# pkorus/neural-imaging

Hardware: AMD Instinct MI355X
Metric: patches/s (fwd+bwd) ISP->JPEG->FAN @256^2 (higher is better)
Workload: dtype bf16; 1 GPU; c4 = train_manipulation UNet->[native,sharpen:1,resample:50,gaussian:0.83,jpeg:80]->dJPEG(QF80,soft)->FAN, ds none, trainable nip+fan, lambda_nip 0.1; raw_patch=128, batch_per_gpu=64, global_batch=64, parallelism=dp1, world_size=1, hip_graph=False

## Files before the change

include/nimg.h:

```cpp
#ifndef NIMG_H
#define NIMG_H

#include <stddef.h>
#include <stdint.h>

#ifdef __cplusplus
extern "C" {
#endif

#define NIMG_OK 0
#define NIMG_ERR_ARG (-1)
#define NIMG_ERR_LAUNCH (-2)
#define NIMG_ERR_WORKSPACE (-3)

#define NIMG_BF16_IN 1
#define NIMG_BF16_OUT 2
#define NIMG_BF16_MASK 4
#define NIMG_BF16_DZ 8
#define NIMG_D2S_OUT 16
#define NIMG_MASK_CONV 128
#define NIMG_COPY_LRELU 64
#define NIMG_S2D_OUT 32
#define NIMG_UNPOOL_OUT 512
#define NIMG_D2S_CONVT 1024
// ... 273 lines not shown
int nimg_conv2d_wgrad_bf16(const float* in1, int c1, const float* in2, int c2, const float* dz, int cout, float* dw,
                           float* db, int n, int h, int wd, int ks, int stride, int pad_t, int pad_l, int pad_mode,
                           int hout, int wout, int accumulate, void* workspace, size_t workspace_bytes, void* stream);

int nimg_conv2d_fwd_smallc_bf16(const float* in, int cin, const float* w, const float* bias, float* out, int cout,
                                int n, int h, int wd, int ks, int pad_mode, int act, float alpha, void* stream);
int nimg_conv2d_fwd_smallc_bf16_ex(const float* in, int cin, const float* w, const float* bias, float* out, int cout,
                                   int n, int h, int wd, int ks, int pad_mode, int act, float alpha, int flags, void* stream);
int nimg_conv2d_dgrad_fewin_bf16(const float* dz, const float* w, float* out, int ci, int cz, int n, int h, int wd,
                                 int ks, void* stream);

int nimg_awgn_fwd(const float* x, const float* noise, float* y, uint8_t* mask, long count, float strength,
                  void* stream);
int nimg_awgn_bwd(const float* x, const float* noise, const float* dy, const uint8_t* mask, float* dx, long count,
                  float strength, void* stream);
int nimg_gamma_fwd(const float* x, float* y, long count, float gamma, void* stream);
int nimg_gamma_bwd(const float* x, const float* dy, float* dx, long count, float gamma, void* stream);
int nimg_median_fwd(const float* x, float* y, uint8_t* sel, int n, int h, int w, int kernel, void* stream);
int nimg_median_bwd(const float* dy, const uint8_t* sel, float* dx, int n, int h, int w, int kernel, void* stream);

#define NIMG_L3IC_E_READ 1
#define NIMG_L3IC_E_LANES 2
#define NIMG_L3IC_E_RANGE 4
#define NIMG_L3IC_E_SYMBOL 8
#define NIMG_L3IC_E_FREQ 16
#define NIMG_L3IC_E_VARINT 32
#define NIMG_L3IC_E_ODD 64
#define NIMG_L3IC_E_UNUSED 128
#define NIMG_L3IC_E_STATE 256
#define NIMG_L3IC_E_RLE 512
size_t nimg_l3ic_workspace_bytes(int n_streams, int n_sym);
int nimg_l3ic_quantise(const float* z, const float* codebook, int codebook_size, uint8_t* idx, int* err, int n, int h,
                       int w, int c, void* stream);
int nimg_l3ic_encode(const uint8_t* idx, int n_streams, int n_sym, uint8_t* out, uint32_t* lengths, uint32_t* hist,
                     uint32_t* freq, void* workspace, size_t workspace_bytes, void* stream);
int nimg_l3ic_decode(const uint8_t* data, const uint32_t* offsets, const uint32_t* lengths, const float* codebook,
                     int codebook_size, float* z, uint32_t* err, int n, int h, int w, int c, void* stream);

size_t nimg_jpeg_workspace_bytes(int n, int h, int w, int hs, int vs);
int nimg_jpeg_transform(const void* x, int is_u8, int n, int h, int w, int hs, int vs, int quality, int16_t* coef, void* workspace,
                        size_t workspace_bytes, void* stream);
int nimg_jpeg_encode(const int16_t* coef, int n, int h, int w, int hs, int vs, uint8_t* out, size_t out_capacity, uint32_t* lengths,
                     void* workspace, size_t workspace_bytes, void* stream);
int nimg_jpeg_reconstruct(const int16_t* coef, int n, int h, int w, int hs, int vs, int quality, float* y, void* workspace,
                          size_t workspace_bytes, void* stream);
int nimg_jpeg_transform_items(const void* x, int is_u8, int n_src, int h, int w, int hs, int vs, const uint8_t* quality, int n_items,
                              int16_t* coef, int* err, void* workspace, size_t workspace_bytes, void* stream);
int nimg_jpeg_reconstruct_items(const int16_t* coef, int n_items, int h, int w, int hs, int vs, const uint8_t* quality, float* y, int* err,
                                void* workspace, size_t workspace_bytes, void* stream);

size_t nimg_jpeg_decode_workspace_bytes(int n, int h, int w, int hs, int vs, size_t ecd_bytes, int subseq_bits);
int nimg_jpeg_decode(const uint8_t* ecd, const uint64_t* ecd_off, const uint8_t* huffman, int n, int h, int w, int hs, int vs,
                     int subseq_bits, int16_t* coef, uint32_t* status, uint32_t* rounds, void* workspace, size_t workspace_bytes,
                     void* stream);
int nimg_jpeg_reconstruct_tables(const int16_t* coef, int n, int h, int w, int hs, int vs, const uint16_t* qtabs, void* y, int out_u8,
                                 void* workspace, size_t workspace_bytes, void* stream);

int nimg_jpeg_histogram(const int16_t* coef, int n, int h, int w, int hs, int vs, uint32_t* hist, void* stream);
int nimg_jpeg_optimal_tables(const uint32_t* hist, int n_tables, uint8_t* tables, uint32_t* status, void* stream);
size_t nimg_jpeg_encode_tables_workspace_bytes(int n, int h, int w, int hs, int vs);
int nimg_jpeg_encode_tables(const int16_t* coef, int n, int h, int w, int hs, int vs, const uint8_t* tables, uint8_t* out,
                            size_t out_capacity, uint32_t* lengths, uint32_t* status, void* workspace, size_t workspace_bytes,
                            void* stream);

int nimg_jpeg_transform_tables(const void* x, int is_u8, int n_src, int h, int w, int hs, int vs, const uint16_t* qtabs, int n_items,
                               int16_t* coef, int* err, void* workspace, size_t workspace_bytes, void* stream);
int nimg_jpeg_tables_from_float(const float* t, int n_sets, int n_tabs, uint16_t* qtabs, uint32_t* status, void* stream);

size_t nimg_jpeg_encode_restart_workspace_bytes(int n, int h, int w, int hs, int vs, int restart_interval);
int nimg_jpeg_encode_restart(const int16_t* coef, int n, int h, int w, int hs, int vs, int restart_interval, uint8_t* out,
                             size_t out_capacity, uint32_t* lengths, void* workspace, size_t workspace_bytes, void* stream);
int nimg_jpeg_histogram_restart(const int16_t* coef, int n, int h, int w, int hs, int vs, int restart_interval, uint32_t* hist,
                                void* stream);
size_t nimg_jpeg_encode_tables_restart_workspace_bytes(int n, int h, int w, int hs, int vs, int restart_interval);
int nimg_jpeg_encode_tables_restart(const int16_t* coef, int n, int h, int w, int hs, int vs, int restart_interval, const uint8_t* tables,
                                    uint8_t* out, size_t out_capacity, uint32_t* lengths, uint32_t* status, void* workspace,
                                    size_t workspace_bytes, void* stream);
size_t nimg_jpeg_decode_restart_workspace_bytes(int n, int h, int w, int hs, int vs, int restart_interval, size_t ecd_bytes,
                                                int subseq_bits);
int nimg_jpeg_decode_restart(const uint8_t* ecd, const uint64_t* ecd_off, const uint8_t* huffman, int n, int h, int w, int hs, int vs,
                             int restart_interval, int subseq_bits, int16_t* coef, uint32_t* status, uint32_t* rounds, void* workspace,
                             size_t workspace_bytes, void* stream);

#ifdef __cplusplus
}
#endif
#endif
```

neural-imaging_amd/_lib.py:

```python
import ctypes
import os
from ctypes import c_float, c_int, c_long, c_size_t, c_void_p

_HERE = os.path.dirname(os.path.abspath(__file__))
LIB_PATH = os.environ.get('NIMG_LIBPATH') or os.path.join(_HERE, 'libnimg.so')

P = c_void_p

PROTOTYPES = {
    'nimg_abi_version': (c_int, []),
    'nimg_djpeg_fwd': (c_int, [P, P, P, P, P, P, c_int, c_int, c_int, c_int, P]),
    'nimg_djpeg_bwd': (c_int, [P, P, P, P, P, c_int, c_int, c_int, c_int, P]),
    'nimg_djpeg_dq_workspace_bytes': (c_size_t, [c_int, c_int, c_int]),
    'nimg_djpeg_bwd_dq': (c_int, [P, P, P, P, P, P, c_int, c_int, c_int, c_int, c_int, P, c_size_t, P]),
    'nimg_jpeg_qtable': (c_int, [c_int, c_int, P]),
    'nimg_conv2d_fwd': (c_int, [P, c_int, P, c_int, P, P, P, c_int, P, c_int, P, c_int, c_int, c_int, c_int, c_int,
                                c_int, c_int, c_int, c_int, c_int, c_int, c_float, P]),
    'nimg_conv_flip_weights': (c_int, [P, P, c_int, c_int, c_int, c_int, P]),
    'nimg_conv2d_wgrad_workspace_bytes': (c_size_t, [c_int, c_int, c_int, c_int, c_int, c_int, c_int]),
    'nimg_conv2d_wgrad': (c_int, [P, c_int, P, c_int, P, c_int, P, P, c_int, c_int, c_int, c_int, c_int, c_int, c_int,
                                  c_int, c_int, c_int, c_int, P, c_size_t, P]),
    'nimg_bias_grad_workspace_bytes': (c_size_t, [c_long, c_int]),
    'nimg_bias_grad': (c_int, [P, P, c_long, c_int, c_int, P, c_size_t, P]),
    'nimg_bias_grad_ex': (c_int, [P, P, c_long, c_int, c_int, P, c_size_t, c_int, P]),
# ... 95 lines not shown
    'nimg_mae255': (c_int, [P, P, P, P, c_long, c_float, c_int, P, c_size_t, P]),
    'nimg_ssim_loss_workspace_bytes': (c_size_t, [c_int, c_int, c_int, c_int, c_int]),
    'nimg_ssim_loss': (c_int, [P, P, P, P, c_int, c_int, c_int, c_int, c_float, P, c_float, c_int, P, c_size_t, P]),
    'nimg_patch_stats': (c_int, [P, c_int, c_int, c_int, P, P, c_int, c_int, c_int, P, P, P]),
    'nimg_patch_select': (c_int, [P, P, P, P, c_int, c_int, c_int, c_int, P, P, P]),
    'nimg_patch_gather': (c_int, [P, P, c_int, c_int, c_int, P, P, c_int, c_int, P, P, P]),
    'nimg_mask_scale': (c_int, [P, P, P, c_long, c_float, P]),
    'nimg_conv5_dgrad_sparse_image_bytes': (c_size_t, [c_int, c_int]),
    'nimg_conv5_dgrad_sparse_weights': (c_int, [P, P, c_int, c_int, P]),
    'nimg_conv5_dgrad_sparse': (c_int, [P, P, c_int, P, P, c_int, P, c_int, c_int, c_int, c_float, c_int, P]),
    'nimg_conv2d_fwd_bf16_res': (c_int, [P, c_int, P, P, P, c_int, P, P, P, c_int, c_int, c_int, c_int, c_int, c_int, c_int, c_int, c_int,
                                 c_int, c_int, c_float, c_int, P]),
    'nimg_conv2d_fwd_bf16_unpool': (c_int, [P, P, c_int, P, P, P, c_int, P, c_int, c_int, c_int, c_int, c_int, c_int, c_int,
                                            c_int, c_int, c_float, c_int, P]),
    'nimg_conv2d_wgrad_bf16_unpool': (c_int, [P, c_int, P, P, c_int, P, P, c_int, c_int, c_int, c_int, c_int, P, c_size_t, P]),
    'nimg_cconv3': (c_int, [P, P, P, P, c_int, c_int, c_int, c_int, P]),
    'nimg_conv5c3_bf16': (c_int, [P, P, P, c_int, c_int, c_int, P]),
    'nimg_cconv3_dgrad_border': (c_int, [P, P, P, c_int, c_int, c_int, P]),
    'nimg_conv1_pool_fwd_c4': (c_int, [P, P, P, P, P, c_int, c_int, c_int, c_float, c_int, P]),
    'nimg_conv1_wgrad_c4_workspace_bytes': (c_size_t, []),
    'nimg_conv1_wgrad_c4': (c_int, [P, P, P, P, P, c_int, c_int, c_int, c_int, c_int, P, c_size_t, P]),
    'nimg_conv1_dgrad_pooled': (c_int, [P, P, P, P, c_int, c_int, c_int, c_int, P]),
    'nimg_confusion_accumulate': (c_int, [P, P, P, P, c_int, c_int, P]),
    'nimg_ssim_planes_workspace_bytes': (c_size_t, [c_int, c_int]),
    'nimg_ssim_planes': (c_int, [P, P, c_int, c_int, c_int, c_int, c_float, P, P, P, P, c_int, P, c_size_t, P]),
    'nimg_msssim_combine': (c_int, [P, P, c_int, c_int, P, P, P]),
    'nimg_ssim_maps_grad': (c_int, [P, P, P, P, P, c_int, c_int, c_int, c_int, P, c_float, c_int, P]),
    'nimg_pad2d': (c_int, [P, P, c_int, c_int, c_int, c_int, c_int, c_int, P]),
    'nimg_conv2d_fwd_bf16_ex': (c_int, [P, c_int, P, c_int, P, P, P, c_int, P, c_int, P, c_int, c_int, c_int, c_int, c_int,
                                        c_int, c_int, c_int, c_int, c_int, c_int, c_float, c_int, P]),
    'nimg_conv2d_wgrad_bf16_ex': (c_int, [P, c_int, P, c_int, P, c_int, P, P, c_int, c_int, c_int, c_int, c_int, c_int,
                                          c_int, c_int, c_int, c_int, c_int, P, c_size_t, c_int, P]),
    'nimg_conv2d_pool_fwd_bf16_ex': (c_int, [P, c_int, P, P, P, P, P, c_int, c_int, c_int, c_int, c_int, c_int, c_float,
                                             c_int, P]),
    'nimg_conv2d_dgrad_unpool_out_bf16': (c_int, [P, c_int, P, P, P, P, c_int, c_int, c_int, c_int, c_int, c_float, P]),
    'nimg_conv2d_fwd_pool_also_bf16': (c_int, [P, c_int, P, P, P, P, P, c_int, c_int, c_int, c_int, c_int, c_float, P]),
    'nimg_conv2d_wgrad_pooled_bf16_ex': (c_int, [P, c_int, P, P, c_int, P, P, c_int, c_int, c_int, c_int, c_int, P,
                                                 c_size_t, c_int, P]),
    'nimg_conv2d_dgrad_fewin_pooled_bf16_ex': (c_int, [P, P, P, P, c_int, c_int, c_int, c_int, c_int, c_int, c_int, P]),
    'nimg_maxpool2_unpool_ex': (c_int, [P, P, P, P, c_int, c_int, c_int, c_int, c_int, c_float, c_int, P]),
    'nimg_conv_weights_bf16_batch': (c_int, [P, c_int, P]),
    'nimg_convt2x2_fwd_bf16': (c_int, [P, P, P, P, c_int, c_int, c_int, c_int, c_int, P]),
    'nimg_convt2x2_fwd_bf16_ex': (c_int, [P, P, P, P, c_int, c_int, c_int, c_int, c_int, c_int, P]),
    'nimg_conv2d_fwd_smallc_bf16': (c_int, [P, c_int, P, P, P, c_int, c_int, c_int, c_int, c_int, c_int, c_int,
                                            c_float, P]),
    'nimg_conv2d_fwd_smallc_bf16_ex': (c_int, [P, c_int, P, P, P, c_int, c_int, c_int, c_int, c_int, c_int, c_int,
                                               c_float, c_int, P]),
    'nimg_conv2d_dgrad_fewin_bf16': (c_int, [P, P, P, c_int, c_int, c_int, c_int, c_int, c_int, P]),
    'nimg_awgn_fwd': (c_int, [P, P, P, P, c_long, c_float, P]),
    'nimg_awgn_bwd': (c_int, [P, P, P, P, P, c_long, c_float, P]),
    'nimg_gamma_fwd': (c_int, [P, P, c_long, c_float, P]),
    'nimg_gamma_bwd': (c_int, [P, P, P, c_long, c_float, P]),
    'nimg_median_fwd': (c_int, [P, P, P, c_int, c_int, c_int, c_int, P]),
    'nimg_median_bwd': (c_int, [P, P, P, c_int, c_int, c_int, c_int, P]),
    'nimg_sparse_axis_apply': (c_int, [P, P, P, P, P, c_int, c_int, c_int, c_int, c_int, c_int, P]),
    'nimg_l3ic_workspace_bytes': (c_size_t, [c_int, c_int]),
    'nimg_l3ic_quantise': (c_int, [P, P, c_int, P, P, c_int, c_int, c_int, c_int, P]),
    'nimg_l3ic_encode': (c_int, [P, c_int, c_int, P, P, P, P, P, c_size_t, P]),
    'nimg_l3ic_decode': (c_int, [P, P, P, P, c_int, P, P, c_int, c_int, c_int, c_int, P]),
    'nimg_jpeg_workspace_bytes': (c_size_t, [c_int, c_int, c_int, c_int, c_int]),
    'nimg_jpeg_transform': (c_int, [P, c_int, c_int, c_int, c_int, c_int, c_int, c_int, P, P, c_size_t, P]),
    'nimg_jpeg_encode': (c_int, [P, c_int, c_int, c_int, c_int, c_int, P, c_size_t, P, P, c_size_t, P]),
    'nimg_jpeg_reconstruct': (c_int, [P, c_int, c_int, c_int, c_int, c_int, c_int, P, P, c_size_t, P]),
    'nimg_jpeg_transform_items': (c_int, [P, c_int, c_int, c_int, c_int, c_int, c_int, P, c_int, P, P, P, c_size_t, P]),
    'nimg_jpeg_reconstruct_items': (c_int, [P, c_int, c_int, c_int, c_int, c_int, P, P, P, P, c_size_t, P]),
    'nimg_jpeg_decode_workspace_bytes': (c_size_t, [c_int, c_int, c_int, c_int, c_int, c_size_t, c_int]),
    'nimg_jpeg_decode': (c_int, [P, P, P, c_int, c_int, c_int, c_int, c_int, c_int, P, P, P, P, c_size_t, P]),
    'nimg_jpeg_reconstruct_tables': (c_int, [P, c_int, c_int, c_int, c_int, c_int, P, P, c_int, P, c_size_t, P]),
    'nimg_jpeg_histogram': (c_int, [P, c_int, c_int, c_int, c_int, c_int, P, P]),
    'nimg_jpeg_optimal_tables': (c_int, [P, c_int, P, P, P]),
    'nimg_jpeg_encode_tables_workspace_bytes': (c_size_t, [c_int, c_int, c_int, c_int, c_int]),
    'nimg_jpeg_encode_tables': (c_int, [P, c_int, c_int, c_int, c_int, c_int, P, P, c_size_t, P, P, P, c_size_t, P]),
    'nimg_jpeg_transform_tables': (c_int, [P, c_int, c_int, c_int, c_int, c_int, c_int, P, c_int, P, P, P, c_size_t, P]),
    'nimg_jpeg_tables_from_float': (c_int, [P, c_int, c_int, P, P, P]),
    'nimg_jpeg_encode_restart_workspace_bytes': (c_size_t, [c_int, c_int, c_int, c_int, c_int, c_int]),
    'nimg_jpeg_encode_restart': (c_int, [P, c_int, c_int, c_int, c_int, c_int, c_int, P, c_size_t, P, P, c_size_t, P]),
    'nimg_jpeg_histogram_restart': (c_int, [P, c_int, c_int, c_int, c_int, c_int, c_int, P, P]),
    'nimg_jpeg_encode_tables_restart_workspace_bytes': (c_size_t, [c_int, c_int, c_int, c_int, c_int, c_int]),
    'nimg_jpeg_encode_tables_restart': (c_int, [P, c_int, c_int, c_int, c_int, c_int, c_int, P, P, c_size_t, P, P, P, c_size_t, P]),
    'nimg_jpeg_decode_restart_workspace_bytes': (c_size_t, [c_int, c_int, c_int, c_int, c_int, c_int, c_size_t, c_int]),
    'nimg_jpeg_decode_restart': (c_int, [P, P, P, c_int, c_int, c_int, c_int, c_int, c_int, c_int, P, P, P, P, c_size_t, P]),
    'nimg_msssim_workspace_bytes': (c_size_t, [c_int, c_int, c_int, c_int]),
    'nimg_msssim': (c_int, [P, P, c_int, c_int, c_int, c_int, c_float, P, P, P, c_size_t, P]),
}

ERRORS = {-1: 'NIMG_ERR_ARG (invalid argument / unsupported configuration)',
          -2: 'NIMG_ERR_LAUNCH (HIP kernel launch failed)',
          -3: 'NIMG_ERR_WORKSPACE (workspace too small)'}

_lib = None


ABI_VERSION = 8
TICKET_BYTES = 64 * 1024


def load():
    global _lib
    if _lib is not None:
        return _lib
    if not os.path.isfile(LIB_PATH):
        raise RuntimeError('libnimg.so not found at {} - build it with neural-imaging_amd/csrc/build.sh '
                           '(or __graft_entry__.build()); there is no CPU fallback'.format(LIB_PATH))
    import torch
    lib = ctypes.CDLL(LIB_PATH)
    for name, (res, args) in PROTOTYPES.items():
        fn = getattr(lib, name)
        fn.restype = res
        fn.argtypes = args
    if lib.nimg_abi_version() != ABI_VERSION:
        raise RuntimeError('libnimg.so at {} has ABI version {}, this binding was written against {} - rebuild it '
                           '(neural-imaging_amd/csrc/build.sh)'.format(LIB_PATH, lib.nimg_abi_version(), ABI_VERSION))
    _lib = lib
    return lib


def call(name, *args):
    rc = getattr(load(), name)(*args)
    if rc != 0:
        raise RuntimeError('{} failed: {}'.format(name, ERRORS.get(rc, rc)))
    return rc
```

neural-imaging_amd/csrc/common.h:

```cpp
#pragma once
#include <hip/hip_runtime.h>
#include <stdint.h>
#include "../../include/nimg.h"

#define NIMG_CHECK_LAUNCH()                                   \
    do {                                                      \
        hipError_t e__ = hipGetLastError();                   \
        if (e__ != hipSuccess) return NIMG_ERR_LAUNCH;        \
    } while (0)

namespace nimg {

constexpr int WAVE = 64;

__device__ __forceinline__ float lrelu(float v, float alpha) { return v > 0.0f ? v : alpha * v; }

__device__ __forceinline__ float wave_sum(float v) {
#pragma unroll
    for (int o = 32; o > 0; o >>= 1) v += __shfl_xor(v, o, 64);
    return v;
}

__device__ __forceinline__ double wave_sum_d(double v) {
#pragma unroll
    for (int o = 32; o > 0; o >>= 1) v += __shfl_xor(v, o, 64);
    return v;
}

__device__ __forceinline__ bool map_coord(int& g, int size, int pad_mode) {
    const bool inside = (unsigned)g < (unsigned)size;
    const int sym = g < 0 ? -1 - g : 2 * size - 1 - g;
    const int ref = g < 0 ? -g : 2 * size - 2 - g;
    const int m = pad_mode == 1 ? sym : ref;
    const bool mapped = pad_mode != 0 && (unsigned)m < (unsigned)size;
    g = inside ? g : (mapped ? m : g);
    return inside || mapped;
}

__device__ __forceinline__ int xcd_order(int bid) {
#ifdef NIMG_NO_XCD_ORDER
    return bid;
#else
    const int g = (int)gridDim.x, x = bid & 7, r = g & 7;
    return x * (g >> 3) + (x < r ? x : r) + (bid >> 3);
#endif
}

typedef float nimg_f32x16 __attribute__((ext_vector_type(16)));

constexpr int EPI_PAD = 4;
template <int NI, bool BLOCK_SYNC = true, typename Emit>
__device__ __forceinline__ void epilogue_via_lds(const nimg_f32x16 (&acc)[NI], float* lds, int lane, Emit emit) {
    constexpr int RS = NI * 32 + EPI_PAD;
    const int half = lane >> 5, n = lane & 31;
    if (BLOCK_SYNC) __syncthreads();
    else __builtin_amdgcn_wave_barrier();
#pragma unroll
    for (int ni = 0; ni < NI; ++ni)
#pragma unroll
        for (int j = 0; j < 16; ++j) lds[((j & 3) + 8 * (j >> 2) + 4 * half) * RS + ni * 32 + n] = acc[ni][j];
    if (BLOCK_SYNC) __syncthreads();
    else __builtin_amdgcn_wave_barrier();
#pragma unroll
    for (int it = 0; it < (32 * NI * 8) / 64; ++it) {
        const int idx = it * 64 + lane, row = idx / (NI * 8), c4 = idx % (NI * 8);
        const float4 v = *reinterpret_cast<const float4*>(lds + row * RS + c4 * 4);
        emit(row, c4 * 4, v);
    }
}

template <int NI, bool BLOCK_SYNC = true, typename Bias, typename Emit>
__device__ __forceinline__ void pool_via_lds(const nimg_f32x16 (&acc)[NI], float* lds, int lane, float alpha, Bias bias4,
                                             Emit emit) {
    constexpr int RS = NI * 32 + EPI_PAD;
    const int half = lane >> 5, n = lane & 31;
    if (BLOCK_SYNC) __syncthreads();
    else __builtin_amdgcn_wave_barrier();
#pragma unroll
    for (int ni = 0; ni < NI; ++ni)
#pragma unroll
        for (int j = 0; j < 16; ++j) lds[((j & 3) + 8 * (j >> 2) + 4 * half) * RS + ni * 32 + n] = acc[ni][j];
    if (BLOCK_SYNC) __syncthreads();
    else __builtin_amdgcn_wave_barrier();
#pragma unroll
    for (int it = 0; it < NI; ++it) {
        const int idx = it * 64 + lane, pc = idx / (NI * 8), c = (idx % (NI * 8)) * 4;
        const float4 b = bias4(c);
        float m[4];
        unsigned char k[4];
#pragma unroll
        for (int pos = 0; pos < 4; ++pos) {
            const float4 r = *reinterpret_cast<const float4*>(lds + (2 * pc + (pos & 1) + 16 * (pos >> 1)) * RS + c);
            const float v[4] = {lrelu(r.x + b.x, alpha), lrelu(r.y + b.y, alpha), lrelu(r.z + b.z, alpha),
                                lrelu(r.w + b.w, alpha)};
#pragma unroll
            for (int e = 0; e < 4; ++e)
                if (pos == 0 || v[e] > m[e]) { m[e] = v[e]; k[e] = (unsigned char)pos; }
        }
// ... 351 lines not shown
```

neural-imaging_amd/csrc/conv_bf16.h:

```cpp
#pragma once
#include <stdlib.h>

#include <cstdlib>
#include "common.h"

struct ConvArgsB {
    const float* in1;
    const float* in2;
    const __bf16* wb;
    const float* bias;
    float* out1;
    float* out2;
    const float* act1;
    float* pool_out;
    unsigned char* pool_idx;
    int C1, C2, O1, O2, CinP;
    int N, H, W, Hout, Wout, pad_t, pad_l;
    int tiles_y, tiles_x, act, pad_mode;
    float alpha;
    int convt;
    int flags;
    const unsigned char* in_idx;
    const float* res;
    float* out1b;
};

namespace {

using namespace nimg;
typedef float f32x16 __attribute__((ext_vector_type(16)));
typedef __bf16 bf16x8 __attribute__((ext_vector_type(8)));

__device__ __forceinline__ bf16x8 pack8(const float (&f)[8]) {
    bf16x8 r;
#pragma unroll
    for (int k = 0; k < 8; ++k) r[k] = (__bf16)f[k];
    return r;
}

typedef __bf16 bf16x4 __attribute__((ext_vector_type(4)));
__device__ __forceinline__ void store4_bf16(float* base_as_bf16, long elem, float4 v) {
    bf16x4 o;
    o[0] = (__bf16)v.x; o[1] = (__bf16)v.y; o[2] = (__bf16)v.z; o[3] = (__bf16)v.w;
    *reinterpret_cast<bf16x4*>(reinterpret_cast<__bf16*>(base_as_bf16) + elem) = o;
}
__device__ __forceinline__ float4 load4_bf16(const float* base_as_bf16, long elem) {
    const bf16x4 o = *reinterpret_cast<const bf16x4*>(reinterpret_cast<const __bf16*>(base_as_bf16) + elem);
    return make_float4((float)o[0], (float)o[1], (float)o[2], (float)o[3]);
}

struct ConvParamsB : ConvArgsB {};

__device__ __forceinline__ unsigned unp_eq_bytes(unsigned k, unsigned pos) {
    const unsigned x = k ^ (pos * 0x01010101u);
    return (((x | (x >> 1)) & 0x01010101u) ^ 0x01010101u) * 0xFFu;
}
__device__ __forceinline__ uint4 unp_route(uint4 g, unsigned k0, unsigned k1, unsigned pos) {
    const unsigned m0 = unp_eq_bytes(k0, pos), m1 = unp_eq_bytes(k1, pos);
    return make_uint4(g.x & __builtin_amdgcn_perm(m0, m0, 0x01010000u), g.y & __builtin_amdgcn_perm(m0, m0, 0x03030202u),
                      g.z & __builtin_amdgcn_perm(m1, m1, 0x01010000u), g.w & __builtin_amdgcn_perm(m1, m1, 0x03030202u));
}

struct EpiBias { float b[8]; };
template <int NI>
__device__ __forceinline__ EpiBias epi_bias_preload(const ConvParamsB& p, int lane, int wn, int co0, int Cout) {
    EpiBias r;
#pragma unroll
    for (int e = 0; e < 8; ++e) r.b[e] = 0.f;
    const int co = co0 + wn * NI * 32 + (lane % (NI * 4)) * 8;
    if (p.bias && co + 7 < Cout) {
        const int cb = (p.flags & NIMG_D2S_CONVT) ? co % (p.O1 >> 2) : co;
        const float4 b0 = *reinterpret_cast<const float4*>(p.bias + cb), b1 = *reinterpret_cast<const float4*>(p.bias + cb + 4);
        r.b[0] = b0.x; r.b[1] = b0.y; r.b[2] = b0.z; r.b[3] = b0.w; r.b[4] = b1.x; r.b[5] = b1.y; r.b[6] = b1.z; r.b[7] = b1.w;
    }
    return r;
}

template <int TH, int TW, int NB, int PMAP>
__device__ __forceinline__ void tile_pixel(int P, int& img, int& dy, int& dx) {
    if constexpr (PMAP == 0) {
        img = P / (TH * TW);
        const int rem = P % (TH * TW);
        dy = rem / TW;
        dx = rem % TW;
    } else if constexpr (NB == 1) {
        static_assert(TH == 16 && TW == 16, "plane layout: 16 x 16 tile");
        const int f = P >> 5, l = P & 31;
        img = 0;
        dy = 4 * (f >> 1) + (l >> 3);
        dx = 8 * (f & 1) + (l & 7);
    } else {
        static_assert(TH == 8 && TW == 8 && NB == 4, "plane layout: 8 x 8 x 4 tile");
        img = (P & 31) >> 3;
        dy = P >> 5;
        dx = P & 7;
    }
}

template <int KS, int TH, int TW, int NB, int MI, int NI, int PMAP = 0>
__device__ __forceinline__ void conv_epilogue_vec(const f32x16 (&acc)[MI][NI], const ConvParamsB& p, unsigned char* smem_raw,
                                                  int wave, int lane, int wm, int wn, int co0, int Cout, int ty0, int tx0,
                                                  int grp, int phase, const EpiBias& pre_) {
#ifdef NIMG_NO_EPI_PRELOAD
    const EpiBias pre = epi_bias_preload<NI>(p, lane, wn, co0, Cout);
    (void)pre_;
#else
    const EpiBias& pre = pre_;
// ... 106 lines not shown
                    *reinterpret_cast<bf16x8*>(reinterpret_cast<__bf16*>(p.out2) + pixoff * p.O2 + (co - p.O1)) = pack8(f);
                }
            });
            if constexpr (TW == 16 && NB == 1 && PMAP == 0)
                if (p.pool_out) {
                    const int Hp = p.Hout >> 1, Wp = p.Wout >> 1, py = (ty0 >> 1) + wm * MI + mi;
                    pool_in_regs8<NI>(acc[mi], elds, lane, p.act == 1 ? p.alpha : 1.0f,
                        [&](int c) { const int co = co0 + wn * NI * 32 + c; return (p.bias && co < Cout) ? p.bias[co] : 0.f; },
                        [&](int pc, int c, float4 lo, float4 hi, uint2 k) {
                            const int co = co0 + wn * NI * 32 + c, px = (tx0 >> 1) + pc;
                            if (co >= Cout || grp >= p.N || py >= Hp || px >= Wp) return;
                            const long o = (((long)grp * Hp + py) * Wp + px) * Cout + co;
                            const float f[8] = {lo.x, lo.y, lo.z, lo.w, hi.x, hi.y, hi.z, hi.w};
                            *reinterpret_cast<bf16x8*>(reinterpret_cast<__bf16*>(p.pool_out) + o) = pack8(f);
                            if (p.pool_idx) *reinterpret_cast<uint2*>(p.pool_idx + o) = k;
                        });
                }
        }
        return;
    }
#endif
#pragma unroll
    for (int mi = 0; mi < MI; ++mi) {
        epilogue_via_lds<NI, false>(acc[mi], elds, lane, [&](int row, int c, float4 v) {
            const int co = co0 + wn * NI * 32 + c;
            if (co >= Cout) return;
            const int P = (wm * MI + mi) * 32 + row;
            int img, dy_, dx_;
            tile_pixel<TH, TW, NB, PMAP>(P, img, dy_, dx_);
            const int oy = ty0 + dy_, ox = tx0 + dx_, n = grp * NB + img;
            if (n >= p.N || oy >= p.Hout || ox >= p.Wout) return;
            const long pixoff = (KS == 1 && p.convt)
                ? ((long)n * 2 * p.Hout + 2 * oy + (phase >> 1)) * (2 * p.Wout) + 2 * ox + (phase & 1)
                : ((long)n * p.Hout + oy) * p.Wout + ox;
            if (p.bias) {
                const float4 b = *reinterpret_cast<const float4*>(p.bias + co);
                v.x += b.x; v.y += b.y; v.z += b.z; v.w += b.w;
            }
            if (p.act == 1) {
                v.x = lrelu(v.x, p.alpha); v.y = lrelu(v.y, p.alpha); v.z = lrelu(v.z, p.alpha); v.w = lrelu(v.w, p.alpha);
            }
            if (co < p.O1) {
                long o = pixoff * p.O1 + co;
                const long om_conv = o;
                if (p.flags & NIMG_D2S_OUT) {
                    const int cd = p.O1 >> 2, blk = co / cd;
                    o = (((long)n * 2 * p.Hout + 2 * oy + (blk >> 1)) * (2 * p.Wout) + 2 * ox + (blk & 1)) * cd + (co - blk * cd);
                }
                if (p.act1) {
                    const long om = (p.flags & NIMG_MASK_CONV) ? om_conv : o;
                    const float4 m = (p.flags & NIMG_BF16_MASK) ? load4_bf16(p.act1, om)
                                                                : *reinterpret_cast<const float4*>(p.act1 + om);
                    v.x *= m.x > 0.f ? 1.0f : p.alpha; v.y *= m.y > 0.f ? 1.0f : p.alpha;
                    v.z *= m.z > 0.f ? 1.0f : p.alpha; v.w *= m.w > 0.f ? 1.0f : p.alpha;
                }
                if (p.res) {
                    const float4 r = *reinterpret_cast<const float4*>(p.res + o);
                    v.x += r.x; v.y += r.y; v.z += r.z; v.w += r.w;
                }
                if (p.flags & NIMG_S2D_OUT)
                    o = (((long)n * (p.Hout >> 1) + (oy >> 1)) * (p.Wout >> 1) + (ox >> 1)) * (4 * p.O1) +
                        (2 * (oy & 1) + (ox & 1)) * p.O1 + co;
                if (p.out1b) {
                    float4 c = v;
                    if (p.flags & NIMG_COPY_LRELU) { c.x = lrelu(c.x, p.alpha); c.y = lrelu(c.y, p.alpha); c.z = lrelu(c.z, p.alpha); c.w = lrelu(c.w, p.alpha); }
                    store4_bf16(p.out1b, o, c);
                }
                if (p.flags & NIMG_BF16_OUT) store4_bf16(p.out1, o, v);
                else *reinterpret_cast<float4*>(p.out1 + o) = v;
            } else {
                if (p.flags & NIMG_BF16_OUT) store4_bf16(p.out2, pixoff * p.O2 + (co - p.O1), v);
                else *reinterpret_cast<float4*>(p.out2 + pixoff * p.O2 + (co - p.O1)) = v;
            }
        });
    }
}

}

template <int KS, int STRIDE, bool INB>
int conv_bf16_dispatch(const ConvArgsB& a, hipStream_t s);
template <int KS, bool INB>
int conv_bf16_launch_16x16(const ConvArgsB& a, bool tn32, hipStream_t s);
```

neural-imaging_amd/csrc/conv_bf16.hip:

```cpp
#include "conv_bf16.h"

namespace {

__global__ void weights_bf16_kernel(const float* __restrict__ w, __bf16* __restrict__ wb, int taps, int cin, int cout,
                                    int mode) {
    const int rows = mode == 0 ? cout : cin, cols = mode == 0 ? cin : cout;
    const int cpad = (cols + 15) / 16 * 16;
    const long total = (long)taps * rows * cpad;
    for (long i = (long)blockIdx.x * blockDim.x + threadIdx.x; i < total; i += (long)gridDim.x * blockDim.x) {
        const int c = (int)(i % 16) + 16 * (int)(i / (16L * rows * taps)), r = (int)((i / 16) % rows);
        const int t = (int)((i / (16L * rows)) % taps);
        float v = 0.f;
        if (c < cols) v = mode == 0 ? w[((long)t * cin + c) * cout + r] : w[((long)(taps - 1 - t) * cin + r) * cout + c];
        wb[i] = (__bf16)v;
    }
}

__global__ __launch_bounds__(256) void weights_bf16_batch_kernel(const long long* __restrict__ table) {
    const long long* e = table + 4 * blockIdx.y;
    const float* w = reinterpret_cast<const float*>(e[0]);
    __bf16* wb = reinterpret_cast<__bf16*>(e[1]);
    const int taps = (int)(e[2] >> 32), mode = (int)(e[2] & 0xffffffffll);
    const int cin = (int)(e[3] >> 32), cout = (int)(e[3] & 0xffffffffll);
    const int rows = mode == 0 ? cout : cin, cols = mode == 0 ? cin : cout;
    const int chunks = (cols + 15) / 16, rblocks = (rows + 63) / 64;
    const int ntiles = chunks * taps * rblocks;
    __shared__ float tile[16][65];
    const int tid = threadIdx.x;
    for (int tl = blockIdx.x; tl < ntiles; tl += gridDim.x) {
        const int rb = tl % rblocks, ct = tl / rblocks, t = ct % taps, chunk = ct / taps;
        const int r0 = rb * 64, c0 = chunk * 16;
        __syncthreads();
        if (mode == 0) {
            const int cl = tid >> 4, rq = (tid & 15) * 4;
#pragma unroll
            for (int k = 0; k < 4; ++k) {
                const int c = c0 + cl, r = r0 + rq + k;
                tile[cl][rq + k] = (c < cols && r < rows) ? w[((long)t * cin + c) * cout + r] : 0.f;
            }
        } else {
            const int rl = tid >> 2, cq = (tid & 3) * 4;
#pragma unroll
            for (int k = 0; k < 4; ++k) {
                const int c = c0 + cq + k, r = r0 + rl;
                tile[cq + k][rl] = (c < cols && r < rows) ? w[((long)(taps - 1 - t) * cin + r) * cout + c] : 0.f;
            }
        }
        __syncthreads();
        const int rl = tid >> 2, kq = (tid & 3) * 4;
        if (r0 + rl < rows) {
            bf16x4 o;
#pragma unroll
            for (int k = 0; k < 4; ++k) o[k] = (__bf16)tile[kq + k][rl];
            *reinterpret_cast<bf16x4*>(wb + ((long)ct * rows + r0 + rl) * 16 + kq) = o;
        }
    }
}

template <int KS, int STRIDE>
int dispatch_b(const ConvParamsB& p, hipStream_t s) {
    if constexpr (STRIDE == 1) {
        if (p.flags & NIMG_BF16_IN) return conv_bf16_dispatch<KS, STRIDE, true>(p, s);
    } else if constexpr (KS == 2) {
        if (p.flags & NIMG_BF16_IN) return conv_bf16_dispatch<KS, STRIDE, true>(p, s);
    } else {
        if (p.flags & NIMG_BF16_IN) return NIMG_ERR_ARG;
    }
    return conv_bf16_dispatch<KS, STRIDE, false>(p, s);
}

}

extern "C" {

size_t nimg_conv_weights_bf16_bytes(int ks_h, int ks_w, int cin, int cout, int mode) {
    const long rows = mode == 0 ? cout : cin, cols = mode == 0 ? cin : cout;
    return (size_t)ks_h * ks_w * rows * ((cols + 15) / 16 * 16) * 2;
}

int nimg_conv_weights_bf16(const float* w, void* wb, int ks_h, int ks_w, int cin, int cout, int mode, void* stream) {
    if (!w || !wb || ks_h <= 0 || ks_w <= 0 || cin <= 0 || cout <= 0 || mode < 0 || mode > 1) return NIMG_ERR_ARG;
    const long total = (long)nimg_conv_weights_bf16_bytes(ks_h, ks_w, cin, cout, mode) / 2;
    const int grid = (int)((total + 255) / 256 > 2048 ? 2048 : (total + 255) / 256);
    hipLaunchKernelGGL(weights_bf16_kernel, dim3(grid), dim3(256), 0, (hipStream_t)stream, w, (__bf16*)wb,
                       ks_h * ks_w, cin, cout, mode);
    NIMG_CHECK_LAUNCH();
    return NIMG_OK;
}

int nimg_conv_weights_bf16_batch(const void* table, int n_entries, void* stream) {
    if (n_entries == 0) return NIMG_OK;
    if (!table || n_entries < 0) return NIMG_ERR_ARG;
    hipLaunchKernelGGL(weights_bf16_batch_kernel, dim3(384, (unsigned)n_entries), dim3(256), 0, (hipStream_t)stream,
                       (const long long*)table);
    NIMG_CHECK_LAUNCH();
    return NIMG_OK;
}

static int conv2d_fwd_bf16_impl(const float* in1, int c1, const float* in2, int c2, const void* wb, const float* bias,
                         float* out1, int o1, float* out2, int o2, const float* act_mask, int n, int h, int wd,
                         int ks, int stride, int pad_t, int pad_l, int pad_mode, int hout, int wout, int act,
                         float alpha, int flags, void* stream, const unsigned char* in_idx = nullptr,
                         const float* res = nullptr, void* out1b = nullptr, float* pool_out = nullptr,
                         unsigned char* pool_idx = nullptr) {
    if (n == 0) return NIMG_OK;
    if (!in1 || !wb || !out1 || c1 <= 0 || c2 < 0 || o1 <= 0 || o2 < 0 || n < 0 || h <= 0 || wd <= 0) return NIMG_ERR_ARG;
    if ((c2 > 0 && !in2) || (o2 > 0 && !out2) || hout <= 0 || wout <= 0 || pad_t < 0 || pad_l < 0) return NIMG_ERR_ARG;
    if (act < 0 || act > 1 || pad_mode < 0 || pad_mode > 2) return NIMG_ERR_ARG;
    if (c2 == 0 ? ((c1 % 4) || ((flags & NIMG_BF16_IN) && (c1 % 8))) : ((c1 % 8) || (c2 % 8)))
        return NIMG_ERR_ARG;
    if (n == 0) return NIMG_OK;
    ConvParamsB p;
    p.in1 = in1; p.in2 = in2; p.wb = (const __bf16*)wb; p.bias = bias; p.out1 = out1; p.out2 = out2; p.act1 = act_mask;
    p.pool_out = pool_out; p.pool_idx = pool_idx; p.convt = 0; p.flags = flags; p.in_idx = in_idx; p.res = res;
    p.out1b = (float*)out1b;
    if (((flags & NIMG_POOL_ALSO) != 0) != (pool_out != nullptr)) return NIMG_ERR_ARG;
    if (res && (ks != 3 || stride != 1)) return NIMG_ERR_ARG;
    if ((res || out1b) && (o2 != 0 || (o1 & 3))) return NIMG_ERR_ARG;
    if (out1b && (flags & NIMG_BF16_OUT)) return NIMG_ERR_ARG;
    if ((flags & NIMG_COPY_LRELU) && (!out1b || act != 0)) return NIMG_ERR_ARG;
    if (in_idx && (!(flags & NIMG_BF16_IN) || stride != 1 || ks != 5 || (h & 1) || (wd & 1) || pad_mode != 0)) return NIMG_ERR_ARG;
    if ((flags & (NIMG_BF16_OUT | NIMG_BF16_MASK)) && ((o1 & 3) || (o2 & 3))) return NIMG_ERR_ARG;
    if ((flags & NIMG_BF16_MASK) && o2 != 0) return NIMG_ERR_ARG;
    if ((flags & NIMG_D2S_OUT) && (ks != 3 || stride != 1 || o2 != 0 || (o1 & 15) || in_idx)) return NIMG_ERR_ARG;
    if ((flags & NIMG_S2D_OUT) && (ks != 3 || stride != 1 || o2 != 0 || (o1 & 3) || in_idx || (hout & 1) || (wout & 1) ||
                                   (flags & NIMG_D2S_OUT)))
        return NIMG_ERR_ARG;
    p.C1 = c1; p.C2 = c2; p.O1 = o1; p.O2 = o2; p.CinP = (c1 + c2 + 15) / 16 * 16;
    p.N = n; p.H = h; p.W = wd; p.Hout = hout; p.Wout = wout; p.pad_t = pad_t; p.pad_l = pad_l;
    p.tiles_y = p.tiles_x = 0; p.act = act; p.pad_mode = pad_mode; p.alpha = alpha;
    hipStream_t s = (hipStream_t)stream;
    if (stride == 1 && ks == 1) return dispatch_b<1, 1>(p, s);
    if (stride == 1 && ks == 3) return dispatch_b<3, 1>(p, s);
    if (stride == 1 && ks == 5) return dispatch_b<5, 1>(p, s);
    if (stride == 2 && ks == 2) return dispatch_b<2, 2>(p, s);
    if (stride == 2 && ks == 5) return dispatch_b<5, 2>(p, s);
    return NIMG_ERR_ARG;
}

int nimg_conv2d_fwd_bf16(const float* in1, int c1, const float* in2, int c2, const void* wb, const float* bias,
                         float* out1, int o1, float* out2, int o2, const float* act_mask, int n, int h, int wd,
                         int ks, int stride, int pad_t, int pad_l, int pad_mode, int hout, int wout, int act,
                         float alpha, void* stream) {
    return conv2d_fwd_bf16_impl(in1, c1, in2, c2, wb, bias, out1, o1, out2, o2, act_mask, n, h, wd, ks, stride, pad_t, pad_l,
                                pad_mode, hout, wout, act, alpha, 0, stream);
}

int nimg_conv2d_fwd_bf16_ex(const float* in1, int c1, const float* in2, int c2, const void* wb, const float* bias,
                            float* out1, int o1, float* out2, int o2, const float* act_mask, int n, int h, int wd,
                            int ks, int stride, int pad_t, int pad_l, int pad_mode, int hout, int wout, int act,
                            float alpha, int flags, void* stream) {
    return conv2d_fwd_bf16_impl(in1, c1, in2, c2, wb, bias, out1, o1, out2, o2, act_mask, n, h, wd, ks, stride, pad_t, pad_l,
                                pad_mode, hout, wout, act, alpha, flags, stream);
}

int nimg_conv2d_fwd_pool_also_bf16(const float* in, int cin, const void* wb, const float* bias, float* out, float* pool_out,
                                   unsigned char* pool_idx, int cout, int n, int h, int wd, int act, float alpha, void* stream) {
#ifdef NIMG_NO_EPI8
    return NIMG_ERR_ARG;
#endif
    if (n == 0) return NIMG_OK;
    if (!pool_out || (h & 1) || (wd & 1) || h <= 8 || wd <= 8 || (cout & 7) || (cin & 7)) return NIMG_ERR_ARG;
    return conv2d_fwd_bf16_impl(in, cin, nullptr, 0, wb, bias, out, cout, nullptr, 0, nullptr, n, h, wd, 3, 1, 1, 1, 0, h, wd, act,
                                alpha, NIMG_BF16_IN | NIMG_BF16_OUT | NIMG_POOL_ALSO, stream, nullptr, nullptr, nullptr, pool_out,
                                pool_idx);
}

int nimg_conv2d_dgrad_unpool_out_bf16(const float* dz, int c1, const void* wb, const float* act, const float* skip, float* out,
                                      int cout, int n, int h, int wd, int apply_mask, float alpha, void* stream) {
#ifdef NIMG_NO_EPI8
    return NIMG_ERR_ARG;
#endif
    if (n == 0) return NIMG_OK;
    if (!dz || !wb || !act || !out || (c1 & 7) || (cout & 7) || h <= 0 || wd <= 0) return NIMG_ERR_ARG;
    if ((long)n * 4 * h * wd * cout * 2 >= (1l << 40)) return NIMG_ERR_ARG;
    ConvParamsB p;
    p.in1 = dz; p.in2 = nullptr; p.wb = (const __bf16*)wb; p.bias = nullptr; p.out1 = out; p.out2 = nullptr; p.act1 = act;
    p.pool_out = nullptr; p.pool_idx = nullptr; p.convt = 0; p.flags = NIMG_BF16_IN | NIMG_BF16_OUT | NIMG_BF16_MASK | NIMG_UNPOOL_OUT;
    p.in_idx = nullptr; p.res = skip; p.out1b = nullptr;
    p.C1 = c1; p.C2 = 0; p.O1 = cout; p.O2 = 0; p.CinP = (c1 + 15) / 16 * 16;
    p.N = n; p.H = h; p.W = wd; p.Hout = h; p.Wout = wd; p.pad_t = p.pad_l = 1;
    p.tiles_y = p.tiles_x = 0; p.act = apply_mask ? 1 : 0; p.pad_mode = 0; p.alpha = alpha;
    return dispatch_b<3, 1>(p, (hipStream_t)stream);
}

int nimg_conv2d_fwd_bf16_res(const float* in1, int c1, const void* wb, const float* bias, float* out1, int o1,
                             const float* act_mask, const float* residual, void* out_bf16_copy, int n, int h, int wd, int ks,
                             int stride, int pad_t, int pad_l, int pad_mode, int hout, int wout, int act, float alpha, int flags,
                             void* stream) {
    if (!residual && !out_bf16_copy) return NIMG_ERR_ARG;
    return conv2d_fwd_bf16_impl(in1, c1, nullptr, 0, wb, bias, out1, o1, nullptr, 0, act_mask, n, h, wd, ks, stride, pad_t, pad_l,
                                pad_mode, hout, wout, act, alpha, flags, stream, nullptr, residual, out_bf16_copy);
}

int nimg_conv2d_fwd_bf16_unpool(const void* in_pooled, const unsigned char* in_idx, int c1, const void* wb, const float* bias,
                                float* out1, int o1, const float* act_mask, int n, int h, int wd, int ks, int pad_t, int pad_l,
                                int hout, int wout, int act, float alpha, int flags, void* stream) {
    if (!in_idx) return NIMG_ERR_ARG;
    return conv2d_fwd_bf16_impl((const float*)in_pooled, c1, nullptr, 0, wb, bias, out1, o1, nullptr, 0, act_mask, n, h, wd, ks, 1,
                                pad_t, pad_l, 0, hout, wout, act, alpha, flags | NIMG_BF16_IN, stream, in_idx);
}

int nimg_convt2x2_fwd_bf16(const float* x, const void* wb, const float* bias, float* y, int n, int h, int wd, int cin,
                           int cout, void* stream) {
    return nimg_convt2x2_fwd_bf16_ex(x, wb, bias, y, n, h, wd, cin, cout, 0, stream);
}

int nimg_convt2x2_fwd_bf16_ex(const float* x, const void* wb, const float* bias, float* y, int n, int h, int wd, int cin,
                              int cout, int flags, void* stream) {
    if (n == 0) return NIMG_OK;
    if (!x || !wb || !y || n < 0 || h <= 0 || wd <= 0 || cin <= 0 || cout <= 0 || (cin % 8)) return NIMG_ERR_ARG;
    if ((flags & ~(NIMG_BF16_IN | NIMG_BF16_OUT)) || ((flags & NIMG_BF16_OUT) && (cout & 3))) return NIMG_ERR_ARG;
    ConvParamsB p;
    p.in1 = x; p.in2 = nullptr; p.wb = (const __bf16*)wb; p.bias = bias; p.out1 = y; p.out2 = nullptr; p.act1 = nullptr;
    p.pool_out = nullptr; p.pool_idx = nullptr; p.convt = 1; p.flags = flags; p.in_idx = nullptr; p.res = nullptr; p.out1b = nullptr;
    p.C1 = cin; p.C2 = 0; p.O1 = cout; p.O2 = 0; p.CinP = (cin + 15) / 16 * 16;
    p.N = n; p.H = h; p.W = wd; p.Hout = h; p.Wout = wd; p.pad_t = 0; p.pad_l = 0;
    p.tiles_y = p.tiles_x = 0; p.act = 0; p.pad_mode = 0; p.alpha = 0.f;
#ifndef NIMG_NO_EPI8
    static const bool no_fat = getenv("NIMG_NO_CONVT_FAT") != nullptr;
    if (!no_fat && (flags & NIMG_BF16_OUT) && (cout & 7) == 0) {
        p.convt = 0; p.O1 = 4 * cout; p.flags = flags | NIMG_D2S_CONVT;
    }
#endif
    return dispatch_b<1, 1>(p, (hipStream_t)stream);
}

}
```

neural-imaging_amd/csrc/conv_bf16_k5b.hip:

```cpp
#include "conv_bf16_tile.h"

template int conv_bf16_dispatch<5, 1, true>(const ConvArgsB&, hipStream_t);
template int conv_bf16_launch_16x16<5, true>(const ConvArgsB&, bool, hipStream_t);
```

neural-imaging_amd/csrc/conv_bf16_packed.hip:

```cpp
#include "conv_bf16_wgrad.h"

namespace {

template <int KS, int CINP, int TN>
__global__ __launch_bounds__(256) void conv_fwd_packed_bf16_kernel(const float* __restrict__ in,
                                                                   const float* __restrict__ w,
                                                                   const float* __restrict__ bias,
                                                                   float* __restrict__ out,
                                                                   float* __restrict__ pool_out,
                                                                   unsigned char* __restrict__ pool_idx, int N, int H,
                                                                   int W, int Cout, int pad_mode, int act, float alpha,
                                                                   int tiles_y, int tiles_x, int tiles_per_wg,
                                                                   int out_bf16) {
    constexpr int TH = 16, TW = 16, THH = TH + KS - 1, TWH = TW + KS - 1, P = (KS - 1) / 2;
    constexpr int NPIXH = THH * TWH, PS = ((NPIXH + 31) / 32) * 32 + 2;
    constexpr int KTOT = KS * KS * CINP, KSTEPS = (KTOT + 15) / 16, KP = KSTEPS * 16;
    constexpr int NI = TN / 32, MI = 2;
    extern __shared__ __attribute__((aligned(16))) unsigned char smem_raw[];
    float* sA = reinterpret_cast<float*>(smem_raw);
    constexpr int A_BYTES = (CINP * PS * 4 + 15) / 16 * 16;
    __bf16* sB = reinterpret_cast<__bf16*>(smem_raw + A_BYTES);
    const int tid = threadIdx.x, lane = tid & 63, half = lane >> 5;
    const int wave = __builtin_amdgcn_readfirstlane(tid >> 6);
    const int cot = (Cout + TN - 1) / TN;
// ... 479 lines not shown
    constexpr int MF = (KS * KS + 32 / C - 1) / (32 / C);
    constexpr bool FOLD = MF * NI <= 2;
    constexpr size_t lds_f = FOLD ? (size_t)3 * MF * NI * 16 * 64 * sizeof(float) : 0;
    constexpr size_t lds = lds_t > lds_f ? lds_t : lds_f;
    if (!q.dz_idx)
        hipLaunchKernelGGL((conv_wgrad_packed_bf16_kernel<KS, C, NI, 0>), dim3((unsigned)pblocks), dim3(256), lds, s, q);
    else if (q.flags & NIMG_BF16_DZ)
        hipLaunchKernelGGL((conv_wgrad_packed_bf16_kernel<KS, C, NI, 2>), dim3((unsigned)pblocks), dim3(256), lds, s, q);
    else
        hipLaunchKernelGGL((conv_wgrad_packed_bf16_kernel<KS, C, NI, 1>), dim3((unsigned)pblocks), dim3(256), lds, s, q);
    return FOLD ? 1 : 4;
}

int nimg_internal_wgrad_packed(WgradArgsB* a, int ks, bool want_db, hipStream_t s) {
    a->tiles_y = cdiv(a->Hout, B_TH); a->tiles_x = cdiv(a->Wout, B_TW);
    a->splits = nimg_internal_wgrad_packed_splits(a->Cout, a->N, a->Hout, a->Wout);
    const long work = (long)a->N * a->tiles_y * a->tiles_x;
    a->work_per_split = (int)((work + a->splits - 1) / a->splits);
    if (want_db) a->db_partial = a->partial + (size_t)4 * a->splits * ks * ks * a->C1 * a->Cout;
    const int ni = a->Cout <= 32 ? 1 : 2;
    const long pblocks = (long)cdiv(a->Cout, 32 * ni) * a->splits;
    const WgradParamsB q{*a};
    int slabs_per_wg;
    if (ks == 5 && q.C1 == 3) slabs_per_wg = ni == 1 ? launch_wgrad_packed<5, 3, 1>(q, pblocks, s) : launch_wgrad_packed<5, 3, 2>(q, pblocks, s);
    else if (ks == 5) slabs_per_wg = ni == 1 ? launch_wgrad_packed<5, 4, 1>(q, pblocks, s) : launch_wgrad_packed<5, 4, 2>(q, pblocks, s);
    else if (q.C1 == 3) slabs_per_wg = ni == 1 ? launch_wgrad_packed<3, 3, 1>(q, pblocks, s) : launch_wgrad_packed<3, 3, 2>(q, pblocks, s);
    else slabs_per_wg = ni == 1 ? launch_wgrad_packed<3, 4, 1>(q, pblocks, s) : launch_wgrad_packed<3, 4, 2>(q, pblocks, s);
    if (hipGetLastError() != hipSuccess) return -1;
    return slabs_per_wg * a->splits;
}

extern "C" {

static int launch_packed_bf16(const float* in, int cin, const float* w, const float* bias, float* out, float* pool_out,
                              unsigned char* pool_idx, int cout, int n, int h, int wd, int ks, int pad_mode, int act,
                              float alpha, hipStream_t s, int out_bf16 = 0) {
    const int ty = cdiv(h, 16), tx = cdiv(wd, 16);
    const long total_tiles = (long)ty * tx * n;
    const int tpw = total_tiles >= 8192 ? 8 : (total_tiles >= 2048 ? 2 : 1);
#define NIMG_FP(KS_, C_, TN_)                                                                                     \
    do {                                                                                                          \
        constexpr int THH = 16 + KS_ - 1, NPIXH = THH * THH, PS = ((NPIXH + 31) / 32) * 32 + 2;                    \
        constexpr int KP = (KS_ * KS_ * C_ + 15) / 16 * 16;                                                       \
        constexpr size_t lds = (size_t)((C_ * PS * 4 + 15) / 16 * 16) + (size_t)TN_ * KP * 2 +                    \
                               (size_t)4 * 32 * (TN_ + EPI_PAD) * sizeof(float);                                  \
        const long blocks = cdiv(total_tiles, tpw) * (long)cdiv(cout, TN_);                                       \
        hipLaunchKernelGGL((conv_fwd_packed_bf16_kernel<KS_, C_, TN_>), dim3((unsigned)blocks), dim3(256), lds, s, \
                           in, w, bias, out, pool_out, pool_idx, n, h, wd, cout, pad_mode, act, alpha, ty, tx, tpw,    \
                           out_bf16);                                                                             \
    } while (0)
    if (ks == 5 && cin == 3) { if (cout > 32) NIMG_FP(5, 3, 64); else NIMG_FP(5, 3, 32); }
    else if (ks == 5 && cin == 4) { if (cout > 32) NIMG_FP(5, 4, 64); else NIMG_FP(5, 4, 32); }
    else if (ks == 3 && cin == 3) { if (cout > 32) NIMG_FP(3, 3, 64); else NIMG_FP(3, 3, 32); }
    else if (ks == 3 && cin == 4) { if (cout > 32) NIMG_FP(3, 4, 64); else NIMG_FP(3, 4, 32); }
    else return NIMG_ERR_ARG;
#undef NIMG_FP
    NIMG_CHECK_LAUNCH();
    return NIMG_OK;
}

int nimg_conv2d_fwd_smallc_bf16(const float* in, int cin, const float* w, const float* bias, float* out, int cout,
                                int n, int h, int wd, int ks, int pad_mode, int act, float alpha, void* stream) {
    return nimg_conv2d_fwd_smallc_bf16_ex(in, cin, w, bias, out, cout, n, h, wd, ks, pad_mode, act, alpha, 0, stream);
}

int nimg_conv2d_fwd_smallc_bf16_ex(const float* in, int cin, const float* w, const float* bias, float* out, int cout,
                                   int n, int h, int wd, int ks, int pad_mode, int act, float alpha, int flags, void* stream) {
    if (n == 0) return NIMG_OK;
    if (!in || !w || !out || n < 0 || h <= 0 || wd <= 0 || cout <= 0 || pad_mode < 0 || pad_mode > 2) return NIMG_ERR_ARG;
    if ((flags & ~NIMG_BF16_OUT) || ((flags & NIMG_BF16_OUT) && (cout & 3))) return NIMG_ERR_ARG;
    return launch_packed_bf16(in, cin, w, bias, out, nullptr, nullptr, cout, n, h, wd, ks, pad_mode, act, alpha,
                              (hipStream_t)stream, (flags & NIMG_BF16_OUT) ? 1 : 0);
}

int nimg_conv2d_pool_fwd_bf16(const float* in, int cin, const float* w, const void* wb, const float* bias,
                              float* pool_out, unsigned char* pool_idx, int cout, int n, int h, int wd, int ks, int act,
                              float alpha, void* stream) {
    return nimg_conv2d_pool_fwd_bf16_ex(in, cin, w, wb, bias, pool_out, pool_idx, cout, n, h, wd, ks, act, alpha, 0, stream);
}

int nimg_conv2d_pool_fwd_bf16_ex(const float* in, int cin, const float* w, const void* wb, const float* bias,
                                 float* pool_out, unsigned char* pool_idx, int cout, int n, int h, int wd, int ks,
                                 int act, float alpha, int flags, void* stream) {
    if (n == 0) return NIMG_OK;
    if (!in || !pool_out || cin <= 0 || cout <= 0 || (cout & 3) || n < 0 || h <= 0 || wd <= 0) return NIMG_ERR_ARG;
    if ((h & 1) || (wd & 1) || (ks != 3 && ks != 5) || act < 0 || act > 1) return NIMG_ERR_ARG;
    if (n == 0) return NIMG_OK;
    hipStream_t s = (hipStream_t)stream;
    if (cin == 3 || cin == 4) {
        if (!w) return NIMG_ERR_ARG;
        if (flags & NIMG_BF16_IN) return NIMG_ERR_ARG;
        return launch_packed_bf16(in, cin, w, bias, nullptr, pool_out, pool_idx, cout, n, h, wd, ks, 0, act, alpha, s,
                                  (flags & NIMG_BF16_OUT) ? 1 : 0);
    }
    if (!wb || (cin % 8)) return NIMG_ERR_ARG;
    ConvParamsB p;
    p.in1 = in; p.in2 = nullptr; p.wb = (const __bf16*)wb; p.bias = bias; p.out1 = nullptr; p.out2 = nullptr;
    p.act1 = nullptr; p.pool_out = pool_out; p.pool_idx = pool_idx; p.convt = 0; p.flags = flags; p.in_idx = nullptr; p.res = nullptr;
    p.out1b = nullptr;
    p.C1 = cin; p.C2 = 0; p.O1 = cout; p.O2 = 0; p.CinP = (cin + 15) / 16 * 16;
    p.N = n; p.H = h; p.W = wd; p.Hout = h; p.Wout = wd; p.pad_t = p.pad_l = (ks - 1) / 2;
    p.tiles_y = p.tiles_x = 0; p.act = act; p.pad_mode = 0; p.alpha = alpha;
    const bool tn32 = cout <= 32 || (long)cdiv(cout, 64) * cdiv(h, 16) * cdiv(wd, 16) * n < 384;
    if (flags & NIMG_BF16_IN)
        return ks == 3 ? conv_bf16_launch_16x16<3, true>(p, tn32, s) : conv_bf16_launch_16x16<5, true>(p, tn32, s);
    return ks == 3 ? conv_bf16_launch_16x16<3, false>(p, tn32, s) : conv_bf16_launch_16x16<5, false>(p, tn32, s);
}

static int dgrad_fewin_impl(const float* dz, const unsigned char* dz_idx, int dz_bf16, const float* w, float* out,
                            int ci, int cz, int n, int h, int wd, int ks, void* stream) {
    if (!dz || !w || !out || n < 0 || h <= 0 || wd <= 0) return NIMG_ERR_ARG;
    if (cz != 32 || ci != 3 || ks != 5) return NIMG_ERR_ARG;
    if (n == 0) return NIMG_OK;
    constexpr int KS = 5, TH = 8, TWO = 32 - (KS - 1), ROWS = TH + KS - 1;
    const int ty = cdiv(h, TH), tx = cdiv(wd, TWO);
    constexpr size_t lds = (size_t)(ROWS * 32 * 4 + KS * 32 * 4) * sizeof(uint4) + 4 * 32 * 16 * sizeof(float);
    const long total = (long)n * ty * tx;
    if (total >= (1L << 31)) return NIMG_ERR_ARG;
    const unsigned grid = (unsigned)(total < 4096 ? total : 4096);
    hipStream_t s = (hipStream_t)stream;
    if (!dz_idx)
        hipLaunchKernelGGL((conv_dgrad_fewin_bf16_kernel<5, 3, 0>), dim3(grid), dim3(256), lds, s, dz, dz_idx, w, out, n, h, wd,
                           ty, tx);
    else if (dz_bf16)
        hipLaunchKernelGGL((conv_dgrad_fewin_bf16_kernel<5, 3, 2>), dim3(grid), dim3(256), lds, s, dz, dz_idx, w, out, n, h, wd,
                           ty, tx);
    else
        hipLaunchKernelGGL((conv_dgrad_fewin_bf16_kernel<5, 3, 1>), dim3(grid), dim3(256), lds, s, dz, dz_idx, w, out, n, h, wd,
                           ty, tx);
    NIMG_CHECK_LAUNCH();
    return NIMG_OK;
}

int nimg_conv2d_dgrad_fewin_bf16(const float* dz, const float* w, float* out, int ci, int cz, int n, int h, int wd,
                                 int ks, void* stream) {
    return dgrad_fewin_impl(dz, nullptr, 0, w, out, ci, cz, n, h, wd, ks, stream);
}

int nimg_conv2d_dgrad_fewin_pooled_bf16(const float* g, const unsigned char* idx, const float* w, float* out, int ci,
                                        int cz, int n, int h, int wd, int ks, void* stream) {
    return nimg_conv2d_dgrad_fewin_pooled_bf16_ex(g, idx, w, out, ci, cz, n, h, wd, ks, 0, stream);
}

int nimg_conv2d_dgrad_fewin_pooled_bf16_ex(const float* g, const unsigned char* idx, const float* w, float* out, int ci,
                                           int cz, int n, int h, int wd, int ks, int flags, void* stream) {
    if (!idx || (h & 1) || (wd & 1)) return NIMG_ERR_ARG;
    return dgrad_fewin_impl(g, idx, (flags & NIMG_BF16_DZ) ? 1 : 0, w, out, ci, cz, n, h, wd, ks, stream);
}

}
```

neural-imaging_amd/csrc/conv_bf16_ring.h:

```cpp
#pragma once
#include "conv_bf16.h"

namespace {

typedef unsigned int r_u32x4 __attribute__((ext_vector_type(4)));
__device__ __forceinline__ void glds16(r_u32x4 rsrc, unsigned lds_addr, unsigned voff, int soff) {
    unsigned keep;
    asm volatile("s_mov_b32 %0, m0\n\ts_mov_b32 m0, %1\n\ts_nop 0\n\tbuffer_load_dwordx4 %2, %3, %4 offen lds\n\ts_mov_b32 m0, %0"
                 : "=&s"(keep) : "s"(lds_addr), "v"(voff), "s"(rsrc), "s"(soff) : "memory");
}
__device__ __forceinline__ void dma_wait() { asm volatile("s_waitcnt vmcnt(0)" ::: "memory"); }
template <int N>
__device__ __forceinline__ void dma_wait_leave() { asm volatile("s_waitcnt vmcnt(%0)" ::"n"(N) : "memory"); }

#ifndef NIMG_RING_ABLATE
#define NIMG_RING_ABLATE 0
#endif

template <int TN, int NW = 4, int KS = 5>
struct RingGeom {
    static constexpr int NI = TN / 32, MI = NI == 1 ? 4 : 8 / NI;
    static constexpr int NT = 64 * NW;
    static constexpr int TH = 2 * NW * MI, TW = 16, THH = TH + KS - 1, TWH = TW + KS - 1;
    static constexpr int NPIXH = THH * TWH, AP = (NPIXH * 2 + NT - 1) / NT;
// ... 170 lines not shown
                    else dma_wait_leave<NLO>();
                }
                asm volatile("s_waitcnt lgkmcnt(0)\n\ts_barrier" ::: "memory");
            }
            s0 = (s0 + 2) % 3;
        }
    } else
    for (int c = 0; c < chunks; ++c) {
        const int ab = G::ADBL ? (c & 1) * ABUF : 0;
        const bool more = c + 1 < chunks;
#pragma unroll
        for (int ky = 0; ky < KS; ++ky) {
            const int slot = (c + ky) & 1;
            if constexpr (!(ABL & 1)) {
                if (ky < KS - 1) gldsB(c, ky + 1, slot ^ 1);
                else if (more) gldsB(c + 1, 0, slot ^ 1);
            }
            if constexpr (!(ABL & 2)) if (ky == 0 && more) fetchA((c + 1) * 16);
            const uint4* sBs = sB + slot * SLOT + bbase;
#pragma unroll
            for (int kx = 0; kx < KS; ++kx) {
                bf16x8 a[MI], b[NI];
#pragma unroll
                for (int mi = 0; mi < MI; ++mi) {
                    if constexpr (ABL & 8) { a[mi] = a0[mi]; continue; }
                    const uint4 v = sA[ab + abase[mi] + ky * 32 + kx];
                    a[mi] = *reinterpret_cast<const bf16x8*>(&v);
                }
#pragma unroll
                for (int ni = 0; ni < NI; ++ni) {
                    if constexpr (ABL & 8) { b[ni] = b0[ni]; continue; }
                    const uint4 v = sBs[(kx * TN + ni * 32) * 2];
                    b[ni] = *reinterpret_cast<const bf16x8*>(&v);
                }
#pragma unroll
                for (int mi = 0; mi < MI; ++mi)
#pragma unroll
                    for (int ni = 0; ni < NI; ++ni)
                        acc[mi][ni] = __builtin_amdgcn_mfma_f32_32x32x16_bf16(a[mi], b[ni], acc[mi][ni], 0, 0, 0);
            }
            if constexpr (!(ABL & 2)) if (G::ADBL && ky == KS - 1 && more) commitA(ab ^ ABUF);
            if constexpr (!(ABL & 4)) {
                dma_wait();
                __syncthreads();
            }
            if constexpr (!(ABL & 2)) if (!G::ADBL && ky == KS - 1 && more) {
                commitA(0);
                if constexpr (!(ABL & 4)) __syncthreads();
            }
        }
    }
    if constexpr (ABL & 4) { dma_wait(); __syncthreads(); }
    if constexpr (ABL & 16) {
        float sacc = 0.f;
#pragma unroll
        for (int mi = 0; mi < MI; ++mi)
#pragma unroll
            for (int ni = 0; ni < NI; ++ni)
#pragma unroll
                for (int j = 0; j < 16; ++j) sacc += acc[mi][ni][j];
        if (sacc == 123.456f) p.out1[0] = sacc;
        return;
    }
    if constexpr (KS == 3) {
        conv_epilogue_vec<3, TH, TW, 1, MI, NI>(acc, p, smem_raw, wave, lane, wave, 0, co0, Cout, ty0, tx0, grp, 0,
                                                epi_bias_preload<NI>(p, lane, 0, co0, Cout));
        return;
    }
    float* elds = reinterpret_cast<float*>(smem_raw) + wave * (32 * (NI * 32 + EPI_PAD));
    if (p.pool_out) {
        const int Hp = p.Hout >> 1, Wp = p.Wout >> 1;
        const float al = p.act == 1 ? p.alpha : 1.0f;
        if (p.flags & NIMG_BF16_OUT) {
#pragma unroll
            for (int mi = 0; mi < MI; ++mi) {
                const int py = (ty0 >> 1) + wave * MI + mi;
                pool_in_regs8<NI>(acc[mi], elds, lane, al,
                    [&](int c) { return p.bias ? p.bias[co0 + c] : 0.f; },
                    [&](int pc, int c, float4 lo, float4 hi, uint2 k) {
                        const int px = (tx0 >> 1) + pc;
                        if (grp >= p.N || py >= Hp || px >= Wp) return;
                        const long o = (((long)grp * Hp + py) * Wp + px) * Cout + co0 + c;
                        const float f[8] = {lo.x, lo.y, lo.z, lo.w, hi.x, hi.y, hi.z, hi.w};
                        *reinterpret_cast<bf16x8*>(reinterpret_cast<__bf16*>(p.pool_out) + o) = pack8(f);
                        if (p.pool_idx) *reinterpret_cast<uint2*>(p.pool_idx + o) = k;
                    });
            }
            return;
        }
#pragma unroll
        for (int mi = 0; mi < MI; ++mi) {
            const int py = (ty0 >> 1) + wave * MI + mi;
            pool_in_regs<NI>(acc[mi], elds, lane, al,
                [&](int c) { return p.bias ? p.bias[co0 + c] : 0.f; },
                [&](int pc, int c, float4 v, uchar4 k) {
                    const int co = co0 + c, px = (tx0 >> 1) + pc;
                    if (grp >= p.N || py >= Hp || px >= Wp) return;
                    const long o = (((long)grp * Hp + py) * Wp + px) * Cout + co;
                    if (p.flags & NIMG_BF16_OUT) store4_bf16(p.pool_out, o, v);
                    else *reinterpret_cast<float4*>(p.pool_out + o) = v;
                    if (p.pool_idx) *reinterpret_cast<uchar4*>(p.pool_idx + o) = k;
                });
        }
        return;
    }
    if ((p.flags & NIMG_BF16_OUT) && (!p.act1 || (p.flags & NIMG_BF16_MASK))) {
#pragma unroll
        for (int mi = 0; mi < MI; ++mi) {
            epilogue_via_lds8<NI>(acc[mi], elds, lane, [&](int row, int c, float4 lo, float4 hi) {
                const int P = (wave * MI + mi) * 32 + row;
                const int oy = ty0 + P / TW, ox = tx0 + P % TW;
                if (grp >= p.N || oy >= p.Hout || ox >= p.Wout) return;
                const long o = (((long)grp * p.Hout + oy) * p.Wout + ox) * Cout + co0 + c;
                float f[8] = {lo.x, lo.y, lo.z, lo.w, hi.x, hi.y, hi.z, hi.w};
                if (p.bias) {
#pragma unroll
                    for (int e = 0; e < 8; ++e) f[e] += p.bias[co0 + c + e];
                }
                if (p.act == 1) {
#pragma unroll
                    for (int e = 0; e < 8; ++e) f[e] = lrelu(f[e], p.alpha);
                }
                if (p.act1) {
                    const bf16x8 m = *reinterpret_cast<const bf16x8*>(reinterpret_cast<const __bf16*>(p.act1) + o);
#pragma unroll
                    for (int e = 0; e < 8; ++e) f[e] *= (float)m[e] > 0.f ? 1.0f : p.alpha;
                }
                *reinterpret_cast<bf16x8*>(reinterpret_cast<__bf16*>(p.out1) + o) = pack8(f);
            });
        }
        return;
    }
#pragma unroll
    for (int mi = 0; mi < MI; ++mi) {
        epilogue_via_lds<NI, false>(acc[mi], elds, lane, [&](int row, int c, float4 v) {
            const int co = co0 + c;
            const int P = (wave * MI + mi) * 32 + row;
            const int oy = ty0 + P / TW, ox = tx0 + P % TW;
            if (grp >= p.N || oy >= p.Hout || ox >= p.Wout) return;
            const long o = (((long)grp * p.Hout + oy) * p.Wout + ox) * Cout + co;
            if (p.bias) {
                const float4 b = *reinterpret_cast<const float4*>(p.bias + co);
                v.x += b.x; v.y += b.y; v.z += b.z; v.w += b.w;
            }
            if (p.act == 1) {
                v.x = lrelu(v.x, p.alpha); v.y = lrelu(v.y, p.alpha); v.z = lrelu(v.z, p.alpha); v.w = lrelu(v.w, p.alpha);
            }
            if (p.act1) {
                const float4 m = (p.flags & NIMG_BF16_MASK) ? load4_bf16(p.act1, o) : *reinterpret_cast<const float4*>(p.act1 + o);
                v.x *= m.x > 0.f ? 1.0f : p.alpha; v.y *= m.y > 0.f ? 1.0f : p.alpha;
                v.z *= m.z > 0.f ? 1.0f : p.alpha; v.w *= m.w > 0.f ? 1.0f : p.alpha;
            }
            if (p.flags & NIMG_BF16_OUT) store4_bf16(p.out1, o, v);
            else *reinterpret_cast<float4*>(p.out1 + o) = v;
        });
    }
}

template <int TN, int NW = 4, int KS = 5>
int launch_conv5_ring(const ConvParamsB& p, hipStream_t stream) {
    using G = RingGeom<TN, NW, KS>;
    if constexpr (NW == 4 && TN == 128 && KS == 5) {
        static const bool nw8 = getenv("NIMG_RING_NW8") != nullptr;
        if (nw8 && p.Hout % 32 == 0) return launch_conv5_ring<TN, 8>(p, stream);
    }
    ConvParamsB q = p;
    q.tiles_y = cdiv(p.Hout, G::TH);
    q.tiles_x = cdiv(p.Wout, G::TW);
    const long blocks = (long)(p.O1 / TN) * q.tiles_y * q.tiles_x * p.N;
    auto kern = conv5_ring_kernel<TN, false, NW, KS>;
    if constexpr (KS == 5) { if (p.in_idx) kern = conv5_ring_kernel<TN, true, NW, KS>; }
    (void)hipFuncSetAttribute((const void*)kern, hipFuncAttributeMaxDynamicSharedMemorySize, (int)G::LDS);
    hipLaunchKernelGGL(kern, dim3((unsigned)blocks), dim3(G::NT), G::LDS, stream, q);
    NIMG_CHECK_LAUNCH();
    return NIMG_OK;
}

}
```

neural-imaging_amd/csrc/conv_bf16_tile.h:

```cpp
#pragma once
#include "conv_bf16_dma.h"
#include "conv_bf16_ring.h"

namespace {

template <int KS, int STRIDE, int TH, int TW, int NB, int TN, bool INB, bool BUF = false, bool UNP = false, int CKT = 16>
__global__ __launch_bounds__(256) void conv_fwd_bf16_kernel(const ConvParamsB p) {
#ifdef NIMG_CK32
    constexpr int CK = CKT != 16 ? CKT : ((KS == 3 && !INB && !BUF) ? 32 : 16);
#else
    constexpr int CK = CKT;
#endif
    static_assert(CK == 16 || CK == 32 || (CK == 64 && KS == 1 && !BUF), "K chunk");
    constexpr int CKH = CK / 8;
    static_assert(!UNP || (INB && BUF && STRIDE == 1), "un-pooling input: bf16 buffer-load path only");
    constexpr int THH = (TH - 1) * STRIDE + KS, TWH = (TW - 1) * STRIDE + KS;
    constexpr int NPIXH = NB * THH * TWH;
    constexpr int MFRAGS = NB * TH * TW / 32, NFRAGS = TN / 32;
    constexpr int WAVES_M = MFRAGS >= 4 ? 4 : MFRAGS, WAVES_N = 4 / WAVES_M;
    constexpr int MI = MFRAGS / WAVES_M, NI = NFRAGS / WAVES_N;
    constexpr int TAPS = KS * KS;
    static_assert(NI >= 1 && MFRAGS % WAVES_M == 0, "bad tile configuration");
    extern __shared__ __attribute__((aligned(16))) unsigned char smem_raw[];
    constexpr bool PLANAR = (STRIDE == 1 && TW == 16 && NB == 1 && KS == 5);
// ... 189 lines not shown
                    const uint4 v = CKH == 2 ? sB[row * 2 + (half ^ ((row >> 3) & 1))]
                                             : (CKH == 4 ? sB[row * 4 + ((2 * ks2 + half) ^ ((row >> 2) & 3))]
                                                         : sB[row * 8 + ((2 * ks2 + half) ^ ((row >> 1) & 7))]);
                    b[ni] = *reinterpret_cast<const bf16x8*>(&v);
                }
#pragma unroll
                for (int mi = 0; mi < MI; ++mi)
#pragma unroll
                    for (int ni = 0; ni < NI; ++ni)
                        acc[mi][ni] = __builtin_amdgcn_mfma_f32_32x32x16_bf16(a[mi], b[ni], acc[mi][ni], 0, 0, 0);
            }
        }
    }
    if constexpr ((GABL & 16) != 0) {
        float sacc = 0.f;
#pragma unroll
        for (int mi = 0; mi < MI; ++mi)
#pragma unroll
            for (int ni = 0; ni < NI; ++ni)
#pragma unroll
                for (int j = 0; j < 16; ++j) sacc += acc[mi][ni][j];
        if (sacc == 123.456f) p.out1[0] = sacc;
        return;
    }
    if constexpr (TW == 16 && NB == 1 && STRIDE == 1) {
        if (p.pool_out && !(p.flags & NIMG_POOL_ALSO)) {
            float* elds = reinterpret_cast<float*>(smem_raw) + wave * (32 * (NI * 32 + EPI_PAD));
            const int Hp = p.Hout >> 1, Wp = p.Wout >> 1;
            const float al = p.act == 1 ? p.alpha : 1.0f;
#pragma unroll
            for (int mi = 0; mi < MI; ++mi) {
                const int py = (ty0 >> 1) + wm * MI + mi;
                pool_via_lds<NI>(acc[mi], elds, lane, al,
                    [&](int c) {
                        const int co = co0 + wn * NI * 32 + c;
                        return (p.bias && co < Cout) ? *reinterpret_cast<const float4*>(p.bias + co)
                                                     : make_float4(0.f, 0.f, 0.f, 0.f);
                    },
                    [&](int pc, int c, float4 v, uchar4 k) {
                        const int co = co0 + wn * NI * 32 + c, px = (tx0 >> 1) + pc;
                        if (co >= Cout || grp >= p.N || py >= Hp || px >= Wp) return;
                        const long o = (((long)grp * Hp + py) * Wp + px) * Cout + co;
                        if (p.flags & NIMG_BF16_OUT) store4_bf16(p.pool_out, o, v);
                        else *reinterpret_cast<float4*>(p.pool_out + o) = v;
                        if (p.pool_idx) *reinterpret_cast<uchar4*>(p.pool_idx + o) = k;
                    });
            }
            return;
        }
    }
    if ((p.O1 & 3) == 0 && (p.O2 & 3) == 0) {
        conv_epilogue_vec<KS, TH, TW, NB, MI, NI>(acc, p, smem_raw, wave, lane, wm, wn, co0, Cout, ty0, tx0, grp, phase, epi_pre);
        return;
    }
#pragma unroll
    for (int ni = 0; ni < NI; ++ni) {
        const int co = co0 + (wn * NI + ni) * 32 + (lane & 31);
        if (co >= Cout) continue;
        const float bv = p.bias ? p.bias[co] : 0.f;
#pragma unroll
        for (int mi = 0; mi < MI; ++mi)
#pragma unroll
            for (int j = 0; j < 16; ++j) {
                const int row = (j & 3) + 8 * (j >> 2) + 4 * half;
                const int P = (wm * MI + mi) * 32 + row;
                const int img = P / (TH * TW), rem = P % (TH * TW);
                const int oy = ty0 + rem / TW, ox = tx0 + rem % TW, n = grp * NB + img;
                if (n >= p.N || oy >= p.Hout || ox >= p.Wout) continue;
                const long pixoff = (KS == 1 && p.convt)
                    ? ((long)n * 2 * p.Hout + 2 * oy + (phase >> 1)) * (2 * p.Wout) + 2 * ox + (phase & 1)
                    : ((long)n * p.Hout + oy) * p.Wout + ox;
                float v = acc[mi][ni][j] + bv;
                if (p.act == 1) v = lrelu(v, p.alpha);
                if (co < p.O1) {
                    if (p.act1) v *= (p.act1[pixoff * p.O1 + co] > 0.f ? 1.0f : p.alpha);
                    p.out1[pixoff * p.O1 + co] = v;
                } else {
                    p.out2[pixoff * p.O2 + (co - p.O1)] = v;
                }
            }
    }
}

template <int KS, int STRIDE, int TH, int TW, int NB, int TN, bool INB = false, bool BUF = false, int CKT = 16>
int launch_conv_b(const ConvParamsB& p, hipStream_t stream) {
    if constexpr (KS == 1 && !BUF && CKT == 16) {
        static const bool no_ck64 = getenv("NIMG_NO_CK64") != nullptr;
        if (!no_ck64 && (p.C1 + p.C2) % 64 == 0 && (p.C2 == 0 || p.C1 % 64 == 0))
            return launch_conv_b<KS, STRIDE, TH, TW, NB, TN, INB, false, 64>(p, stream);
    }
    if constexpr (INB && !BUF && KS == 3 && STRIDE == 1 && CKT == 16 && (TN == 32 || TN == 64)) {
        static const bool no_dma = getenv("NIMG_NO_CONV3_DMA") != nullptr || getenv("NIMG_NO_BUFFER_LOADS") != nullptr;
        const long px = (long)p.N * p.H * p.W;
        const long w_bytes = (long)(p.CinP >> 4) * KS * KS * 16 * (p.O1 + p.O2) * 2;
        static const long max_hw = getenv("NIMG_CONV3_DMA_MAXHW") ? atol(getenv("NIMG_CONV3_DMA_MAXHW")) : 1024;
        const bool pays = p.C2 > 0 || (long)p.Hout * p.Wout <= max_hw;
        if (!no_dma && pays && !p.convt && !p.in_idx && (!p.pool_out || (p.flags & NIMG_POOL_ALSO)) && p.C1 % 16 == 0 && p.C2 % 16 == 0 && (p.O1 & 3) == 0 &&
            (p.O2 & 3) == 0 && px * p.C1 * 2 < (1l << 31) - 65536 && px * p.C2 * 2 < (1l << 31) - 65536 &&
            w_bytes < (1l << 31) - 65536)
            return launch_conv3_dma<TH, TW, NB, TN>(p, stream);
    }
    if constexpr (INB && !BUF && (KS == 5 || KS == 3) && STRIDE == 1 && 128 % TN == 0) {
        static const bool no_buf = getenv("NIMG_NO_BUFFER_LOADS") != nullptr;
        const int Cin = p.C1 + p.C2, Cout = p.O1 + p.O2;
        const long in_bytes = ((long)p.N * p.H * p.W * p.C1 * 2) >> (p.in_idx ? 2 : 0);
        const long w_bytes = (long)(p.CinP >> 4) * KS * KS * 16 * Cout * 2;
        if (!no_buf && p.C2 == 0 && Cin % 16 == 0 && Cout % TN == 0 && !p.convt && in_bytes < (1l << 31) - 65536 &&
            w_bytes < (1l << 31) - 65536) {
            if constexpr (KS == 3 && TH == 16 && TW == 16 && NB == 1 && TN == 64) {
                static const long ring3_min = getenv("NIMG_CONV3_RING_MIN") ? atol(getenv("NIMG_CONV3_RING_MIN")) : -1;
                const long rblocks = (long)(Cout / 128) * cdiv(p.Hout, 16) * cdiv(p.Wout, 16) * p.N;
                if (ring3_min >= 0 && Cout % 128 == 0 && p.O2 == 0 && (p.O1 & 7) == 0 && p.pad_t == 1 && p.pad_l == 1 && p.Hout == p.H &&
                    p.Wout == p.W && !p.pool_out && !p.in_idx && rblocks >= ring3_min)
                    return launch_conv5_ring<128, 4, 3>(p, stream);
            }
            if constexpr (KS == 5 && TH == 16 && TW == 16 && NB == 1 && TN == 64) {
                static const bool no_ring = getenv("NIMG_NO_CONV5_RING") != nullptr;
                static const bool no_ring64 = getenv("NIMG_NO_CONV5_RING64") != nullptr;
                const bool plain_epi = !p.res && !p.out1b && !(p.flags & (NIMG_D2S_OUT | NIMG_S2D_OUT | NIMG_COPY_LRELU));
                if (!no_ring && plain_epi && p.O2 == 0 && p.pad_t == 2 && p.pad_l == 2 && p.Hout == p.H && p.Wout == p.W) {
                    static const bool tn64 = getenv("NIMG_RING_TN64") != nullptr;
                    if (Cout % 128 == 0 && !(tn64 && p.Hout >= 32)) return launch_conv5_ring<128>(p, stream);
                    if (!no_ring64 && p.Hout >= 32) return launch_conv5_ring<64>(p, stream);
                }
            }
            return launch_conv_b<KS, STRIDE, TH, TW, NB, TN, true, true>(p, stream);
        }
    }
    constexpr int THH = (TH - 1) * STRIDE + KS, TWH = (TW - 1) * STRIDE + KS;
    constexpr bool PLANAR = (STRIDE == 1 && TW == 16 && NB == 1 && KS == 5);
#ifdef NIMG_CK32
    constexpr int CKH = CKT != 16 ? CKT / 8 : ((KS == 3 && !INB && !BUF) ? 4 : 2);
#else
    constexpr int CKH = CKT / 8;
#endif
    constexpr size_t a_entries = PLANAR ? (size_t)2 * THH * 32 : (size_t)NB * THH * TWH * CKH;
    constexpr size_t lds_tiles = (a_entries + (size_t)KS * KS * TN * CKH) * sizeof(uint4);
    constexpr size_t lds_epi = (size_t)4 * 32 * (TN + EPI_PAD) * sizeof(float);
    constexpr size_t lds = lds_tiles > lds_epi ? lds_tiles : lds_epi;
    ConvParamsB q = p;
    q.tiles_y = cdiv(p.Hout, TH);
    q.tiles_x = cdiv(p.Wout, TW);
    const long blocks = (long)cdiv(p.O1 + p.O2, TN) * q.tiles_y * q.tiles_x * cdiv(p.N, NB) * (p.convt ? 4 : 1);
    auto kern = conv_fwd_bf16_kernel<KS, STRIDE, TH, TW, NB, TN, INB, BUF, false, CKT>;
    if (p.in_idx) {
        if constexpr (INB && BUF && STRIDE == 1 && CKT == 16) kern = conv_fwd_bf16_kernel<KS, STRIDE, TH, TW, NB, TN, true, true, true>;
        else return NIMG_ERR_ARG;
    }
    (void)hipFuncSetAttribute((const void*)kern, hipFuncAttributeMaxDynamicSharedMemorySize, (int)lds);
    hipLaunchKernelGGL(kern, dim3((unsigned)blocks), dim3(256), lds, stream, q);
    NIMG_CHECK_LAUNCH();
    return NIMG_OK;
}

template <int KS, int STRIDE, bool INB>
int dispatch_b_t(const ConvParamsB& p, hipStream_t s) {
    const int Cout = p.O1 + p.O2;
    const bool small = (p.Hout <= 8 && p.Wout <= 8);
    const long blocks64 = (long)cdiv(Cout, 64) * cdiv(p.Hout, small ? 8 : 16) * cdiv(p.Wout, small ? 8 : 16) *
                          cdiv(p.N, small ? 4 : 1);
    static const long tn32_below = getenv("NIMG_TN32_BELOW") ? atol(getenv("NIMG_TN32_BELOW")) : 384;
    const bool tn32 = (Cout <= 32) || (blocks64 < 512 && Cout % 64 != 0) || (blocks64 < tn32_below);
    if (small)
        return tn32 ? launch_conv_b<KS, STRIDE, 8, 8, 4, 32, INB>(p, s) : launch_conv_b<KS, STRIDE, 8, 8, 4, 64, INB>(p, s);
    if constexpr (STRIDE == 1 && KS == 5) {
        if constexpr (INB) {
            static const bool no_ring32 = getenv("NIMG_NO_CONV5_RING32") != nullptr || getenv("NIMG_NO_CONV5_RING") != nullptr ||
                                          getenv("NIMG_NO_BUFFER_LOADS") != nullptr;
            const long in_bytes = ((long)p.N * p.H * p.W * p.C1 * 2) >> (p.in_idx ? 2 : 0);
            if (!no_ring32 && !p.res && !p.out1b && !(p.flags & NIMG_COPY_LRELU) && Cout == 32 && p.O2 == 0 && p.C2 == 0 && p.C1 % 16 == 0 && !p.convt && p.pad_t == 2 && p.pad_l == 2 &&
                p.Hout == p.H && p.Wout == p.W && p.Hout >= 32 && in_bytes < (1l << 31) - 65536)
                return launch_conv5_ring<32>(p, s);
        }
        if (Cout <= 32 && !p.pool_out && p.Hout % 32 == 0 && (long)cdiv(p.Hout, 32) * cdiv(p.Wout, 16) * p.N >= 2048)
            return launch_conv_b<KS, STRIDE, 32, 16, 1, 32, INB>(p, s);
    }
    return tn32 ? launch_conv_b<KS, STRIDE, 16, 16, 1, 32, INB>(p, s) : launch_conv_b<KS, STRIDE, 16, 16, 1, 64, INB>(p, s);
}

}

template <int KS, int STRIDE, bool INB>
int conv_bf16_dispatch(const ConvArgsB& a, hipStream_t s) {
    return dispatch_b_t<KS, STRIDE, INB>(ConvParamsB{a}, s);
}
template <int KS, bool INB>
int conv_bf16_launch_16x16(const ConvArgsB& a, bool tn32, hipStream_t s) {
    const ConvParamsB p{a};
    return tn32 ? launch_conv_b<KS, 1, 16, 16, 1, 32, INB>(p, s) : launch_conv_b<KS, 1, 16, 16, 1, 64, INB>(p, s);
}
```

neural-imaging_amd/csrc/frontend.hip:

```cpp
#include <stdlib.h>
#include "common.h"

namespace {

using namespace nimg;

typedef __bf16 bf16x4 __attribute__((ext_vector_type(4)));

struct CConvParams {
    const float* in;
    const float* w;
    float* out_f32;
    uint2* out_c4;
    int N, H, W, pad_mode, tiles_y, tiles_x;
};

template <int TPR, int RPT>
__global__ __launch_bounds__(256) void cconv_kernel(const float* __restrict__ p_in, const float* __restrict__ p_w,
                                                    float* __restrict__ p_out_f32, uint2* __restrict__ p_out_c4,
                                                    const CConvParams p) {
    constexpr int TW = 4 * TPR, TROWS = 256 / TPR, TR = TROWS * RPT, HR = TR + 4, HC = TW + 4;
    constexpr int RS = (HC * 3 + 3) / 4 * 4;
    constexpr int NPIX = HR * HC, PPT = (NPIX + 255) / 256;
    extern __shared__ __attribute__((aligned(16))) float tile[];
// ... 138 lines not shown
            }
        }
    }
}

__global__ void cdgrad_border_kernel(const float* __restrict__ dc, const float* __restrict__ nf, float* __restrict__ dx, int N,
                                     int H, int W) {
    const int per = 4 * W + 4 * (H - 4);
    const long total = (long)N * per;
    for (long t = (long)blockIdx.x * blockDim.x + threadIdx.x; t < total; t += (long)gridDim.x * blockDim.x) {
        const int n = (int)(t / per), b = (int)(t % per);
        int y, x;
        if (b < 4 * W) {
            const int r = b / W;
            y = r < 2 ? r : H - 4 + r;
            x = b % W;
        } else {
            const int c = (b - 4 * W) & 3;
            y = 2 + (b - 4 * W) / 4;
            x = c < 2 ? c : W - 4 + c;
        }
        int us[3], vs[3], nu = 0, nv = 0;
        us[nu++] = y + 2;
        if (y < 2) us[nu++] = 1 - y;
        if (y >= H - 2) us[nu++] = 2 * H + 1 - y;
        vs[nv++] = x + 2;
        if (x < 2) vs[nv++] = 1 - x;
        if (x >= W - 2) vs[nv++] = 2 * W + 1 - x;
        float a0 = 0.f, a1 = 0.f, a2 = 0.f;
        for (int iu = 0; iu < nu; ++iu)
            for (int iv = 0; iv < nv; ++iv) {
                if (iu == 0 && iv == 0) continue;
                const int u = us[iu], v = vs[iv];
                for (int ky = 0; ky < 5; ++ky) {
                    const int py = u - ky;
                    if (py < 0 || py >= H) continue;
                    for (int kx = 0; kx < 5; ++kx) {
                        const int px = v - kx;
                        if (px < 0 || px >= W) continue;
                        const float* g = dc + (((long)n * H + py) * W + px) * 3;
                        const float* wv = nf + (ky * 5 + kx) * 9;
#pragma unroll
                        for (int o = 0; o < 3; ++o) {
                            a0 = fmaf(g[o], wv[o], a0);
                            a1 = fmaf(g[o], wv[3 + o], a1);
                            a2 = fmaf(g[o], wv[6 + o], a2);
                        }
                    }
                }
            }
        float* d = dx + (((long)n * H + y) * W + x) * 3;
        d[0] += a0; d[1] += a1; d[2] += a2;
    }
}

#ifndef CONV1_WGS
#define CONV1_WGS 3
#endif
typedef float f32x16 __attribute__((ext_vector_type(16)));
typedef __bf16 bf16x8 __attribute__((ext_vector_type(8)));
typedef unsigned int u32x2 __attribute__((ext_vector_type(2)));
typedef unsigned int u32x4 __attribute__((ext_vector_type(4)));

__device__ __forceinline__ float dpp_swap1(float v) {
    return __int_as_float(__builtin_amdgcn_mov_dpp(__float_as_int(v), 0xB1, 0xF, 0xF, true));
}

__device__ __forceinline__ unsigned pk_bf16(float a, float b) {
    typedef __bf16 bf16x2 __attribute__((ext_vector_type(2)));
    bf16x2 r;
    r[0] = (__bf16)a; r[1] = (__bf16)b;
    return *reinterpret_cast<const unsigned*>(&r);
}

__device__ __forceinline__ void conv1_slot(int ks, int h, int j, int& ky, int& kx) {
    if (ks < 5) { ky = ks; kx = 2 * h + j; }
    else if (ks == 5) { ky = 2 * h + j; kx = 4; }
    else { ky = (h == 0 && j == 0) ? 4 : -1; kx = 4; }
}

template <int TWD, bool OUT_BF16>
__global__ __launch_bounds__(256, CONV1_WGS) void conv1_pool_fwd_kernel(const void* __restrict__ c4, const float* __restrict__ w,
                                                             const float* __restrict__ bias, void* __restrict__ pooled,
                                                             unsigned char* __restrict__ pidx, int N, int H, int W,
                                                             float alpha, int tiles_y, int tiles_x) {
    constexpr int TRD = 8, HR = TRD + 4, HC = TWD + 4, NPC = HC / 2;
    constexpr int PT = NPC <= 64 ? 64 : 128, RG = 256 / PT, RPTS = (HR + RG - 1) / RG;
    constexpr int EXC = NPC > PT ? NPC - PT : 0, EXN = EXC * HR;
    constexpr int UC = TWD / 64, UNITS = (TRD / 2) * UC;
    constexpr unsigned OOB = 0x80000000u;
    static_assert(EXN <= 256 && HC % 2 == 0, "staging layout");
    __shared__ __attribute__((aligned(16))) uint4 tile[HR * NPC];
    const int tid = threadIdx.x, lane = tid & 63, h = lane >> 5, nl = lane & 31;
    const int wave = __builtin_amdgcn_readfirstlane(tid >> 6);
    const int tiles = tiles_y * tiles_x, total = N * tiles;

    const int co_a = 16 * ((nl >> 2) & 1) + 4 * (nl >> 3) + (nl & 3);
    bf16x8 wa[7];
#pragma unroll
    for (int ks = 0; ks < 7; ++ks)
#pragma unroll
        for (int j = 0; j < 2; ++j) {
            int ky, kx;
            conv1_slot(ks, h, j, ky, kx);
#pragma unroll
            for (int c = 0; c < 4; ++c)
                wa[ks][4 * j + c] = (__bf16)((ky >= 0 && c < 3) ? w[((ky * 5 + kx) * 3 + c) * 32 + co_a] : 0.f);
        }
    float br[16];
#pragma unroll
    for (int r = 0; r < 16; ++r) br[r] = bias ? bias[16 * h + r] : 0.f;

    const __amdgpu_buffer_rsrc_t rin = __builtin_amdgcn_make_buffer_rsrc(const_cast<void*>(c4), 0, (int)((long)N * H * W * 8),
                                                                         0x00020000);
    const int sp = tid % PT, sr = tid / PT;
    const int er = EXC ? tid / (EXC ? EXC : 1) : 0, ep = EXC ? PT + tid % (EXC ? EXC : 1) : 0;
    u32x4 pre[RPTS], pre_x;
    auto fetch = [&](int t) {
        const int n = t / tiles, tl = t % tiles;
        const int y0 = (tl / tiles_x) * TRD, x0 = (tl % tiles_x) * TWD;
        const int gx = x0 - 2 + 2 * sp;
        const unsigned xb = (sp < NPC && (unsigned)gx < (unsigned)W) ? (unsigned)(gx * 8) : OOB;
#pragma unroll
        for (int q = 0; q < RPTS; ++q) {
            const int gy = y0 - 2 + q * RG + sr;
            const bool ok = ((unsigned)gy < (unsigned)H) & (q * RG + sr < HR);
            pre[q] = __builtin_amdgcn_raw_buffer_load_b128(rin, ((unsigned)((n * H + gy) * W * 8) + xb) | (ok ? 0u : OOB), 0, 0);
        }
        if constexpr (EXN > 0) {
            const int gy = y0 - 2 + er, gx2 = x0 - 2 + 2 * ep;
            const bool ok = ((unsigned)gy < (unsigned)H) & ((unsigned)gx2 < (unsigned)W) & (tid < EXN);
            pre_x = __builtin_amdgcn_raw_buffer_load_b128(rin, ok ? (unsigned)(((n * H + gy) * W + gx2) * 8) : OOB, 0, 0);
        }
    };
    const int first = xcd_order(blockIdx.x);
    if (first < total) fetch(first);
    const int Hp = H >> 1, Wp = W >> 1;
    for (int t = first; t < total; t += gridDim.x) {
        const int n = t / tiles, tl = t % tiles;
        const int y0 = (tl / tiles_x) * TRD, x0 = (tl % tiles_x) * TWD;
        __syncthreads();
        if (sp < NPC) {
#pragma unroll
            for (int q = 0; q < RPTS; ++q)
                if (q * RG + sr < HR) tile[(q * RG + sr) * NPC + sp] = *reinterpret_cast<const uint4*>(&pre[q]);
        }
        if constexpr (EXN > 0) {
            if (tid < EXN) tile[er * NPC + ep] = *reinterpret_cast<const uint4*>(&pre_x);
        }
        __syncthreads();
        if (t + (int)gridDim.x < total) fetch(t + gridDim.x);

        const unsigned char* tb = reinterpret_cast<const unsigned char*>(tile);
        for (int u = wave; u < UNITS; u += 4) {
            const int ur = u / UC, uc = u % UC;
            const int a0 = ((2 * ur) * HC + 64 * uc + 2 * nl) * 8;
            const int baseA = a0 + h * 16, baseB = a0 + h * (2 * HC * 8);
            f32x16 acc[2][2];
            auto rd = [&](int off) { return *reinterpret_cast<const u32x2*>(tb + off); };
            auto op = [](u32x2 lo, u32x2 hi) {
                u32x4 b;
                b[0] = lo[0]; b[1] = lo[1]; b[2] = hi[0]; b[3] = hi[1];
                return *reinterpret_cast<const bf16x8*>(&b);
            };
#pragma unroll
            for (int ks = 0; ks < 7; ++ks)
#pragma unroll
                for (int row = 0; row < 2; ++row) {
                    bf16x8 b0, b1;
                    if (ks < 5) {
                        const int o = baseA + (ks + row) * HC * 8;
                        const u32x2 q0 = rd(o), q1 = rd(o + 8), q2 = rd(o + 16);
                        b0 = op(q0, q1);
                        b1 = op(q1, q2);
                    } else if (ks == 5) {
                        const int o = baseB + row * HC * 8 + 4 * 8;
                        b0 = op(rd(o), rd(o + HC * 8));
                        b1 = op(rd(o + 8), rd(o + HC * 8 + 8));
                    } else {
                        const int o = a0 + ((4 + row) * HC + 4) * 8;
                        const u32x2 q0 = rd(o), q1 = rd(o + 8);
                        b0 = op(q0, q0);
                        b1 = op(q1, q1);
                    }
                    if (ks == 0) {
                        const f32x16 zero = {0.f, 0.f, 0.f, 0.f, 0.f, 0.f, 0.f, 0.f, 0.f, 0.f, 0.f, 0.f, 0.f, 0.f, 0.f, 0.f};
                        acc[row][0] = __builtin_amdgcn_mfma_f32_32x32x16_bf16(wa[0], b0, zero, 0, 0, 0);
                        acc[row][1] = __builtin_amdgcn_mfma_f32_32x32x16_bf16(wa[0], b1, zero, 0, 0, 0);
                    } else {
                        acc[row][0] = __builtin_amdgcn_mfma_f32_32x32x16_bf16(wa[ks], b0, acc[row][0], 0, 0, 0);
                        acc[row][1] = __builtin_amdgcn_mfma_f32_32x32x16_bf16(wa[ks], b1, acc[row][1], 0, 0, 0);
                    }
                }
            float mx[16];
            unsigned kk[16];
#pragma unroll
            for (int r = 0; r < 16; ++r) {
                const float tl = acc[0][0][r], tr = acc[0][1][r], bl = acc[1][0][r], bq = acc[1][1][r];
                const bool rt = tr > tl, rb = bq > bl;
                const float mt = rt ? tr : tl, mb = rb ? bq : bl;
                const unsigned kt = rt ? 1u : 0u, kb = rb ? 3u : 2u;
                const bool bot = mb > mt;
                const float v = (bot ? mb : mt) + br[r];
                mx[r] = __builtin_fmaxf(v, alpha * v);
                kk[r] = bot ? kb : kt;
            }
            const int py = (y0 + 2 * ur) >> 1, px = ((x0 + 64 * uc) >> 1) + nl;
            if (py < Hp && px < Wp) {
                const long po = ((long)(n * Hp + py) * Wp + px) * 32 + 16 * h;
                if (pidx) {
                    unsigned ib = 0;
#pragma unroll
                    for (int r = 0; r < 16; ++r) ib |= kk[r] << (2 * r);
                    *reinterpret_cast<unsigned*>(pidx + (po >> 2)) = ib;
                }
                if constexpr (OUT_BF16) {
                    unsigned pb[8];
#pragma unroll
                    for (int g = 0; g < 8; ++g) pb[g] = pk_bf16(mx[2 * g], mx[2 * g + 1]);
                    uint4* d = reinterpret_cast<uint4*>(reinterpret_cast<unsigned short*>(pooled) + po);
                    d[0] = make_uint4(pb[0], pb[1], pb[2], pb[3]);
                    d[1] = make_uint4(pb[4], pb[5], pb[6], pb[7]);
                } else {
                    float4* d = reinterpret_cast<float4*>(reinterpret_cast<float*>(pooled) + po);
#pragma unroll
                    for (int g = 0; g < 4; ++g) d[g] = make_float4(mx[4 * g], mx[4 * g + 1], mx[4 * g + 2], mx[4 * g + 3]);
                }
            }
        }
    }
}

template <int TPR, int RPT>
int launch_cconv(CConvParams p, hipStream_t s) {
    constexpr int TW = 4 * TPR, TR = (256 / TPR) * RPT, HR = TR + 4, HC = TW + 4, RS = (HC * 3 + 3) / 4 * 4;
    constexpr size_t lds = ((size_t)HR * RS + 5 * 48) * sizeof(float);
    p.tiles_y = cdiv(p.H, TR);
    p.tiles_x = cdiv(p.W, TW);
    const long total = (long)p.N * p.tiles_y * p.tiles_x;
    static const int capmul = getenv("NIMG_CCONV_CAP") ? atoi(getenv("NIMG_CCONV_CAP")) : 0;
    const long cap = 256L * (capmul > 0 ? capmul : (lds > 40000 ? 3 : (lds > 20000 ? 4 : 8)));
    auto k = cconv_kernel<TPR, RPT>;
    (void)hipFuncSetAttribute((const void*)k, hipFuncAttributeMaxDynamicSharedMemorySize, (int)lds);
    hipLaunchKernelGGL(k, dim3((unsigned)(total < cap ? total : cap)), dim3(256), lds, s, p.in, p.w, p.out_f32, p.out_c4, p);
    NIMG_CHECK_LAUNCH();
    return NIMG_OK;
}

typedef short s16x4 __attribute__((ext_vector_type(4)));
typedef short s16x8 __attribute__((ext_vector_type(8)));

__device__ __forceinline__ bf16x8 tr_read8(const unsigned char* p0, const unsigned char* p1) {
    const s16x4 lo = __builtin_amdgcn_ds_read_tr16_b64_v4i16((s16x4 __attribute__((address_space(3)))*)p0);
    const s16x4 hi = __builtin_amdgcn_ds_read_tr16_b64_v4i16((s16x4 __attribute__((address_space(3)))*)p1);
    s16x8 r;
    r[0] = lo[0]; r[1] = lo[1]; r[2] = lo[2]; r[3] = lo[3]; r[4] = hi[0]; r[5] = hi[1]; r[6] = hi[2]; r[7] = hi[3];
    return *reinterpret_cast<bf16x8*>(&r);
}

__device__ __forceinline__ u32x2 argmax2_bytes(unsigned short k16) {
    const unsigned k = k16;
    auto spread = [](unsigned x) {
        const unsigned t = (x | (x << 12)) & 0x000F000Fu;
        return (t | (t << 6)) & 0x03030303u;
    };
    u32x2 r;
    r[0] = spread(k & 0xFFu);
    r[1] = spread(k >> 8);
    return r;
}

__device__ __forceinline__ unsigned eq_bytes(unsigned k, unsigned pos) {
    const unsigned x = k ^ (pos * 0x01010101u);
    return (((x | (x >> 1)) & 0x01010101u) ^ 0x01010101u) * 0xFFu;
}

constexpr int F_TR = 8, F_TW = 64, F_HR = F_TR + 4, F_HC = F_TW + 4;
constexpr int F_C4_BYTES = F_HR * F_HC * 8, F_DZ_BYTES = F_TR * F_TW * 64;
constexpr int F_DW = 25 * 3 * 32;

template <bool GB>
__global__ __launch_bounds__(256) void conv1_wgrad_pooled_kernel(const void* __restrict__ c4, const void* __restrict__ gp,
                                                                 const unsigned char* __restrict__ pidx,
                                                                 float* __restrict__ dw_slabs, float* __restrict__ db_slabs,
                                                                 int N, int H, int W, int tiles_y, int tiles_x, int per_wg) {
    constexpr unsigned OOB = 0x80000000u;
    __shared__ __attribute__((aligned(16))) unsigned char smem[F_C4_BYTES + F_DZ_BYTES];
    unsigned char* sC = smem;
    unsigned char* sZ = smem + F_C4_BYTES;
    const int tid = threadIdx.x, lane = tid & 63, kh = lane >> 5, q1 = (lane >> 4) & 1, g16 = lane & 15;
    const int wave = __builtin_amdgcn_readfirstlane(tid >> 6);
    const int tiles = tiles_y * tiles_x, total = N * tiles;
    const int Hp = H >> 1, Wp = W >> 1;
    const int w_begin = blockIdx.x * per_wg, w_end = min(total, w_begin + per_wg);

    const __amdgpu_buffer_rsrc_t rc = __builtin_amdgcn_make_buffer_rsrc(const_cast<void*>(c4), 0, (int)((long)N * H * W * 8),
                                                                        0x00020000);
    const __amdgpu_buffer_rsrc_t rg = __builtin_amdgcn_make_buffer_rsrc(const_cast<void*>(gp), 0,
                                                                        (int)((long)N * Hp * Wp * 32 * (GB ? 2 : 4)), 0x00020000);
    const __amdgpu_buffer_rsrc_t rk = __builtin_amdgcn_make_buffer_rsrc(const_cast<unsigned char*>(pidx), 0,
                                                                        (int)((long)N * Hp * Wp * 8), 0x00020000);
    const int tl = 4 * q1 + (g16 & 3);
    int a_off[4];
#pragma unroll
    for (int f = 0; f < 4; ++f) {
// ... 205 lines not shown
        __syncthreads();
        if (t + (int)gridDim.x < total) fetch(t + gridDim.x);

#ifndef NIMG_E_NO_PAIR
        static_assert(E_TR == 8, "four waves x two adjacent rows");
        {
            const int r0 = 2 * wave;
            f32x4 acc2[2][5];
#pragma unroll
            for (int fq = 0; fq < 5; ++fq) {
                const int q = 16 * fq + nl;
                const int slot = (kg ^ (((q >> 3) & 1) << 1)) * 16;
                f32x4 a0 = {0.f, 0.f, 0.f, 0.f}, a1 = {0.f, 0.f, 0.f, 0.f};
#pragma unroll
                for (int j = 0; j < 6; ++j) {
                    const bf16x8 b = *reinterpret_cast<const bf16x8*>(sZ + ((r0 + 5 - j) * E_HC + q) * 64 + slot);
                    if (j < 5) a1 = __builtin_amdgcn_mfma_f32_16x16x32_bf16(wa[j], b, a1, 0, 0, 0);
                    if (j >= 1) a0 = __builtin_amdgcn_mfma_f32_16x16x32_bf16(wa[j - 1], b, a0, 0, 0, 0);
                }
                acc2[0][fq] = a0;
                acc2[1][fq] = a1;
            }
#pragma unroll
            for (int rr = 0; rr < 2; ++rr) {
#pragma unroll
                for (int fq = 0; fq < 5; ++fq) {
                    const int q = 16 * fq + nl;
                    if (q < E_HC) {
#pragma unroll
                        for (int reg = 0; reg < 4; ++reg) sP[(4 * kg + reg) * E_PS + q] = acc2[rr][fq][reg];
                    }
                }
                __builtin_amdgcn_wave_barrier();
                const int oy = y0 + r0 + rr;
                float o3[3] = {0.f, 0.f, 0.f};
#pragma unroll
                for (int kx = 0; kx < 5; ++kx)
#pragma unroll
                    for (int ci = 0; ci < 3; ++ci) o3[ci] += sP[(kx * 3 + ci) * E_PS + lane + 4 - kx];
                if (oy < H && x0 + lane < W) {
                    float* d = dc + ((long)(n * H + oy) * W + x0 + lane) * 3;
                    d[0] = o3[0]; d[1] = o3[1]; d[2] = o3[2];
                }
                __builtin_amdgcn_wave_barrier();
            }
        }
#else
        for (int r = wave; r < E_TR; r += 4) {
#pragma unroll
            for (int fq = 0; fq < 5; ++fq) {
                const int q = 16 * fq + nl;
                const int slot = (kg ^ (((q >> 3) & 1) << 1)) * 16;
                f32x4 acc = {0.f, 0.f, 0.f, 0.f};
#pragma unroll
                for (int ky = 0; ky < 5; ++ky) {
                    const bf16x8 b = *reinterpret_cast<const bf16x8*>(sZ + ((r + 4 - ky) * E_HC + q) * 64 + slot);
                    acc = __builtin_amdgcn_mfma_f32_16x16x32_bf16(wa[ky], b, acc, 0, 0, 0);
                }
                if (q < E_HC) {
#pragma unroll
                    for (int reg = 0; reg < 4; ++reg) sP[(4 * kg + reg) * E_PS + q] = acc[reg];
                }
            }
            __builtin_amdgcn_wave_barrier();
            const int oy = y0 + r;
            float o3[3] = {0.f, 0.f, 0.f};
#pragma unroll
            for (int kx = 0; kx < 5; ++kx)
#pragma unroll
                for (int ci = 0; ci < 3; ++ci) o3[ci] += sP[(kx * 3 + ci) * E_PS + lane + 4 - kx];
            if (oy < H && x0 + lane < W) {
                float* d = dc + ((long)(n * H + oy) * W + x0 + lane) * 3;
                d[0] = o3[0]; d[1] = o3[1]; d[2] = o3[2];
            }
            __builtin_amdgcn_wave_barrier();
        }
#endif
    }
}

constexpr int F1_WGS = 1024;

template <int TWD>
int launch_conv1_pool(const void* c4, const float* w, const float* bias, void* pooled, unsigned char* pidx, int n, int h,
                      int wd, float alpha, int out_bf16, hipStream_t s) {
    const int tiles_y = cdiv(h, 8), tiles_x = cdiv(wd, TWD);
    const long total = (long)n * tiles_y * tiles_x;
    static const int capmul = getenv("NIMG_CONV1_CAP") ? atoi(getenv("NIMG_CONV1_CAP")) : 0;
    const long cap = 256L * (capmul > 0 ? capmul : CONV1_WGS);
    const dim3 grid((unsigned)(total < cap ? total : cap));
    if (out_bf16)
        hipLaunchKernelGGL((conv1_pool_fwd_kernel<TWD, true>), grid, dim3(256), 0, s, c4, w, bias, pooled, pidx, n, h, wd, alpha,
                           tiles_y, tiles_x);
    else
        hipLaunchKernelGGL((conv1_pool_fwd_kernel<TWD, false>), grid, dim3(256), 0, s, c4, w, bias, pooled, pidx, n, h, wd,
                           alpha, tiles_y, tiles_x);
    NIMG_CHECK_LAUNCH();
    return NIMG_OK;
}


typedef float f32x4c __attribute__((ext_vector_type(4)));
typedef __bf16 bf16x8c __attribute__((ext_vector_type(8)));

template <int ABL>
__global__ __launch_bounds__(256) void conv5c3_mfma_kernel(const float* __restrict__ in, const float* __restrict__ w,
                                                           float* __restrict__ out, int N, int H, int W, int tiles_y) {
    constexpr int TR = 16, TC = 64, HR = TR + 4, HC = TC + 8;
    __shared__ __attribute__((aligned(16))) uint2 tile[HR * HC];
    __shared__ __attribute__((aligned(16))) float orow[4][TC * 3];
    const int tid = threadIdx.x, lane = tid & 63;
    const int wave = __builtin_amdgcn_readfirstlane(tid >> 6);
    int bid = xcd_order(blockIdx.x);
    const int tiles_x = W / TC;
    const int tx = bid % tiles_x;
    bid /= tiles_x;
    const int ty = bid % tiles_y, n = bid / tiles_y;
    const int y0 = ty * TR, x0 = tx * TC;
    constexpr int ITEMS = HR * (TC + 4), SQ = (ITEMS + 255) / 256;
    float sv[SQ][3];
    bool sok[SQ];
#pragma unroll
    for (int q = 0; q < SQ; ++q) {
        const int i = tid + 256 * q, r = i / (TC + 4), c = i % (TC + 4);
        const int gy = y0 - 2 + r, gx = x0 - 2 + c;
        sok[q] = !(ABL & 1) && i < ITEMS && (unsigned)gy < (unsigned)H && (unsigned)gx < (unsigned)W;
        const float* src = in + (sok[q] ? (((long)n * H + gy) * W + gx) * 3 : 0L);
        sv[q][0] = src[0]; sv[q][1] = src[1]; sv[q][2] = src[2];
    }
#pragma unroll
    for (int q = 0; q < SQ; ++q) {
        const int i = tid + 256 * q, r = i / (TC + 4), c = i % (TC + 4);
        if (i < ITEMS) {
            const __bf16 b0 = (__bf16)(sok[q] ? sv[q][0] : 0.f), b1 = (__bf16)(sok[q] ? sv[q][1] : 0.f), b2 = (__bf16)(sok[q] ? sv[q][2] : 0.f);
            tile[r * HC + c] = make_uint2((unsigned)__builtin_bit_cast(unsigned short, b0) | ((unsigned)__builtin_bit_cast(unsigned short, b1) << 16),
                                          (unsigned)__builtin_bit_cast(unsigned short, b2));
        }
    }
    __shared__ float sw[232];
    if (tid < 225) sw[tid] = w[tid];
    if (tid >= 225 && tid < 232) sw[tid] = 0.f;
    const int col = lane & 15, kg = lane >> 4;
    const int j = col / 3, co = col % 3;
    __syncthreads();
    bf16x8c bw[5];
#pragma unroll
    for (int wr = 0; wr < 5; ++wr)
#pragma unroll
        for (int e = 0; e < 8; ++e) {
            const int wc = 2 * kg + (e >> 2), ci = e & 3, kx = wc - j;
            const bool on = col < 12 && ci < 3 && kx >= 0 && kx < 5;
            const float v = sw[on ? ((wr * 5 + kx) * 3 + ci) * 3 + co : 225];
            bw[wr][e] = (__bf16)v;
        }
    const int g = lane & 15;
    const uint2* abase = tile + 4 * g + 2 * kg;
#pragma unroll
    for (int q = 0; q < TR / 4; ++q) {
        const int r = wave + 4 * q;
        f32x4c acc = {0.f, 0.f, 0.f, 0.f};
        if (!(ABL & 4))
#pragma unroll
        for (int wr = 0; wr < 5; ++wr) {
            const uint4 v = *reinterpret_cast<const uint4*>(abase + (r + wr) * HC);
            acc = __builtin_amdgcn_mfma_f32_16x16x32_bf16(*reinterpret_cast<const bf16x8c*>(&v), bw[wr], acc, 0, 0, 0);
        }
        __builtin_amdgcn_wave_barrier();
        if (col < 12) {
#pragma unroll
            for (int e = 0; e < 4; ++e) orow[wave][12 * (4 * kg + e) + col] = acc[e];
        }
        __builtin_amdgcn_wave_barrier();
        const int gy = y0 + r;
        if (!(ABL & 2) && gy < H && lane < 48)
            *reinterpret_cast<float4*>(out + (((long)n * H + gy) * W + x0) * 3 + 4 * lane) =
                *reinterpret_cast<const float4*>(&orow[wave][4 * lane]);
    }
}

}

extern "C" {

int nimg_conv1_pool_fwd_c4(const void* c4, const float* w, const float* bias, void* pooled, unsigned char* pool_idx, int n,
                           int h, int wd, float alpha, int out_bf16, void* stream) {
    if (n == 0) return NIMG_OK;
    if (!c4 || !w || !pooled || n < 0 || h < 2 || wd < 2 || (h & 1) || (wd & 1) || !(alpha > 0.f && alpha <= 1.f))
        return NIMG_ERR_ARG;
    const long per_image = (long)h * wd * 8;
    if (per_image > 0x7fffffffL) return NIMG_ERR_ARG;
    const int chunk = (int)(0x7fffffffL / per_image);
    const size_t esz = out_bf16 ? 2 : 4;
    for (int n0 = 0; n0 < n; n0 += chunk) {
        const int nn = n - n0 < chunk ? n - n0 : chunk;
        const long px0 = (long)n0 * h * wd, pp0 = (long)n0 * (h / 2) * (wd / 2) * 32;
        const void* src = (const char*)c4 + px0 * 8;
        void* dst = (char*)pooled + pp0 * esz;
        unsigned char* di = pool_idx ? pool_idx + (pp0 >> 2) : nullptr;
        const int rc = wd > 96 ? launch_conv1_pool<256>(src, w, bias, dst, di, nn, h, wd, alpha, out_bf16, (hipStream_t)stream)
                               : launch_conv1_pool<64>(src, w, bias, dst, di, nn, h, wd, alpha, out_bf16, (hipStream_t)stream);
        if (rc != NIMG_OK) return rc;
    }
    return NIMG_OK;
}

int nimg_conv1_dgrad_pooled(const void* g, const unsigned char* pool_idx, const float* w, float* dc, int n, int h, int wd,
                            int g_bf16, void* stream) {
    if (n == 0) return NIMG_OK;
    if (!g || !pool_idx || !w || !dc || n < 0 || h < 2 || wd < 2 || (h & 1) || (wd & 1)) return NIMG_ERR_ARG;
    if ((long)n * (h / 2) * (wd / 2) * 32 * (g_bf16 ? 2 : 4) > 0x7fffffffL) return NIMG_ERR_ARG;
    const int tiles_y = cdiv(h, E_TR), tiles_x = cdiv(wd, E_TW);
    const long total = (long)n * tiles_y * tiles_x;
    const dim3 grid((unsigned)(total < 512 ? total : 512));
    if (g_bf16)
        hipLaunchKernelGGL((conv1_dgrad_pooled_kernel<true>), grid, dim3(256), 0, (hipStream_t)stream, g, pool_idx, w, dc, n, h, wd,
                           tiles_y, tiles_x);
    else
        hipLaunchKernelGGL((conv1_dgrad_pooled_kernel<false>), grid, dim3(256), 0, (hipStream_t)stream, g, pool_idx, w, dc, n, h,
                           wd, tiles_y, tiles_x);
    NIMG_CHECK_LAUNCH();
    return NIMG_OK;
}

size_t nimg_conv1_wgrad_c4_workspace_bytes(void) { return (size_t)F1_WGS * (F_DW + 32) * sizeof(float); }

int nimg_conv1_wgrad_c4(const void* c4, const void* g, const unsigned char* pool_idx, float* dw, float* db, int n, int h, int wd,
                        int g_bf16, int accumulate, void* workspace, size_t workspace_bytes, void* stream) {
    if (n == 0) return NIMG_OK;
    if (!c4 || !g || !pool_idx || !dw || !workspace || n < 0 || h < 2 || wd < 2 || (h & 1) || (wd & 1)) return NIMG_ERR_ARG;
    if (workspace_bytes < nimg_conv1_wgrad_c4_workspace_bytes()) return NIMG_ERR_WORKSPACE;
    if ((long)n * h * wd * 8 > 0x7fffffffL) return NIMG_ERR_ARG;
    const int tiles_y = cdiv(h, F_TR), tiles_x = cdiv(wd, F_TW);
    const long total = (long)n * tiles_y * tiles_x;
    const int wgs = (int)(total < F1_WGS ? total : F1_WGS), per = cdiv(total, wgs);
    const int used = cdiv(total, per);
    float* dws = (float*)workspace;
    float* dbs = dws + (size_t)F1_WGS * F_DW;
    if (g_bf16)
        hipLaunchKernelGGL((conv1_wgrad_pooled_kernel<true>), dim3(used), dim3(256), 0, (hipStream_t)stream, c4, g, pool_idx, dws,
                           db ? dbs : nullptr, n, h, wd, tiles_y, tiles_x, per);
    else
        hipLaunchKernelGGL((conv1_wgrad_pooled_kernel<false>), dim3(used), dim3(256), 0, (hipStream_t)stream, c4, g, pool_idx,
                           dws, db ? dbs : nullptr, n, h, wd, tiles_y, tiles_x, per);
    NIMG_CHECK_LAUNCH();
    launch_reduce2(dws, dw, F_DW, used, db ? dbs : nullptr, db, 32, used, accumulate, (hipStream_t)stream);
    NIMG_CHECK_LAUNCH();
    return NIMG_OK;
}

int nimg_cconv3(const float* in, const float* w, float* out_f32, void* out_c4, int n, int h, int wd, int pad_mode,
                void* stream) {
    if (n == 0) return NIMG_OK;
    if (!in || !w || (!out_f32 && !out_c4) || n < 0 || h < 1 || wd < 1 || pad_mode < 0 || pad_mode > 2) return NIMG_ERR_ARG;
    if (pad_mode != 0 && (h < 2 || wd < 2)) return NIMG_ERR_ARG;
    const long per_image = (long)h * wd * 12;
    if (per_image > 0x7fffffffL) return NIMG_ERR_ARG;
    const int chunk = (int)(0x7fffffffL / per_image);
    for (int n0 = 0; n0 < n; n0 += chunk) {
        CConvParams p;
        const long px0 = (long)n0 * h * wd;
        p.in = in + px0 * 3; p.w = w; p.out_f32 = out_f32 ? out_f32 + px0 * 3 : nullptr;
        p.out_c4 = out_c4 ? (uint2*)out_c4 + px0 : nullptr;
        p.N = n - n0 < chunk ? n - n0 : chunk; p.H = h; p.W = wd; p.pad_mode = pad_mode; p.tiles_y = p.tiles_x = 0;
        static const int variant = getenv("NIMG_CCONV_VARIANT") ? atoi(getenv("NIMG_CCONV_VARIANT")) : 0;
        const int rc = wd <= 96 ? launch_cconv<16, 1>(p, (hipStream_t)stream)
                     : variant == 1 ? launch_cconv<64, 1>(p, (hipStream_t)stream)
                     : variant == 2 ? launch_cconv<64, 4>(p, (hipStream_t)stream)
                     : variant == 3 ? launch_cconv<32, 2>(p, (hipStream_t)stream)
                                    : launch_cconv<64, 2>(p, (hipStream_t)stream);
        if (rc != NIMG_OK) return rc;
    }
    return NIMG_OK;
}

int nimg_conv5c3_bf16(const float* in, const float* w, float* out, int n, int h, int wd, void* stream) {
    if (n == 0) return NIMG_OK;
    if (!in || !w || !out || n < 0 || h < 1 || wd < 64 || (wd & 63)) return NIMG_ERR_ARG;
    const int tiles_y = (h + 15) / 16;
    const long blocks = (long)n * tiles_y * (wd / 64);
    if (blocks > 0x7fffffffL) return NIMG_ERR_ARG;
    static const int abl = getenv("NIMG_C5C3_ABL") ? atoi(getenv("NIMG_C5C3_ABL")) : 0;
    auto kern = abl == 1 ? conv5c3_mfma_kernel<1> : abl == 2 ? conv5c3_mfma_kernel<2> : abl == 4 ? conv5c3_mfma_kernel<4>
              : abl == 3 ? conv5c3_mfma_kernel<3> : conv5c3_mfma_kernel<0>;
// ... 18 lines not shown
```

neural-imaging_amd/models/forensics.py:

```python
import os
from collections import OrderedDict

import numpy as np

import torch

from .. import ops, parallel
from ..device import DeviceArray, to_device
from ..helpers import paramspec
from .layers import ConstrainedConv2D, Conv2D
from .tfmodel import ParamStore, TFModel, glorot_uniform_


LATE_PARAMS = os.environ.get('NIMG_NO_LATE_PARAMS') is None
LATE_MIN_IMAGES = int(os.environ.get('NIMG_LATE_MIN_IMAGES', '160'))
DEFER_MASK = int(os.environ.get('NIMG_PIPELINE_FAN_MASK', '255'))
LATE_MASK = int(os.environ.get('NIMG_LATE_MASK', '255'))


class FAN(TFModel):

    def __init__(self, n_classes, patch_size=None, n_filters=32, n_fscale=2, n_convolutions=4, kernel=5, dropout=0.0,
                 use_gap=True, n_dense=0, activation='leaky_relu', device=None, seed=4321):
        super().__init__(device=device)
        self._h = paramspec.ParamSpec({
            'n_classes': (7, int, (2, 256)),
            'n_filters': (32, int, (4, 128)),
            'n_fscale': (2, float, (0.25, 4)),
            'n_convolutions': (4, int, (1, 32)),
            'kernel': (5, int, (3, 11)),
            'dropout': (0, float, (0, 1)),
            'use_gap': (False, bool, None),
            'n_dense': (2, int, (0, 16)),
            'activation': ('leaky_relu', str, set(ops.ACTIVATIONS)),
        })
        params = locals()
        self._h.update(**{k: params[k] for k in self._h.keys()})
        if not 0 <= float(dropout) < 1:
            raise ValueError('dropout rate must be in [0, 1)')
        self._dropout_gen, self._dropout_seed = None, int(seed) + 17
        self.dropout_masks = None
        if not use_gap and patch_size is None:
            raise ValueError('the Flatten head (use_gap=False) needs a fixed patch_size')
        self.patch_size = patch_size
        self.x = _Shape((None, patch_size, patch_size, 3))
        self.y = _Shape((None, n_classes))

        self._constrained = ConstrainedConv2D('constrained')
        self._convs = []
        cin, nf = 3, n_filters
        for i in range(self._h.n_convolutions):
            self._convs.append(Conv2D('conv{}'.format(i + 1), self._h.kernel, cin, nf, self._h.activation,
                                      mask_activation=self._h.activation))
            cin, nf = nf, int(nf * self._h.n_fscale)
        nf = int(nf // self._h.n_fscale)
        self._conv1x1 = Conv2D('conv1x1', 1, cin, nf, self._h.activation, mask_activation=self._h.activation)
        self._generic_act = self._h.activation != 'leaky_relu'
        self._use_gap = bool(use_gap)
        feat = nf if use_gap else nf * (patch_size // 2 ** self._h.n_convolutions) ** 2
        self._hidden = []
        for i in range(self._h.n_dense):
            nf = int(nf // self._h.n_fscale)
            self._hidden.append(Conv2D('dense' if i == 0 else 'dense_{}'.format(i), 1, feat, nf, self._h.activation))
            feat = nf
        self._cls = 'dense' if self._h.n_dense == 0 else 'dense_{}'.format(self._h.n_dense)
        self._n_features = feat
        specs = self._constrained.specs()
        for c in self._convs:
            specs += c.specs()
        specs += self._conv1x1.specs()
        for d in self._hidden:
            specs += [(d.name + '/kernel', (d.cin, d.cout)), (d.name + '/bias', (d.cout,))]
        specs += [(self._cls + '/kernel', (feat, n_classes)), (self._cls + '/bias', (n_classes,))]
        self._model = ParamStore(specs, self.device)
        gen = torch.Generator().manual_seed(seed)
        self._constrained.init(self._model)
        for c in self._convs:
            c.init(self._model, gen)
        self._conv1x1.init(self._model, gen)
        for d in self._hidden + [None]:
            name, fi, fo = (d.name, d.cin, d.cout) if d is not None else (self._cls, feat, n_classes)
            k = torch.empty((fi, fo), dtype=torch.float32)
            glorot_uniform_(k, fi, fo, gen)
            self._model.p[name + '/kernel'].copy_(k)
            self._model.p[name + '/bias'].zero_()
        self.learning_rate = 1e-3
        self.loss = self._loss

    def reset_performance_stats(self):
        self.performance = {'loss': {'training': [], 'validation': []}, 'accuracy': {'validation': []},
                            'confusion': []}

    def forward(self, x, labels=None, training=False, loss_scale=None):
        self._model.refresh_images()
        P = self._model
        t = OrderedDict()
        t['x'] = x
        c1 = self._convs[0]
        front = ops.front_end_ok(c1.cin, c1.cout, c1.ks, x.shape[1], x.shape[2], n=x.shape[0] if training else None) and \
            c1.activation == 'leaky_relu'
        net, nf = self._constrained.forward(P, x, c4_only=front)
        t['constrained'], t['nf'] = net, nf
        for i, c in enumerate(self._convs):
            if i == 0 and front:
                nxt = self._convs[1] if len(self._convs) > 1 else self._conv1x1
                as_bf16 = ops.STORE_BF16 and nxt.cout >= 8
                net, idx = ops.conv1_pool_c4(net, P.p[c.name + '/kernel'], P.p[c.name + '/bias'], want_idx=training,
                                             out_bf16=as_bf16)
                t['idx1'], t['front'] = idx, True
            elif c.can_pool(net):
                nxt = self._convs[i + 1] if i + 1 < len(self._convs) else self._conv1x1
                as_bf16 = ops.COMPUTE == 'bf16' and ops.STORE_BF16 and c.cout % 8 == 0 and nxt.cout >= 8
                net, idx = c.forward_pool(P, net, want_idx=training, out_bf16=as_bf16)
                t['idx{}'.format(i + 1)] = idx
            else:
                a = c.forward(P, net)
                t['conv{}'.format(i + 1)] = a
                net = ops.maxpool2(a)
            t['pool{}'.format(i + 1)] = net
        n = x.shape[0]
        ls = (1.0 / n) if loss_scale is None else loss_scale
        c5 = self._conv1x1
        if self._use_gap and not self._hidden and not self._generic_act and c5.cin == c5.cout and ops.head_fused_ok(net, c5.cout):
            gap, mask, mask_p = ops.head_fwd(net, P.p[c5.name + '/kernel'], P.p[c5.name + '/bias'], want_mask=training)
            t['head_mask_p'] = mask_p
            probs, loss_per, dlogits = ops.fan_dense_fwd(gap, P.p[self._cls + '/kernel'], P.p[self._cls + '/bias'], labels, ls)
            t['head_mask'], t['gap'], t['probs'], t['loss_per'], t['dlogits'], t['loss_scale'] = mask, gap, probs, loss_per, dlogits, ls
            return probs, (t if training else None)
        a = self._conv1x1.forward(P, net)
        t['conv1x1'] = a
        head_in = a
        if self._hidden or not self._use_gap:
            if self._use_gap:
                if a.shape[1] != a.shape[2]:
                    raise ValueError('the hidden-Dense head pools square feature maps')
                head_in = ops.avgpool(a, a.shape[1])
            else:
                head_in = a.reshape(n, 1, 1, -1)
            t['feat'] = head_in
            rate = float(self._h.dropout)
            for li, d in enumerate(self._hidden):
                w4 = P.p[d.name + '/kernel'].view(1, 1, d.cin, d.cout)
                if self._generic_act:
                    head_in = ops.conv2d(head_in, w4, P.p[d.name + '/bias'])
                    ops.activation(head_in, self._h.activation, out=head_in)
                else:
                    head_in = ops.conv2d(head_in, w4, P.p[d.name + '/bias'], act='leaky_relu')
                t[d.name] = head_in
                if training and rate > 0:
                    if self.dropout_masks is not None:
                        keep = self.dropout_masks[li].to(device=x.device, dtype=torch.uint8).reshape(head_in.shape).contiguous()
                    else:
                        if self._dropout_gen is None:
                            self._dropout_gen = parallel.rank_generator(self._dropout_seed, x.device)
                        keep = (torch.rand(head_in.shape, device=x.device, generator=self._dropout_gen) >= rate).to(torch.uint8)
                    head_in = ops.mask_scale(head_in, keep, 1.0 / (1.0 - rate))
                    t[d.name + '/keep'], t[d.name + '/dropped'] = keep, head_in
            if training:
                self.dropout_masks = None
        gap, probs, loss_per, dlogits = ops.fan_head_fwd(head_in, P.p[self._cls + '/kernel'], P.p[self._cls + '/bias'],
                                                         labels, ls)
        t['head_in'] = head_in
        t['gap'], t['probs'], t['loss_per'], t['dlogits'], t['loss_scale'] = gap, probs, loss_per, dlogits, ls
        return probs, (t if training else None)

    def backward(self, t, need_input_grad=False, join=True, defer=None):
        late = [] if ((LATE_PARAMS or defer is not None) and not join) else None
        self._defer = defer if late is not None else None
        def params(fn, layer=0):
            if late is None or not (LATE_MASK >> layer) & 1:
                fn()
            elif self._defer is not None and (DEFER_MASK >> layer) & 1:
                self._defer.append(fn)
            else:
                late.append(fn)
        P = self._model
        hw = lambda a: (a.shape[1], a.shape[2])
        nconv = len(self._convs)
        fused = lambda i: i >= 1 and t.get('idx{}'.format(i)) is not None
        pooled_path = lambda i: fused(i) and not fused(i - 1) and ops.pooled_backward_ok(
            self._convs[i - 1].cin, self._convs[i - 1].cout, self._convs[i - 1].ks)
        g_bf16 = lambda i: (ops.COMPUTE == 'bf16' and ops.STORE_BF16 and fused(i) and self._convs[i - 1].cout % 8 == 0 and
                            (pooled_path(i) or self._convs[i - 1].cin % 8 == 0))
        if 'head_mask' in t:
            d_pool, loss = self._fused_head_backward(t)
        else:
            d_pool, loss = self._head_backward(t, fused, g_bf16)
        return self._conv_backward(t, d_pool, loss, fused, g_bf16, params, late, need_input_grad, join)

    def _fused_head_backward(self, t):
        P, c5 = self._model, self._conv1x1
        pool = t['pool{}'.format(len(self._convs))]
        wd = P.p[self._cls + '/kernel']
        loss = ops.fan_dense_bwd(t['gap'], t['dlogits'], t['loss_per'], t['loss_scale'], P.g[self._cls + '/kernel'],
                                 P.g[self._cls + '/bias'])
        dw = P.g[c5.name + '/kernel']
        with ops.side_stream(pool, t['head_mask_p'], t['dlogits'], wd, key=dw.data_ptr()):
            ops.head_wgrad(pool, t['head_mask_p'], t['dlogits'], wd, dw.view(dw.shape[2], dw.shape[3]), P.g[c5.name + '/bias'])
        d_pool = ops.head_dgrad(t['head_mask'], t['dlogits'], wd, P.p[c5.name + '/kernel'],
                                pool if t.get('idx{}'.format(len(self._convs))) is not None else None, pool.shape)
        return d_pool, loss

    def _head_backward(self, t, fused, g_bf16):
        P = self._model
        hw = lambda a: (a.shape[1], a.shape[2])
        a = t['conv1x1']
        gen = self._generic_act
        act_bwd = (lambda g, y: ops.activation_bwd(g, y, self._h.activation, out=g)) if gen else ops.lrelu_bwd
        dz, loss = ops.fan_head_bwd(t['head_in'], t['gap'], P.p[self._cls + '/kernel'], t['dlogits'], t['loss_per'],
                                    t['loss_scale'], P.g[self._cls + '/kernel'], P.g[self._cls + '/bias'],
                                    alpha=1.0 if gen else None)
        if gen and not ('feat' in t and self._hidden):
            dz = act_bwd(dz.reshape(a.shape), a)
        if 'feat' in t:
            keep_scale = 1.0 / (1.0 - float(self._h.dropout))
            for i in range(len(self._hidden) - 1, -1, -1):
                d = self._hidden[i]
                if d.name + '/keep' in t:
                    dz = ops.mask_scale(dz.reshape(t[d.name].shape), t[d.name + '/keep'], keep_scale)
                if gen:
                    dz = act_bwd(dz.reshape(t[d.name].shape), t[d.name])
                prev = self._hidden[i - 1].name if i > 0 else None
                inp = t.get(prev + '/dropped', t[prev]) if i > 0 else t['feat']
                ops.conv2d_wgrad(inp, dz, 1, dw=P.g[d.name + '/kernel'].view(1, 1, d.cin, d.cout),
                                 db=P.g[d.name + '/bias'])
                w4 = P.p[d.name + '/kernel'].view(1, 1, d.cin, d.cout)
                dz = ops.conv2d_dgrad(dz, w4, (1, 1), act_mask=t[prev] if (i > 0 and not gen) else None)
            if self._hidden:
                if self._use_gap:
                    dz = act_bwd(ops.avgpool_bwd(dz, a.shape[1]), a)
                else:
                    dz = act_bwd(dz.reshape(a.shape).contiguous(), a)
            else:
                dz = dz.reshape(a.shape)
        nconv = len(self._convs)
        pool = t['pool{}'.format(nconv)]
        self._conv1x1.backward_params(P, pool, dz)
        d_pool = self._conv1x1.backward_input(P, dz, hw(pool), act_mask=pool if fused(nconv) else None,
                                              out_bf16=g_bf16(nconv))
        return d_pool, loss

    def _conv_backward(self, t, d_pool, loss, fused, g_bf16, params, late, need_input_grad, join):
        P = self._model
        hw = lambda a: (a.shape[1], a.shape[2])
        gen = self._generic_act
        act_bwd = (lambda g, y: ops.activation_bwd(g, y, self._h.activation, out=g)) if gen else ops.lrelu_bwd
        nconv = len(self._convs)
        for i in range(nconv, 0, -1):
            conv = self._convs[i - 1]
            inp = t['pool{}'.format(i - 1)] if i > 1 else t['constrained']
            prev_mask = inp if fused(i - 1) else None
            if i == 1 and t.get('front'):
                params(lambda inp=inp, g=d_pool, i=i, conv=conv: ops.conv1_wgrad_c4(
                    inp, g, t['idx{}'.format(i)], dw=P.g[conv.name + '/kernel'], db=P.g[conv.name + '/bias'], side=True), i)
                d_pool = ops.conv1_dgrad_pooled(d_pool, t['idx{}'.format(i)], P.p[conv.name + '/kernel'])
                continue
            if fused(i) and ops.pooled_backward_ok(conv.cin, conv.cout, conv.ks) and prev_mask is None:
                params(lambda inp=inp, g=d_pool, i=i, conv=conv: ops.conv2d_wgrad_pooled(
                    inp, g, t['idx{}'.format(i)], conv.ks, dw=P.g[conv.name + '/kernel'], db=P.g[conv.name + '/bias'],
                    side=True), i)
                d_pool = ops.conv2d_dgrad_pooled(d_pool, t['idx{}'.format(i)], P.p[conv.name + '/kernel'])
                continue
            if fused(i) and ops.unpool_fold_ok(inp, d_pool, conv.cin, conv.cout, conv.ks):
                params(lambda inp=inp, g=d_pool, i=i, conv=conv: ops.conv2d_wgrad_unpool(
                    inp, g, t['idx{}'.format(i)], conv.ks, dw=P.g[conv.name + '/kernel'], db=P.g[conv.name + '/bias'], side=True), i)
                d_pool = ops.conv2d_dgrad_unpool(d_pool, t['idx{}'.format(i)], P.p[conv.name + '/kernel'], act_mask=prev_mask,
                                                 out_bf16=g_bf16(i - 1))
                continue
            if fused(i):
                as_bf16 = ops.COMPUTE == 'bf16' and ops.STORE_BF16 and conv.cout % 8 == 0 and conv.cin % 8 == 0
                dz = ops.maxpool2_unpool(d_pool, t['idx{}'.format(i)], None, apply_mask=False, out_bf16=as_bf16)
            else:
                dz = ops.maxpool2_bwd(d_pool, t['conv{}'.format(i)], None, apply_mask=not gen)
                if gen:
                    dz = act_bwd(dz, t['conv{}'.format(i)])
            params(lambda conv=conv, inp=inp, dz=dz: conv.backward_params(P, inp, dz), i)
            d_pool = conv.backward_input(P, dz, hw(inp), act_mask=prev_mask, out_bf16=g_bf16(i - 1))
        params(lambda g=d_pool: self._constrained.backward_params(P, t['x'], g))
        dx = self._constrained.backward_input(t['nf'], d_pool) if need_input_grad else None
        self._defer = None
        with ops.one_fork():
            for fn in late or ():
                fn()
        if join:
            ops.join_side_stream()
            P.grads_pending = False
        else:
            P.grads_pending = True
        return loss, dx

    def _loss(self, labels, probs):
        p = np.clip(np.asarray(probs, np.float64), 1e-7, 1 - 1e-7)
        lab = np.asarray(labels).astype(np.int64)
        return float(np.mean(np.log(p.sum(axis=1)) - np.log(p[np.arange(len(lab)), lab])))

    def process(self, batch_x, training=False):
        return DeviceArray(self.forward(to_device(batch_x, self.device))[0])

    def process_and_decide(self, batch_x, with_confidence=False):
        probs = self.process(batch_x).numpy()
        if with_confidence:
            return probs.argmax(axis=1), probs.max(axis=1)
        return probs.argmax(axis=1)

    def training_step(self, batch_x, target_labels, learning_rate=None):
        x = to_device(batch_x, self.device)
        labels = torch.as_tensor(np.asarray(target_labels), dtype=torch.int32).to(self.device)
        _, ctx = self.forward(x, labels, training=True)
        loss, _ = self.backward(ctx, need_input_grad=False)
        world = parallel.sync_gradients(self._model.flat_grad)
        if learning_rate is not None:
            self.learning_rate = learning_rate
        self._model.adam(self.learning_rate, grad_scale=1.0 / world)
        return DeviceArray(loss)

    def summary(self):
        return '{kernel}x{kernel} CNN: 1+{conv}+1 conv layers {gap}+ {fc} fc layers [{params:,} parameters]'.format(
            kernel=self._h.kernel, conv=self._h.n_convolutions, fc=self._h.n_dense,
            gap='+ (GAP) ' if self._h.use_gap else '', params=self.count_parameters())


class _Shape(object):
    def __init__(self, shape):
        self.shape = tuple(shape)
```

neural-imaging_amd/models/layers.py:

```python
import numpy as np
import torch

from .. import ops
from ..helpers import kernels as hk


FUSED_ACTIVATIONS = (None, 'leaky_relu')


def act_forward(y, activation):
    if isinstance(y, tuple):
        raise RuntimeError('a bf16 copy cannot be combined with activation {}'.format(activation))
    return ops.activation(y, activation, out=y)


class Conv2D(object):

    def __init__(self, name, ks, cin, cout, activation=None, stride=1, cin2=0, mask_activation='leaky_relu'):
        self.name, self.ks, self.cin, self.cin2, self.cout = name, ks, cin, cin2, cout
        self.activation, self.stride = activation, stride
        self.mask_activation = mask_activation

    def specs(self):
        return [(self.name + '/kernel', (self.ks, self.ks, self.cin + self.cin2, self.cout)),
                (self.name + '/bias', (self.cout,))]

    def init(self, store, gen):
        from .tfmodel import glorot_uniform_
        rf = self.ks * self.ks
        k = torch.empty(store.p[self.name + '/kernel'].shape, dtype=torch.float32)
        glorot_uniform_(k, (self.cin + self.cin2) * rf, self.cout * rf, gen)
        store.p[self.name + '/kernel'].copy_(k)
        store.p[self.name + '/bias'].zero_()

    def forward(self, store, x, x2=None, out_bf16=False, residual=None, bf16_copy=False, d2s_out=False, copy_lrelu=False,
                s2d_out=False):
        fused = self.activation in FUSED_ACTIVATIONS
        y = ops.conv2d(x, store.p[self.name + '/kernel'], store.p[self.name + '/bias'], x2=x2,
                       stride=self.stride, act=self.activation if fused else None, out_bf16=out_bf16, residual=residual,
                       bf16_copy=bf16_copy, d2s_out=d2s_out, copy_lrelu=copy_lrelu, s2d_out=s2d_out)
        return y if fused else act_forward(y, self.activation)

    def can_pool(self, x):
        return self.stride == 1 and self.cin2 == 0 and self.ks in (3, 5) and self.cout % 4 == 0 and \
            x.shape[1] % 2 == 0 and x.shape[2] % 2 == 0 and self.activation == 'leaky_relu'

    def forward_pool(self, store, x, want_idx=True, out_bf16=False):
        return ops.conv2d_pool(x, store.p[self.name + '/kernel'], store.p[self.name + '/bias'], act=self.activation,
                               want_idx=want_idx, out_bf16=out_bf16)

    def forward_and_pool(self, store, x, out_bf16=False):
        w = store.p[self.name + '/kernel']
        if out_bf16 and self.can_pool(x) and ops.conv2d_and_pool_ok(x, w):
            return ops.conv2d_and_pool(x, w, store.p[self.name + '/bias'], act=self.activation)
        y = self.forward(store, x, out_bf16=out_bf16)
        return y, ops.maxpool2(y)

    def backward_params(self, store, x, dz, x2=None):
        ops.conv2d_wgrad(x, dz, self.ks, x2=x2, stride=self.stride, dw=store.g[self.name + '/kernel'],
                         db=store.g[self.name + '/bias'], side=True)

    def s2d_chain_ok(self, in_hw):
        return self.stride == 2 and self.ks == 5 and self.cin2 == 0 and self.cin % 8 == 0 and self.cout % 8 == 0 and \
            ops.COMPUTE == 'bf16' and ops.STORE_BF16 and ops.D2S_EPILOGUE and \
            ops.s2d_conv_ok(self.ks, self.stride, in_hw[0], in_hw[1], self.cin)

    def forward_s2d(self, store, xs, bf16_copy=False, copy_lrelu=False):
        w3 = ops.s2d_conv_weights(store.p[self.name + '/kernel'])
        fused = self.activation in FUSED_ACTIVATIONS
        y = ops.conv2d(xs, w3, store.p[self.name + '/bias'], act=self.activation if fused else None, bf16_copy=bf16_copy,
                       copy_lrelu=copy_lrelu)
        return y if fused else act_forward(y, self.activation)

    def backward_params_s2d(self, store, xs, dz):
        with ops.side_stream(xs, dz, key=store.g[self.name + '/kernel'].data_ptr()):
            dw3 = ops.conv2d_wgrad(xs, dz, 3, db=store.g[self.name + '/bias'])
            ops.s2d_conv_weights_bwd(dw3, store.g[self.name + '/kernel'])

    def backward_input(self, store, dz, in_hw, act_mask=None, out=None, out2=None, out_bf16=False, residual=None,
                       bf16_copy=False, s2d_out=False, mask_s2d=False, mask_activation=None):
        kind = mask_activation or self.mask_activation
        if act_mask is not None and kind not in FUSED_ACTIVATIONS:
            if out2 is not None or mask_s2d:
                raise NotImplementedError('split / space-to-depth-stored masks with activation {}'.format(kind))
            d = self.backward_input(store, dz, in_hw, out=out)
            ops.activation_bwd(d, act_mask, kind, out=d)
            if residual is not None:
                ops.add(residual, d, out=d)
            if s2d_out:
                d = ops.d2s_clip_bwd(d, 1.0)
            return (d, None) if bf16_copy else d
        if self.stride == 2:
            d = ops.conv2d_dgrad_strided2(dz, store.p[self.name + '/kernel'], in_hw, act_mask=act_mask, out_bf16=out_bf16,
                                          mask_s2d=mask_s2d)
            d = d if residual is None else ops.add(residual, d, out=d)
            return (d, None) if bf16_copy else d
        return ops.conv2d_dgrad(dz, store.p[self.name + '/kernel'], in_hw, stride=self.stride, act_mask=act_mask,
                                out=out, out2=out2, out_bf16=out_bf16, residual=residual, bf16_copy=bf16_copy,
                                s2d_out=s2d_out)


class Conv5x5Stride2Image(Conv2D):

    def s2d_ok(self, x):
        return ops.s2d_conv_ok(self.ks, self.stride, x.shape[1], x.shape[2], self.cin) and self.cin2 == 0 and 4 * self.cin <= 16

    def forward_image(self, store, x, a, b, s2d_out=False):
        if not self.s2d_ok(x):
            if s2d_out:
                raise RuntimeError('s2d_out needs the space-to-depth form of the layer')
            x0 = ops.affine(x, a, b)
            return self.forward(store, x0), x0
        xs = ops.s2d2_affine(x, a, b, cp=16)
        w3 = ops.s2d_conv_weights(store.p[self.name + '/kernel'], cp=16)
        fused = self.activation in FUSED_ACTIVATIONS
        y = ops.conv2d(xs, w3, store.p[self.name + '/bias'], act=self.activation if fused else None, s2d_out=s2d_out,
                       out_bf16=s2d_out)
        return (y if fused else act_forward(y, self.activation)), xs

    def backward_params_image(self, store, ctx, dz):
        if ctx.dtype != torch.bfloat16:
            return self.backward_params(store, ctx, dz)
        with ops.side_stream(ctx, dz, key=store.g[self.name + '/kernel'].data_ptr()):
            dw3 = ops.conv2d_wgrad(ctx, dz, 3, db=store.g[self.name + '/bias'])
            ops.s2d_conv_weights_bwd(dw3, store.g[self.name + '/kernel'])

    def backward_input_image(self, store, dz, in_hw, a):
        return ops.conv2d_dgrad_strided2(dz, store.p[self.name + '/kernel'], in_hw, scale=a)


class Conv2DTranspose2x2(object):

# ... 55 lines not shown
```

neural-imaging_amd/ops.py:

```python
import math
import os

import numpy as np
import torch

from . import _lib

LRELU_ALPHA = 0.2

COMPUTE = 'f32'


STORE_BF16 = True


def set_compute(mode):
    global COMPUTE
    if mode not in ('f32', 'bf16'):
        raise ValueError('compute mode must be f32 or bf16')
    COMPUTE = mode


_WB_REGISTRY = {}

# ... 705 lines not shown
        entry = (ctypes.c_char * int(_lib.load().nimg_reduce_entry_bytes()))()
    ws = _SIDE['ws'][k].claim(need, device)
    name, pre = ('nimg_conv2d_wgrad_bf16_chained', (_CHAIN.get(k),)) if carrier == 'chain' else ('nimg_conv2d_wgrad_bf16_deferred', ())
    _lib.call(name, *operands, _p(ws), ws.numel(), flags, *pre, entry, _stream())
    if carrier == 'defer':
        st['n'] += 1
    elif carrier == 'chain':
        _CHAIN[k] = entry
    else:
        _reduce_behind(k, entry, device)


def bias_grad(dz, db=None, accumulate=False, side=False):
    if side and _SIDE['enabled'] and db is not None:
        with _on_side_stream(dz, key=db.data_ptr()):
            return bias_grad(dz, db=db, accumulate=accumulate, side=False)
    _f32(db)
    _fb(dz)
    cout = dz.shape[-1]
    npix = dz.numel() // cout
    if db is None:
        db = torch.empty((cout,), dtype=torch.float32, device=dz.device)
    need = _lib.load().nimg_bias_grad_workspace_bytes(npix, cout)
    ws = _ws_current(dz.device).get(need, dz.device)
    _lib.call('nimg_bias_grad_ex', _p(dz), _p(db), npix, cout, 1 if accumulate else 0, _p(ws), ws.numel(),
              BF16_DZ if _is_bf16(dz) else 0, _stream())
    return db


def convt2x2(x, w, bias, out_bf16=False):
    _f32(w, bias)
    _fb(x)
    n, h, wd, cin = x.shape
    cout = w.shape[2]
    y = torch.empty((n, 2 * h, 2 * wd, cout), dtype=torch.bfloat16 if out_bf16 else torch.float32, device=x.device)
    if COMPUTE == 'bf16' and cin % 8 == 0 and cout >= 8:
        wb = weights_bf16(w, 1)
        _lib.call('nimg_convt2x2_fwd_bf16_ex', _p(x), _p(wb), _p(bias), _p(y), n, h, wd, cin, cout,
                  (BF16_IN if _is_bf16(x) else 0) | (BF16_OUT if out_bf16 else 0), _stream())
        return y
    if _is_bf16(x) or out_bf16:
        raise RuntimeError('bf16-stored tensor reached a float32 transposed-convolution path')
    _lib.call('nimg_convt2x2_fwd', _p(x), _p(w), _p(bias), _p(y), n, h, wd, cin, cout, _stream())
    return y


def convt2x2_dgrad(dy, w, act_mask=None, out_bf16=False):
    n, h2, w2, _ = dy.shape
    return conv2d(dy, w, None, stride=2, pads=(0, 0), out_hw=(h2 // 2, w2 // 2), act_mask=act_mask, out_bf16=out_bf16)


def convt2x2_wgrad(x, dy, dw=None, side=False):
    return conv2d_wgrad(dy, x, 2, stride=2, pads=(0, 0), dw=dw, side=side)


def maxpool2(x):
    _fb(x)
    n, h, w, c = x.shape
    y = torch.empty((n, h // 2, w // 2, c), dtype=x.dtype, device=x.device)
    if _is_bf16(x):
        _lib.call('nimg_maxpool2_fwd_bf16', _p(x), _p(y), n, h, w, c, _stream())
        return y
    _lib.call('nimg_maxpool2_fwd', _p(x), _p(y), n, h, w, c, _stream())
    return y


def maxpool2_bwd(dp, yact, add=None, apply_mask=True, out=None, alpha=None):
    a = LRELU_ALPHA if alpha is None else float(alpha)
    _fb(dp, yact, add, out)
    n, h, w, c = yact.shape
    dz = torch.empty_like(yact) if out is None else out
    if _is_bf16(yact):
        if any(t is not None and not _is_bf16(t) for t in (dp, add, dz)):
            raise RuntimeError('maxpool2_bwd on a bf16-stored activation needs bf16-stored gradients')
        _lib.call('nimg_maxpool2_bwd_bf16', _p(dp), _p(yact), _p(add), _p(dz), n, h, w, c, 1 if apply_mask else 0,
                  a, _stream())
        return dz
    _f32(dp, add, dz)
    _lib.call('nimg_maxpool2_bwd', _p(dp), _p(yact), _p(add), _p(dz), n, h, w, c, 1 if apply_mask else 0,
              a, _stream())
    return dz


def conv2d_pool(x, w, bias=None, act='leaky_relu', want_idx=True, out_bf16=False):
    _f32(w, bias)
    _fb(x)
    n, h, wd, cin = x.shape
    ks, cout = w.shape[0], w.shape[3]
    if w.shape[2] != cin or (h & 1) or (wd & 1) or (cout & 3) or ks not in (3, 5):
        raise ValueError('conv2d_pool: unsupported shape')
    bf16_path = COMPUTE == 'bf16' and (cin in (3, 4) or cin % 8 == 0)
    if (out_bf16 or _is_bf16(x)) and not bf16_path:
        raise RuntimeError('bf16 storage needs the throughput-mode convolution path')
    pooled = torch.empty((n, h // 2, wd // 2, cout), dtype=torch.bfloat16 if out_bf16 else torch.float32, device=x.device)
    idx = torch.empty((n, h // 2, wd // 2, cout), dtype=torch.uint8, device=x.device) if want_idx else None
    a = 1 if act == 'leaky_relu' else 0
    if bf16_path:
        wb = None if cin in (3, 4) else weights_bf16(w, 0)
        flags = (BF16_IN if _is_bf16(x) else 0) | (BF16_OUT if out_bf16 else 0)
        _lib.call('nimg_conv2d_pool_fwd_bf16_ex', _p(x), cin, _p(w), _p(wb), _p(bias), _p(pooled), _p(idx), cout, n, h, wd,
                  ks, a, LRELU_ALPHA, flags, _stream())
    else:
        _lib.call('nimg_conv2d_pool_fwd', _p(x), cin, _p(w), _p(bias), _p(pooled), _p(idx), cout, n, h, wd, ks, a,
                  LRELU_ALPHA, _stream())
    return pooled, idx


POOL_ALSO = _os.environ.get('NIMG_NO_POOL_ALSO') is None


_EPI8 = {}


def _epi8_built(entry):
    if entry not in _EPI8:
        lib = _lib.load()
        if entry == 'nimg_conv2d_fwd_pool_also_bf16':
            rc = lib.nimg_conv2d_fwd_pool_also_bf16(None, 8, None, None, None, None, None, 8, 0, 16, 16, 1, LRELU_ALPHA, None)
        else:
            rc = lib.nimg_conv2d_dgrad_unpool_out_bf16(None, 8, None, None, None, None, 8, 0, 16, 16, 1, LRELU_ALPHA, None)
        _EPI8[entry] = rc == 0
    return _EPI8[entry]


def conv2d_and_pool_ok(x, w):
    n, h, wd, cin = x.shape
    return POOL_ALSO and _epi8_built('nimg_conv2d_fwd_pool_also_bf16') and COMPUTE == 'bf16' and _is_bf16(x) and w.shape[0] == 3 and w.shape[1] == 3 and cin % 8 == 0 and \
        w.shape[3] % 8 == 0 and h % 2 == 0 and wd % 2 == 0 and h > 8 and wd > 8


def conv2d_and_pool(x, w, bias=None, act='leaky_relu'):
    _f32(w, bias)
    if not conv2d_and_pool_ok(x, w):
        raise ValueError('conv2d_and_pool: unsupported shape / mode')
    n, h, wd, cin = x.shape
    cout = w.shape[3]
    y = torch.empty((n, h, wd, cout), dtype=torch.bfloat16, device=x.device)
    pooled = torch.empty((n, h // 2, wd // 2, cout), dtype=torch.bfloat16, device=x.device)
    if wd == 128 and rows_conv_ok(x, None, 3, 1, cout, (h, wd), (1, 1), 0, y, None, None, act):
        _lib.call('nimg_conv3_rows_bf16', _p(x), cin, None, 0, _p(weights_bf16(w, 0)), _p(bias), None, _p(y), None, _p(pooled), n, h,
                  wd, cout, 1 if act == 'leaky_relu' else 0, LRELU_ALPHA, 0, _stream())
        return y, pooled
    _lib.call('nimg_conv2d_fwd_pool_also_bf16', _p(x), cin, _p(weights_bf16(w, 0)), _p(bias), _p(y), _p(pooled), None, cout,
              n, h, wd, 1 if act == 'leaky_relu' else 0, LRELU_ALPHA, _stream())
    return y, pooled


DGRAD_UNPOOL_OUT = _os.environ.get('NIMG_NO_DGRAD_UNPOOL_OUT') is None


def conv2d_dgrad_unpool_out_ok(dz, w, act, skip):
    return DGRAD_UNPOOL_OUT and _epi8_built('nimg_conv2d_dgrad_unpool_out_bf16') and COMPUTE == 'bf16' and _is_bf16(dz) and _is_bf16(act) and (skip is None or _is_bf16(skip)) and \
        w.shape[0] == 3 and w.shape[1] == 3 and w.shape[2] % 8 == 0 and w.shape[3] % 8 == 0 and \
        act.shape[1] == 2 * dz.shape[1] and act.shape[2] == 2 * dz.shape[2] and act.shape[3] == w.shape[2]


def conv2d_dgrad_unpool_out(dz, w, act, skip=None, apply_mask=True, out=None):
    if not conv2d_dgrad_unpool_out_ok(dz, w, act, skip):
        raise ValueError('conv2d_dgrad_unpool_out: unsupported shape / mode')
    _f32(w)
    n, h, wd, cz = dz.shape
    cin = w.shape[2]
    if out is None:
        out = torch.empty_like(act)
    _lib.call('nimg_conv2d_dgrad_unpool_out_bf16', _p(dz), cz, _p(weights_bf16(w, 1)), _p(act), _p(skip), _p(out), cin, n, h, wd,
              1 if apply_mask else 0, LRELU_ALPHA, _stream())
    return out


def maxpool2_unpool(dp, idx, pooled, apply_mask=True, out=None, out_bf16=False, alpha=None):
    _f32(pooled)
    _fb(dp, out)
    _chk(idx)
    n, ho, wo, c = dp.shape
    if out is None:
        out = torch.empty((n, 2 * ho, 2 * wo, c), dtype=torch.bfloat16 if out_bf16 else torch.float32, device=dp.device)
    flags = (BF16_IN if _is_bf16(dp) else 0) | (BF16_OUT if _is_bf16(out) else 0)
    _lib.call('nimg_maxpool2_unpool_ex', _p(dp), _p(idx), _p(pooled), _p(out), n, ho, wo, c, 1 if apply_mask else 0,
              LRELU_ALPHA if alpha is None else float(alpha), flags, _stream())
    return out


UNPOOL_FOLD = _os.environ.get('NIMG_NO_UNPOOL_FOLD') is None


def unpool_fold_ok(x, g, cin, cout, ks):
    small = max(x.numel(), g.numel()) * 2 < (1 << 31) - 65536 and 25 * cin * cout * 2 < (1 << 31) - 65536
    return UNPOOL_FOLD and COMPUTE == 'bf16' and ks == 5 and _is_bf16(x) and _is_bf16(g) and cin % 32 == 0 and \
        cout % 64 == 0 and x.shape[1] % 2 == 0 and x.shape[2] % 2 == 0 and small and \
        _os.environ.get('NIMG_NO_BUFFER_LOADS') is None


def conv2d_dgrad_unpool(g, idx, w, act_mask=None, out_bf16=False):
    _f32(w)
    _fb(g, act_mask)
    _chk(idx)
    n, hp, wp, cz = g.shape
    ks, ci = w.shape[0], w.shape[2]
    out = torch.empty((n, 2 * hp, 2 * wp, ci), dtype=torch.bfloat16 if out_bf16 else torch.float32, device=g.device)
    flags = (BF16_OUT if out_bf16 else 0) | (BF16_MASK if _is_bf16(act_mask) else 0)
    if SPARSE_DGRAD and ks == 5 and ci % 32 == 0 and cz % 8 == 0 and _is_bf16(g) and g.numel() * 2 < (1 << 31) - 65536:
        img = torch.empty(int(_lib.load().nimg_conv5_dgrad_sparse_image_bytes(ci, cz)), dtype=torch.uint8, device=g.device)
        _lib.call('nimg_conv5_dgrad_sparse_weights', _p(w), _p(img), ci, cz, _stream())
        _lib.call('nimg_conv5_dgrad_sparse', _p(g), _p(idx), cz, _p(img), _p(out), ci, _p(act_mask), n, 2 * hp, 2 * wp, LRELU_ALPHA,
                  flags, _stream())
        return out
    wb = weights_bf16(w, 1)
    _lib.call('nimg_conv2d_fwd_bf16_unpool', _p(g), _p(idx), cz, _p(wb), None, _p(out), ci, _p(act_mask), n, 2 * hp, 2 * wp, ks,
              ks - 1 - (ks - 1) // 2, ks - 1 - (ks - 1) // 2, 2 * hp, 2 * wp, 0, LRELU_ALPHA, flags, _stream())
    return out


def conv2d_wgrad_unpool(x, g, idx, ks, dw, db=None, side=False, _defer_k=None):
    if side and _SIDE['enabled'] and dw is not None:
        ctx = _on_side_stream(x, g, idx, key=dw.data_ptr())
        with ctx:
            return conv2d_wgrad_unpool(x, g, idx, ks, dw, db=db, side=False, _defer_k=ctx.k)
    _f32(dw, db)
    _fb(x, g)
    _chk(idx)
    n, h, wd, cin = x.shape
    cout = g.shape[3]
    need = _lib.load().nimg_conv2d_wgrad_bf16_workspace_bytes(cin, cout, ks, ks, n, h, wd)
    carrier = _reduce_carrier() if _defer_k is not None and ks == 5 and h % 2 == 0 and wd % 2 == 0 else None
    if carrier:
        _wgrad_carried(_defer_k, carrier, x.device, need, BF16_IN | BF16_DZ, _p(x), cin, None, 0, _p(g), _p(idx), cout, _p(dw), _p(db),
                       n, h, wd, ks, 1, 2, 2, 0, h, wd)
        return dw
    ws = _ws_current(x.device).get(need, x.device)
    _lib.call('nimg_conv2d_wgrad_bf16_unpool', _p(x), cin, _p(g), _p(idx), cout, _p(dw), _p(db), n, h, wd, ks, 0, _p(ws),
              ws.numel(), _stream())
    return dw


def pooled_backward_ok(cin, cout, ks):
    return COMPUTE == 'bf16' and cin == 3 and cout == 32 and ks == 5


def conv2d_wgrad_pooled(x, g, idx, ks, dw=None, db=None, side=False):
    if side and _SIDE['enabled'] and dw is not None:
        with _on_side_stream(x, g, idx, key=dw.data_ptr()):
            return conv2d_wgrad_pooled(x, g, idx, ks, dw=dw, db=db, side=False)
    _f32(x, dw, db)
    _fb(g)
    _chk(idx)
    n, h, wd, cin = x.shape
    cout = g.shape[3]
    if dw is None:
        dw = torch.empty((ks, ks, cin, cout), dtype=torch.float32, device=x.device)
    need = _lib.load().nimg_conv2d_wgrad_bf16_workspace_bytes(cin, cout, ks, ks, n, h, wd)
    ws = _ws_current(x.device).get(need, x.device)
    _lib.call('nimg_conv2d_wgrad_pooled_bf16_ex', _p(x), cin, _p(g), _p(idx), cout, _p(dw), _p(db), n, h, wd, ks, 0, _p(ws),
              ws.numel(), BF16_DZ if _is_bf16(g) else 0, _stream())
    return dw


def conv2d_dgrad_pooled(g, idx, w, out=None):
    _f32(w, out)
    _fb(g)
    _chk(idx)
    n, hp, wp, cz = g.shape
    ks, ci = w.shape[0], w.shape[2]
    if out is None:
        out = torch.empty((n, 2 * hp, 2 * wp, ci), dtype=torch.float32, device=g.device)
    _lib.call('nimg_conv2d_dgrad_fewin_pooled_bf16_ex', _p(g), _p(idx), _p(w), _p(out), ci, cz, n, 2 * hp, 2 * wp, ks,
              BF16_DZ if _is_bf16(g) else 0, _stream())
    return out


def d2s_clip(x, scale=1.0, shift=0.0, clip=True, out=None):
    _f32(x, out)
    n, h, w, c4 = x.shape
    if out is not None and tuple(out.shape) != (n, 2 * h, 2 * w, c4 // 4):
        raise ValueError('d2s_clip: output shape mismatch')
    y = torch.empty((n, 2 * h, 2 * w, c4 // 4), dtype=torch.float32, device=x.device) if out is None else out
    _lib.call('nimg_d2s_clip_fwd', _p(x), _p(y), n, h, w, c4 // 4, float(scale), float(shift), 1 if clip else 0,
              _stream())
    return y


def d2s_clip_bwd(dy, scale=1.0):
    _f32(dy)
    n, h2, w2, c = dy.shape
    dx = torch.empty((n, h2 // 2, w2 // 2, 4 * c), dtype=torch.float32, device=dy.device)
    _lib.call('nimg_d2s_clip_bwd', _p(dy), _p(dx), n, h2 // 2, w2 // 2, c, float(scale), _stream())
    return dx


def lrelu_bwd(dy, yact, out=None, alpha=None):
    _f32(dy, yact, out)
# ... 193 lines not shown
def adam_lr_t(lr, step, beta1=0.9, beta2=0.999):
    lr, beta1, beta2 = (float(np.float32(v)) for v in (lr, beta1, beta2))
    return lr * math.sqrt(1.0 - math.pow(beta2, float(int(step)))) / (1.0 - math.pow(beta1, float(int(step))))


def adam_step(params, grads, m, v, lr, step, beta1=0.9, beta2=0.999, eps=1e-7, grad_scale=1.0, skip_flag=None,
              lr_t_dev=None):
    join_side_stream()
    _f32(params, grads, m, v, lr_t_dev)
    if lr_t_dev is not None:
        _lib.call('nimg_adam_step_dev', _p(params), _p(grads), _p(m), _p(v), params.numel(), _p(lr_t_dev), float(beta1),
                  float(beta2), float(eps), float(grad_scale), _p(skip_flag), _stream())
        return
    _lib.call('nimg_adam_step', _p(params), _p(grads), _p(m), _p(v), params.numel(), float(lr), float(beta1),
              float(beta2), float(eps), int(step), float(grad_scale), _p(skip_flag), _stream())


def int_fill(t, value=0):
    _chk(t)
    if t.dtype != torch.int32 or not t.is_contiguous():
        raise ValueError('int_fill: contiguous int32 tensor expected')
    _lib.call('nimg_int_words', _p(t), None, t.numel(), int(value), 0, _stream())
    return t


def int_max_(dst, src):
    _chk(dst, src)
    if dst.dtype != torch.int32 or src.dtype != torch.int32 or dst.numel() != src.numel():
        raise ValueError('int_max_: two int32 tensors of one size expected')
    _lib.call('nimg_int_words', _p(dst), _p(src), dst.numel(), 0, 1, _stream())
    return dst


def float_fill(t, value):
    _f32(t)
    _lib.call('nimg_float_fill', _p(t), t.numel(), float(value), _stream())
    return t


def nan_flag(g, flag):
    join_side_stream()
    _f32(g)
    _lib.call('nimg_nan_flag', _p(g), g.numel(), _p(flag), _stream())


def constrained_kernel(kernel, strength=100.0):
    _f32(kernel)
    nf = torch.empty_like(kernel)
    _lib.call('nimg_constrained_kernel_fwd', _p(kernel), _p(nf), kernel.shape[0], kernel.shape[2], float(strength),
              _stream())
    return nf


def constrained_kernel_bwd(kernel, dnf, dk, strength=100.0):
    _f32(kernel, dnf, dk)
    _lib.call('nimg_constrained_kernel_bwd', _p(kernel), _p(dnf), _p(dk), kernel.shape[0], kernel.shape[2],
              float(strength), _stream())
    return dk


def cconv3(x, w, pad_mode=1, out=None, want_f32=True, want_c4=False):
    _f32(x, w, out)
    n, h, wd, c = x.shape
    if c != 3 or tuple(w.shape) != (5, 5, 3, 3):
        raise ValueError('cconv3: (N,H,W,3) input and a (5,5,3,3) kernel expected')
    y = (torch.empty_like(x) if out is None else out) if want_f32 else None
    c4 = torch.empty((n, h, wd, 4), dtype=torch.bfloat16, device=x.device) if want_c4 else None
    _lib.call('nimg_cconv3', _p(x), _p(w), _p(y), _p(c4), n, h, wd, int(pad_mode), _stream())
    return y, c4


FRONT_END = _os.environ.get('NIMG_OLD_FRONTEND') is None
CCONV_DGRAD_MFMA = _os.environ.get('NIMG_NO_CCONV_DGRAD_MFMA') is None
S2D_CONV = _os.environ.get('NIMG_NO_S2D_CONV') is None
SPARSE_DGRAD = _os.environ.get('NIMG_SPARSE_DGRAD') is not None


def front_end_ok(cin, cout, ks, h, w, n=None):
    small = n is None or n * h * w * 16 < (1 << 31) - 65536
    return FRONT_END and COMPUTE == 'bf16' and cin == 3 and cout == 32 and ks == 5 and h % 2 == 0 and w % 2 == 0 and \
        h >= 4 and w >= 4 and small


def conv1_pool_c4(c4, w, bias, act='leaky_relu', want_idx=True, out_bf16=True):
    _f32(w, bias)
    _chk(c4)
    n, h, wd, c = c4.shape
    if c4.dtype != torch.bfloat16 or c != 4 or tuple(w.shape) != (5, 5, 3, 32) or (h & 1) or (wd & 1):
        raise ValueError('conv1_pool_c4: (N,H,W,4) bf16 pixels, a (5,5,3,32) kernel and even sizes expected')
    pooled = torch.empty((n, h // 2, wd // 2, 32), dtype=torch.bfloat16 if out_bf16 else torch.float32, device=c4.device)
    idx = torch.empty((n, h // 2, wd // 2, 8), dtype=torch.uint8, device=c4.device) if want_idx else None
    _lib.call('nimg_conv1_pool_fwd_c4', _p(c4), _p(w), _p(bias), _p(pooled), _p(idx), n, h, wd,
              LRELU_ALPHA if act == 'leaky_relu' else 1.0, 1 if out_bf16 else 0, _stream())
    return pooled, idx


def conv1_wgrad_c4(c4, g, idx, dw=None, db=None, accumulate=False, side=False):
    if side and _SIDE['enabled'] and dw is not None:
        with _on_side_stream(c4, g, idx, key=dw.data_ptr()):
            return conv1_wgrad_c4(c4, g, idx, dw=dw, db=db, accumulate=accumulate, side=False)
    _f32(dw, db)
    _fb(g)
    _chk(c4, idx)
    n, h, wd, _ = c4.shape
    if c4.dtype != torch.bfloat16 or tuple(g.shape) != (n, h // 2, wd // 2, 32) or tuple(idx.shape) != (n, h // 2, wd // 2, 8) or \
            idx.dtype != torch.uint8:
        raise ValueError('conv1_wgrad_c4: (N,H,W,4) bf16 pixels, a (N,H/2,W/2,32) gradient and (N,H/2,W/2,8) arg-max codes expected')
    if dw is None:
        dw = torch.empty((5, 5, 3, 32), dtype=torch.float32, device=c4.device)
    need = _lib.load().nimg_conv1_wgrad_c4_workspace_bytes()
    ws = _ws_current(c4.device).get(need, c4.device)
    _lib.call('nimg_conv1_wgrad_c4', _p(c4), _p(g), _p(idx), _p(dw), _p(db), n, h, wd, 1 if _is_bf16(g) else 0,
              1 if accumulate else 0, _p(ws), ws.numel(), _stream())
    return dw


def conv1_dgrad_pooled(g, idx, w, out=None):
    _f32(w, out)
    _fb(g)
    _chk(idx)
    n, hp, wp, c = g.shape
    if c != 32 or tuple(w.shape) != (5, 5, 3, 32) or tuple(idx.shape) != (n, hp, wp, 8) or idx.dtype != torch.uint8:
        raise ValueError('conv1_dgrad_pooled: a (N,H/2,W/2,32) gradient, (N,H/2,W/2,8) arg-max codes and a (5,5,3,32) kernel expected')
    if out is None:
        out = torch.empty((n, 2 * hp, 2 * wp, 3), dtype=torch.float32, device=g.device)
    _lib.call('nimg_conv1_dgrad_pooled', _p(g), _p(idx), _p(w), _p(out), n, 2 * hp, 2 * wp, 1 if _is_bf16(g) else 0, _stream())
    return out


def cconv3_dgrad(dy, nf):
    _f32(dy, nf)
    n, h, wd, _ = dy.shape
    if COMPUTE == 'bf16' and wd % 64 == 0 and CCONV_DGRAD_MFMA:
        dx = torch.empty_like(dy)
        _lib.call('nimg_conv5c3_bf16', _p(dy), _p(flip_weights(nf)), _p(dx), n, h, wd, _stream())
    else:
        dx, _ = cconv3(dy, flip_weights(nf), pad_mode=0)
    _lib.call('nimg_cconv3_dgrad_border', _p(dy), _p(nf), _p(dx), n, h, wd, _stream())
    return dx


def fold_pad(dpad, pad, pad_mode):
    _f32(dpad)
    n, hp, wp, c = dpad.shape
    dx = torch.empty((n, hp - 2 * pad, wp - 2 * pad, c), dtype=torch.float32, device=dpad.device)
    _lib.call('nimg_fold_pad', _p(dpad), _p(dx), n, hp - 2 * pad, wp - 2 * pad, c, pad, pad_mode, _stream())
    return dx


def gaussian_fwd(x, gk25, out=None, clip=True, want_mask=True):
    _f32(x, gk25, out)
    n, h, w, _ = x.shape
    y = torch.empty_like(x) if out is None else out
    mask = torch.empty((n, h, w), dtype=torch.uint8, device=x.device) if want_mask else None
    _lib.call('nimg_gaussian_fwd', _p(x), _p(y), _p(mask), _p(gk25), n, h, w, 1 if clip else 0, _stream())
    return y, mask


def gaussian_bwd(dy, mask, gk25):
    _f32(dy, gk25)
    n, h, w, _ = dy.shape
    dx = torch.empty_like(dy)
    _lib.call('nimg_gaussian_bwd', _p(dy), _p(mask), _p(dx), _p(gk25), n, h, w, _stream())
    return dx


def dwfilter_fwd(x, taps, k, pad_mode, out=None, clip=True, want_mask=True):
    _f32(x, taps, out)
    n, h, w, _ = x.shape
    if taps.numel() != k * k:
        raise ValueError('taps: k*k floats')
    y = torch.empty_like(x) if out is None else out
    mask = torch.empty((n, h, w), dtype=torch.uint8, device=x.device) if want_mask else None
    _lib.call('nimg_dwfilter_fwd', _p(x), _p(y), _p(mask), _p(taps), int(k), PAD_MODES[pad_mode], n, h, w,
              1 if clip else 0, _stream())
    return y, mask

# ... 877 lines not shown
```

Measured before the change: 8291 patches/s.

## Emit packed activation sign bits in pooled conv forward for backward masking

Pooled conv forward kernels (front-end conv1 and the ring conv5 path) now also write a 1-bit-per-channel sign plane of the pooled bf16 output. The backward unpool dgrad then reads these bits to apply the leaky-ReLU derivative instead of loading the full bf16 activation mask. This cuts the backward read of the mask by about 16x, at the cost of an extra small write in the forward pass and more plumbing. It only applies to specific shapes (ring tn=64/128 path, bf16 in and out).

```diff
diff --git a/include/nimg.h b/include/nimg.h
--- a/include/nimg.h
+++ b/include/nimg.h
@@ -379,6 +379,17 @@
                              int restart_interval, int subseq_bits, int16_t* coef, uint32_t* status, uint32_t* rounds, void* workspace,
                              size_t workspace_bytes, void* stream);
 
+int nimg_conv1_pool_fwd_c4_sign(const void* c4, const float* w, const float* bias, void* pooled, unsigned char* pool_idx,
+                                unsigned char* pool_sign, int n, int h, int wd, float alpha, int out_bf16, void* stream);
+int nimg_conv2d_pool_sign_ok(int cin, int cout, int n, int h, int wd, int ks, int flags);
+int nimg_conv2d_pool_fwd_bf16_sign(const float* in, int cin, const float* w, const void* wb, const float* bias,
+                                   float* pool_out, unsigned char* pool_idx, unsigned char* pool_sign, int cout, int n, int h,
+                                   int wd, int ks, int act, float alpha, int flags, void* stream);
+int nimg_conv2d_fwd_bf16_unpool_sign(const void* in_pooled, const unsigned char* in_idx, int c1, const void* wb, const float* bias,
+                                     float* out1, int o1, const float* act_mask, const unsigned char* act_sign, int n, int h, int wd,
+                                     int ks, int pad_t, int pad_l, int hout, int wout, int act, float alpha, int flags,
+                                     void* stream);
+
 #ifdef __cplusplus
 }
 #endif
diff --git a/neural-imaging_amd/_lib.py b/neural-imaging_amd/_lib.py
--- a/neural-imaging_amd/_lib.py
+++ b/neural-imaging_amd/_lib.py
@@ -201,6 +201,12 @@
     'nimg_jpeg_decode_restart': (c_int, [P, P, P, c_int, c_int, c_int, c_int, c_int, c_int, c_int, P, P, P, P, c_size_t, P]),
     'nimg_msssim_workspace_bytes': (c_size_t, [c_int, c_int, c_int, c_int]),
     'nimg_msssim': (c_int, [P, P, c_int, c_int, c_int, c_int, c_float, P, P, P, c_size_t, P]),
+    'nimg_conv1_pool_fwd_c4_sign': (c_int, [P, P, P, P, P, P, c_int, c_int, c_int, c_float, c_int, P]),
+    'nimg_conv2d_pool_sign_ok': (c_int, [c_int, c_int, c_int, c_int, c_int, c_int, c_int]),
+    'nimg_conv2d_pool_fwd_bf16_sign': (c_int, [P, c_int, P, P, P, P, P, P, c_int, c_int, c_int, c_int, c_int, c_int, c_float,
+                                               c_int, P]),
+    'nimg_conv2d_fwd_bf16_unpool_sign': (c_int, [P, P, c_int, P, P, P, c_int, P, P, c_int, c_int, c_int, c_int, c_int, c_int, c_int,
+                                                 c_int, c_int, c_float, c_int, P]),
 }
 
 ERRORS = {-1: 'NIMG_ERR_ARG (invalid argument / unsupported configuration)',
diff --git a/neural-imaging_amd/csrc/common.h b/neural-imaging_amd/csrc/common.h
--- a/neural-imaging_amd/csrc/common.h
+++ b/neural-imaging_amd/csrc/common.h
@@ -14,6 +14,19 @@
 constexpr int WAVE = 64;
 
 __device__ __forceinline__ float lrelu(float v, float alpha) { return v > 0.0f ? v : alpha * v; }
+
+typedef unsigned short nimg_u16x2 __attribute__((ext_vector_type(2)));
+__device__ __forceinline__ unsigned bf16x2_positive(unsigned packed) {
+    const nimg_u16x2 one = {1, 1}, inf = {0x7F80, 0x7F80};
+    const nimg_u16x2 u = __builtin_bit_cast(nimg_u16x2, packed) - one;
+    return __builtin_bit_cast(unsigned, __builtin_elementwise_min(__builtin_elementwise_sub_sat(inf, u), one));
+}
+__device__ __forceinline__ unsigned sign_bits_interleave(unsigned x) {
+    x = (x | (x << 4)) & 0x0F0F0F0Fu;
+    x = (x | (x << 2)) & 0x33333333u;
+    x = (x | (x << 1)) & 0x55555555u;
+    return (x | (x >> 15)) & 0xFFFFu;
+}
 
 __device__ __forceinline__ float wave_sum(float v) {
 #pragma unroll
diff --git a/neural-imaging_amd/csrc/conv_bf16.h b/neural-imaging_amd/csrc/conv_bf16.h
--- a/neural-imaging_amd/csrc/conv_bf16.h
+++ b/neural-imaging_amd/csrc/conv_bf16.h
@@ -23,6 +23,8 @@
     const unsigned char* in_idx;
     const float* res;
     float* out1b;
+    unsigned char* pool_sign = nullptr;
+    const unsigned char* act_sign = nullptr;
 };
 
 namespace {
@@ -295,3 +297,4 @@
 int conv_bf16_dispatch(const ConvArgsB& a, hipStream_t s);
 template <int KS, bool INB>
 int conv_bf16_launch_16x16(const ConvArgsB& a, bool tn32, hipStream_t s);
+int conv_bf16_pool_ring_tn(const ConvArgsB& a, bool tn32);
diff --git a/neural-imaging_amd/csrc/conv_bf16.hip b/neural-imaging_amd/csrc/conv_bf16.hip
--- a/neural-imaging_amd/csrc/conv_bf16.hip
+++ b/neural-imaging_amd/csrc/conv_bf16.hip
@@ -102,7 +102,7 @@
                          int ks, int stride, int pad_t, int pad_l, int pad_mode, int hout, int wout, int act,
                          float alpha, int flags, void* stream, const unsigned char* in_idx = nullptr,
                          const float* res = nullptr, void* out1b = nullptr, float* pool_out = nullptr,
-                         unsigned char* pool_idx = nullptr) {
+                         unsigned char* pool_idx = nullptr, const unsigned char* act_sign = nullptr) {
     if (n == 0) return NIMG_OK;
     if (!in1 || !wb || !out1 || c1 <= 0 || c2 < 0 || o1 <= 0 || o2 < 0 || n < 0 || h <= 0 || wd <= 0) return NIMG_ERR_ARG;
     if ((c2 > 0 && !in2) || (o2 > 0 && !out2) || hout <= 0 || wout <= 0 || pad_t < 0 || pad_l < 0) return NIMG_ERR_ARG;
@@ -122,6 +122,8 @@
     if (in_idx && (!(flags & NIMG_BF16_IN) || stride != 1 || ks != 5 || (h & 1) || (wd & 1) || pad_mode != 0)) return NIMG_ERR_ARG;
     if ((flags & (NIMG_BF16_OUT | NIMG_BF16_MASK)) && ((o1 & 3) || (o2 & 3))) return NIMG_ERR_ARG;
     if ((flags & NIMG_BF16_MASK) && o2 != 0) return NIMG_ERR_ARG;
+    if (act_sign && (!act_mask || !(flags & NIMG_BF16_MASK) || !(flags & NIMG_BF16_OUT) || (o1 & 7) || o2 != 0)) return NIMG_ERR_ARG;
+    p.act_sign = act_sign;
     if ((flags & NIMG_D2S_OUT) && (ks != 3 || stride != 1 || o2 != 0 || (o1 & 15) || in_idx)) return NIMG_ERR_ARG;
     if ((flags & NIMG_S2D_OUT) && (ks != 3 || stride != 1 || o2 != 0 || (o1 & 3) || in_idx || (hout & 1) || (wout & 1) ||
                                    (flags & NIMG_D2S_OUT)))
@@ -196,9 +198,18 @@
 int nimg_conv2d_fwd_bf16_unpool(const void* in_pooled, const unsigned char* in_idx, int c1, const void* wb, const float* bias,
                                 float* out1, int o1, const float* act_mask, int n, int h, int wd, int ks, int pad_t, int pad_l,
                                 int hout, int wout, int act, float alpha, int flags, void* stream) {
+    return nimg_conv2d_fwd_bf16_unpool_sign(in_pooled, in_idx, c1, wb, bias, out1, o1, act_mask, nullptr, n, h, wd, ks, pad_t, pad_l,
+                                            hout, wout, act, alpha, flags, stream);
+}
+
+int nimg_conv2d_fwd_bf16_unpool_sign(const void* in_pooled, const unsigned char* in_idx, int c1, const void* wb, const float* bias,
+                                     float* out1, int o1, const float* act_mask, const unsigned char* act_sign, int n, int h, int wd,
+                                     int ks, int pad_t, int pad_l, int hout, int wout, int act, float alpha, int flags,
+                                     void* stream) {
     if (!in_idx) return NIMG_ERR_ARG;
     return conv2d_fwd_bf16_impl((const float*)in_pooled, c1, nullptr, 0, wb, bias, out1, o1, nullptr, 0, act_mask, n, h, wd, ks, 1,
-                                pad_t, pad_l, 0, hout, wout, act, alpha, flags | NIMG_BF16_IN, stream, in_idx);
+                                pad_t, pad_l, 0, hout, wout, act, alpha, flags | NIMG_BF16_IN, stream, in_idx, nullptr, nullptr,
+                                nullptr, nullptr, act_sign);
 }
 
 int nimg_convt2x2_fwd_bf16(const float* x, const void* wb, const float* bias, float* y, int n, int h, int wd, int cin,
diff --git a/neural-imaging_amd/csrc/conv_bf16_k5b.hip b/neural-imaging_amd/csrc/conv_bf16_k5b.hip
--- a/neural-imaging_amd/csrc/conv_bf16_k5b.hip
+++ b/neural-imaging_amd/csrc/conv_bf16_k5b.hip
@@ -2,3 +2,5 @@
 
 template int conv_bf16_dispatch<5, 1, true>(const ConvArgsB&, hipStream_t);
 template int conv_bf16_launch_16x16<5, true>(const ConvArgsB&, bool, hipStream_t);
+
+int conv_bf16_pool_ring_tn(const ConvArgsB& a, bool tn32) { return tn32 ? 0 : conv5_ring_tn(ConvParamsB{a}); }
diff --git a/neural-imaging_amd/csrc/conv_bf16_packed.hip b/neural-imaging_amd/csrc/conv_bf16_packed.hip
--- a/neural-imaging_amd/csrc/conv_bf16_packed.hip
+++ b/neural-imaging_amd/csrc/conv_bf16_packed.hip
@@ -585,10 +585,37 @@
 int nimg_conv2d_pool_fwd_bf16_ex(const float* in, int cin, const float* w, const void* wb, const float* bias,
                                  float* pool_out, unsigned char* pool_idx, int cout, int n, int h, int wd, int ks,
                                  int act, float alpha, int flags, void* stream) {
+    return nimg_conv2d_pool_fwd_bf16_sign(in, cin, w, wb, bias, pool_out, pool_idx, nullptr, cout, n, h, wd, ks, act, alpha, flags,
+                                          stream);
+}
+
+static bool pool_fwd_params(ConvParamsB& p, int cin, int cout, int n, int h, int wd, int ks, int act, float alpha, int flags) {
+    p.in2 = nullptr; p.out1 = nullptr; p.out2 = nullptr;
+    p.act1 = nullptr; p.pool_idx = nullptr; p.convt = 0; p.flags = flags; p.in_idx = nullptr; p.res = nullptr;
+    p.out1b = nullptr;
+    p.C1 = cin; p.C2 = 0; p.O1 = cout; p.O2 = 0; p.CinP = (cin + 15) / 16 * 16;
+    p.N = n; p.H = h; p.W = wd; p.Hout = h; p.Wout = wd; p.pad_t = p.pad_l = (ks - 1) / 2;
+    p.tiles_y = p.tiles_x = 0; p.act = act; p.pad_mode = 0; p.alpha = alpha;
+    return cout <= 32 || (long)cdiv(cout, 64) * cdiv(h, 16) * cdiv(wd, 16) * n < 384;
+}
+
+int nimg_conv2d_pool_sign_ok(int cin, int cout, int n, int h, int wd, int ks, int flags) {
+    if (cin <= 0 || cout <= 0 || n <= 0 || h <= 0 || wd <= 0 || (h & 1) || (wd & 1) || ks != 5 || (cin % 8) || (cout & 7)) return 0;
+    if ((flags & (NIMG_BF16_IN | NIMG_BF16_OUT)) != (NIMG_BF16_IN | NIMG_BF16_OUT)) return 0;
+    ConvParamsB p;
+    p.in1 = nullptr; p.wb = nullptr; p.bias = nullptr; p.pool_out = nullptr;
+    const bool tn32 = pool_fwd_params(p, cin, cout, n, h, wd, ks, 1, 0.f, flags);
+    return conv_bf16_pool_ring_tn(p, tn32) != 0 ? 1 : 0;
+}
+
+int nimg_conv2d_pool_fwd_bf16_sign(const float* in, int cin, const float* w, const void* wb, const float* bias,
+                                   float* pool_out, unsigned char* pool_idx, unsigned char* pool_sign, int cout, int n, int h,
+                                   int wd, int ks, int act, float alpha, int flags, void* stream) {
     if (n == 0) return NIMG_OK;
     if (!in || !pool_out || cin <= 0 || cout <= 0 || (cout & 3) || n < 0 || h <= 0 || wd <= 0) return NIMG_ERR_ARG;
     if ((h & 1) || (wd & 1) || (ks != 3 && ks != 5) || act < 0 || act > 1) return NIMG_ERR_ARG;
     if (n == 0) return NIMG_OK;
+    if (pool_sign && !nimg_conv2d_pool_sign_ok(cin, cout, n, h, wd, ks, flags)) return NIMG_ERR_ARG;
     hipStream_t s = (hipStream_t)stream;
     if (cin == 3 || cin == 4) {
         if (!w) return NIMG_ERR_ARG;
@@ -598,13 +625,8 @@
     }
     if (!wb || (cin % 8)) return NIMG_ERR_ARG;
     ConvParamsB p;
-    p.in1 = in; p.in2 = nullptr; p.wb = (const __bf16*)wb; p.bias = bias; p.out1 = nullptr; p.out2 = nullptr;
-    p.act1 = nullptr; p.pool_out = pool_out; p.pool_idx = pool_idx; p.convt = 0; p.flags = flags; p.in_idx = nullptr; p.res = nullptr;
-    p.out1b = nullptr;
-    p.C1 = cin; p.C2 = 0; p.O1 = cout; p.O2 = 0; p.CinP = (cin + 15) / 16 * 16;
-    p.N = n; p.H = h; p.W = wd; p.Hout = h; p.Wout = wd; p.pad_t = p.pad_l = (ks - 1) / 2;
-    p.tiles_y = p.tiles_x = 0; p.act = act; p.pad_mode = 0; p.alpha = alpha;
-    const bool tn32 = cout <= 32 || (long)cdiv(cout, 64) * cdiv(h, 16) * cdiv(wd, 16) * n < 384;
+    const bool tn32 = pool_fwd_params(p, cin, cout, n, h, wd, ks, act, alpha, flags);
+    p.in1 = in; p.wb = (const __bf16*)wb; p.bias = bias; p.pool_out = pool_out; p.pool_idx = pool_idx; p.pool_sign = pool_sign;
     if (flags & NIMG_BF16_IN)
         return ks == 3 ? conv_bf16_launch_16x16<3, true>(p, tn32, s) : conv_bf16_launch_16x16<5, true>(p, tn32, s);
     return ks == 3 ? conv_bf16_launch_16x16<3, false>(p, tn32, s) : conv_bf16_launch_16x16<5, false>(p, tn32, s);
diff --git a/neural-imaging_amd/csrc/conv_bf16_ring.h b/neural-imaging_amd/csrc/conv_bf16_ring.h
--- a/neural-imaging_amd/csrc/conv_bf16_ring.h
+++ b/neural-imaging_amd/csrc/conv_bf16_ring.h
@@ -276,8 +276,15 @@
                         if (grp >= p.N || py >= Hp || px >= Wp) return;
                         const long o = (((long)grp * Hp + py) * Wp + px) * Cout + co0 + c;
                         const float f[8] = {lo.x, lo.y, lo.z, lo.w, hi.x, hi.y, hi.z, hi.w};
-                        *reinterpret_cast<bf16x8*>(reinterpret_cast<__bf16*>(p.pool_out) + o) = pack8(f);
+                        const bf16x8 pk = pack8(f);
+                        *reinterpret_cast<bf16x8*>(reinterpret_cast<__bf16*>(p.pool_out) + o) = pk;
                         if (p.pool_idx) *reinterpret_cast<uint2*>(p.pool_idx + o) = k;
+                        if (p.pool_sign) {
+                            const uint4 pw = __builtin_bit_cast(uint4, pk);
+                            const unsigned sb = bf16x2_positive(pw.x) | (bf16x2_positive(pw.y) << 1) | (bf16x2_positive(pw.z) << 2) |
+                                                (bf16x2_positive(pw.w) << 3);
+                            p.pool_sign[o >> 3] = (unsigned char)sign_bits_interleave(sb);
+                        }
                     });
             }
             return;
@@ -315,7 +322,11 @@
 #pragma unroll
                     for (int e = 0; e < 8; ++e) f[e] = lrelu(f[e], p.alpha);
                 }
-                if (p.act1) {
+                if (p.act_sign) {
+                    const unsigned sb = p.act_sign[o >> 3];
+#pragma unroll
+                    for (int e = 0; e < 8; ++e) f[e] *= ((sb >> e) & 1u) ? 1.0f : p.alpha;
+                } else if (p.act1) {
                     const bf16x8 m = *reinterpret_cast<const bf16x8*>(reinterpret_cast<const __bf16*>(p.act1) + o);
 #pragma unroll
                     for (int e = 0; e < 8; ++e) f[e] *= (float)m[e] > 0.f ? 1.0f : p.alpha;
diff --git a/neural-imaging_amd/csrc/conv_bf16_tile.h b/neural-imaging_amd/csrc/conv_bf16_tile.h
--- a/neural-imaging_amd/csrc/conv_bf16_tile.h
+++ b/neural-imaging_amd/csrc/conv_bf16_tile.h
@@ -295,6 +295,24 @@
     }
 }
 
+inline int conv5_ring_tn(const ConvParamsB& p) {
+    static const bool no_buf = getenv("NIMG_NO_BUFFER_LOADS") != nullptr;
+    static const bool no_ring = getenv("NIMG_NO_CONV5_RING") != nullptr;
+    static const bool no_ring64 = getenv("NIMG_NO_CONV5_RING64") != nullptr;
+    static const bool tn64 = getenv("NIMG_RING_TN64") != nullptr;
+    const int Cin = p.C1 + p.C2, Cout = p.O1 + p.O2;
+    const long in_bytes = ((long)p.N * p.H * p.W * p.C1 * 2) >> (p.in_idx ? 2 : 0);
+    const long w_bytes = (long)(p.CinP >> 4) * 25 * 16 * Cout * 2;
+    if (no_buf || p.C2 != 0 || Cin % 16 != 0 || Cout % 64 != 0 || p.convt || in_bytes >= (1l << 31) - 65536 ||
+        w_bytes >= (1l << 31) - 65536)
+        return 0;
+    const bool plain_epi = !p.res && !p.out1b && !(p.flags & (NIMG_D2S_OUT | NIMG_S2D_OUT | NIMG_COPY_LRELU));
+    if (no_ring || !plain_epi || p.O2 != 0 || p.pad_t != 2 || p.pad_l != 2 || p.Hout != p.H || p.Wout != p.W) return 0;
+    if (Cout % 128 == 0 && !(tn64 && p.Hout >= 32)) return 128;
+    if (!no_ring64 && p.Hout >= 32) return 64;
+    return 0;
+}
+
 template <int KS, int STRIDE, int TH, int TW, int NB, int TN, bool INB = false, bool BUF = false, int CKT = 16>
 int launch_conv_b(const ConvParamsB& p, hipStream_t stream) {
     if constexpr (KS == 1 && !BUF && CKT == 16) {
@@ -328,14 +346,9 @@
                     return launch_conv5_ring<128, 4, 3>(p, stream);
             }
             if constexpr (KS == 5 && TH == 16 && TW == 16 && NB == 1 && TN == 64) {
-                static const bool no_ring = getenv("NIMG_NO_CONV5_RING") != nullptr;
-                static const bool no_ring64 = getenv("NIMG_NO_CONV5_RING64") != nullptr;
-                const bool plain_epi = !p.res && !p.out1b && !(p.flags & (NIMG_D2S_OUT | NIMG_S2D_OUT | NIMG_COPY_LRELU));
-                if (!no_ring && plain_epi && p.O2 == 0 && p.pad_t == 2 && p.pad_l == 2 && p.Hout == p.H && p.Wout == p.W) {
-                    static const bool tn64 = getenv("NIMG_RING_TN64") != nullptr;
-                    if (Cout % 128 == 0 && !(tn64 && p.Hout >= 32)) return launch_conv5_ring<128>(p, stream);
-                    if (!no_ring64 && p.Hout >= 32) return launch_conv5_ring<64>(p, stream);
-                }
+                const int ring = conv5_ring_tn(p);
+                if (ring == 128) return launch_conv5_ring<128>(p, stream);
+                if (ring == 64) return launch_conv5_ring<64>(p, stream);
             }
             return launch_conv_b<KS, STRIDE, TH, TW, NB, TN, true, true>(p, stream);
         }
diff --git a/neural-imaging_amd/csrc/frontend.hip b/neural-imaging_amd/csrc/frontend.hip
--- a/neural-imaging_amd/csrc/frontend.hip
+++ b/neural-imaging_amd/csrc/frontend.hip
@@ -244,7 +244,8 @@
 template <int TWD, bool OUT_BF16>
 __global__ __launch_bounds__(256, CONV1_WGS) void conv1_pool_fwd_kernel(const void* __restrict__ c4, const float* __restrict__ w,
                                                              const float* __restrict__ bias, void* __restrict__ pooled,
-                                                             unsigned char* __restrict__ pidx, int N, int H, int W,
+                                                             unsigned char* __restrict__ pidx,
+                                                             unsigned char* __restrict__ psign, int N, int H, int W,
                                                              float alpha, int tiles_y, int tiles_x) {
     constexpr int TRD = 8, HR = TRD + 4, HC = TWD + 4, NPC = HC / 2;
     constexpr int PT = NPC <= 64 ? 64 : 128, RG = 256 / PT, RPTS = (HR + RG - 1) / RG;
@@ -383,6 +384,12 @@
                     uint4* d = reinterpret_cast<uint4*>(reinterpret_cast<unsigned short*>(pooled) + po);
                     d[0] = make_uint4(pb[0], pb[1], pb[2], pb[3]);
                     d[1] = make_uint4(pb[4], pb[5], pb[6], pb[7]);
+                    if (psign) {
+                        unsigned sb = 0;
+#pragma unroll
+                        for (int g = 7; g >= 0; --g) sb = (sb << 1) | nimg::bf16x2_positive(pb[g]);
+                        *reinterpret_cast<unsigned short*>(psign + (po >> 3)) = (unsigned short)nimg::sign_bits_interleave(sb);
+                    }
                 } else {
                     float4* d = reinterpret_cast<float4*>(reinterpret_cast<float*>(pooled) + po);
 #pragma unroll
@@ -754,18 +761,18 @@
 constexpr int F1_WGS = 1024;
 
 template <int TWD>
-int launch_conv1_pool(const void* c4, const float* w, const float* bias, void* pooled, unsigned char* pidx, int n, int h,
-                      int wd, float alpha, int out_bf16, hipStream_t s) {
+int launch_conv1_pool(const void* c4, const float* w, const float* bias, void* pooled, unsigned char* pidx, unsigned char* psign,
+                      int n, int h, int wd, float alpha, int out_bf16, hipStream_t s) {
     const int tiles_y = cdiv(h, 8), tiles_x = cdiv(wd, TWD);
     const long total = (long)n * tiles_y * tiles_x;
     static const int capmul = getenv("NIMG_CONV1_CAP") ? atoi(getenv("NIMG_CONV1_CAP")) : 0;
     const long cap = 256L * (capmul > 0 ? capmul : CONV1_WGS);
     const dim3 grid((unsigned)(total < cap ? total : cap));
     if (out_bf16)
-        hipLaunchKernelGGL((conv1_pool_fwd_kernel<TWD, true>), grid, dim3(256), 0, s, c4, w, bias, pooled, pidx, n, h, wd, alpha,
-                           tiles_y, tiles_x);
+        hipLaunchKernelGGL((conv1_pool_fwd_kernel<TWD, true>), grid, dim3(256), 0, s, c4, w, bias, pooled, pidx, psign, n, h, wd,
+                           alpha, tiles_y, tiles_x);
     else
-        hipLaunchKernelGGL((conv1_pool_fwd_kernel<TWD, false>), grid, dim3(256), 0, s, c4, w, bias, pooled, pidx, n, h, wd,
+        hipLaunchKernelGGL((conv1_pool_fwd_kernel<TWD, false>), grid, dim3(256), 0, s, c4, w, bias, pooled, pidx, psign, n, h, wd,
                            alpha, tiles_y, tiles_x);
     NIMG_CHECK_LAUNCH();
     return NIMG_OK;
@@ -856,9 +863,15 @@
 
 int nimg_conv1_pool_fwd_c4(const void* c4, const float* w, const float* bias, void* pooled, unsigned char* pool_idx, int n,
                            int h, int wd, float alpha, int out_bf16, void* stream) {
+    return nimg_conv1_pool_fwd_c4_sign(c4, w, bias, pooled, pool_idx, nullptr, n, h, wd, alpha, out_bf16, stream);
+}
+
+int nimg_conv1_pool_fwd_c4_sign(const void* c4, const float* w, const float* bias, void* pooled, unsigned char* pool_idx,
+                                unsigned char* pool_sign, int n, int h, int wd, float alpha, int out_bf16, void* stream) {
     if (n == 0) return NIMG_OK;
     if (!c4 || !w || !pooled || n < 0 || h < 2 || wd < 2 || (h & 1) || (wd & 1) || !(alpha > 0.f && alpha <= 1.f))
         return NIMG_ERR_ARG;
+    if (pool_sign && !out_bf16) return NIMG_ERR_ARG;
     const long per_image = (long)h * wd * 8;
     if (per_image > 0x7fffffffL) return NIMG_ERR_ARG;
     const int chunk = (int)(0x7fffffffL / per_image);
@@ -869,8 +882,9 @@
         const void* src = (const char*)c4 + px0 * 8;
         void* dst = (char*)pooled + pp0 * esz;
         unsigned char* di = pool_idx ? pool_idx + (pp0 >> 2) : nullptr;
-        const int rc = wd > 96 ? launch_conv1_pool<256>(src, w, bias, dst, di, nn, h, wd, alpha, out_bf16, (hipStream_t)stream)
-                               : launch_conv1_pool<64>(src, w, bias, dst, di, nn, h, wd, alpha, out_bf16, (hipStream_t)stream);
+        unsigned char* ds = pool_sign ? pool_sign + (pp0 >> 3) : nullptr;
+        const int rc = wd > 96 ? launch_conv1_pool<256>(src, w, bias, dst, di, ds, nn, h, wd, alpha, out_bf16, (hipStream_t)stream)
+                               : launch_conv1_pool<64>(src, w, bias, dst, di, ds, nn, h, wd, alpha, out_bf16, (hipStream_t)stream);
         if (rc != NIMG_OK) return rc;
     }
     return NIMG_OK;
diff --git a/neural-imaging_amd/models/forensics.py b/neural-imaging_amd/models/forensics.py
--- a/neural-imaging_amd/models/forensics.py
+++ b/neural-imaging_amd/models/forensics.py
@@ -102,17 +102,18 @@
         net, nf = self._constrained.forward(P, x, c4_only=front)
         t['constrained'], t['nf'] = net, nf
         for i, c in enumerate(self._convs):
+            want_sign = training and i + 1 < len(self._convs)
             if i == 0 and front:
                 nxt = self._convs[1] if len(self._convs) > 1 else self._conv1x1
                 as_bf16 = ops.STORE_BF16 and nxt.cout >= 8
-                net, idx = ops.conv1_pool_c4(net, P.p[c.name + '/kernel'], P.p[c.name + '/bias'], want_idx=training,
-                                             out_bf16=as_bf16)
-                t['idx1'], t['front'] = idx, True
+                net, idx, *sign = ops.conv1_pool_c4(net, P.p[c.name + '/kernel'], P.p[c.name + '/bias'], want_idx=training,
+                                                    out_bf16=as_bf16, want_sign=want_sign)
+                t['idx1'], t['front'], t['sign1'] = idx, True, sign[0] if sign else None
             elif c.can_pool(net):
                 nxt = self._convs[i + 1] if i + 1 < len(self._convs) else self._conv1x1
                 as_bf16 = ops.COMPUTE == 'bf16' and ops.STORE_BF16 and c.cout % 8 == 0 and nxt.cout >= 8
-                net, idx = c.forward_pool(P, net, want_idx=training, out_bf16=as_bf16)
-                t['idx{}'.format(i + 1)] = idx
+                net, idx, *sign = c.forward_pool(P, net, want_idx=training, out_bf16=as_bf16, want_sign=want_sign)
+                t['idx{}'.format(i + 1)], t['sign{}'.format(i + 1)] = idx, sign[0] if sign else None
             else:
                 a = c.forward(P, net)
                 t['conv{}'.format(i + 1)] = a
@@ -265,7 +266,8 @@
                 params(lambda inp=inp, g=d_pool, i=i, conv=conv: ops.conv2d_wgrad_unpool(
                     inp, g, t['idx{}'.format(i)], conv.ks, dw=P.g[conv.name + '/kernel'], db=P.g[conv.name + '/bias'], side=True), i)
                 d_pool = ops.conv2d_dgrad_unpool(d_pool, t['idx{}'.format(i)], P.p[conv.name + '/kernel'], act_mask=prev_mask,
-                                                 out_bf16=g_bf16(i - 1))
+                                                 out_bf16=g_bf16(i - 1),
+                                                 act_sign=t.get('sign{}'.format(i - 1)) if prev_mask is not None else None)
                 continue
             if fused(i):
                 as_bf16 = ops.COMPUTE == 'bf16' and ops.STORE_BF16 and conv.cout % 8 == 0 and conv.cin % 8 == 0
diff --git a/neural-imaging_amd/models/layers.py b/neural-imaging_amd/models/layers.py
--- a/neural-imaging_amd/models/layers.py
+++ b/neural-imaging_amd/models/layers.py
@@ -45,9 +45,9 @@
         return self.stride == 1 and self.cin2 == 0 and self.ks in (3, 5) and self.cout % 4 == 0 and \
             x.shape[1] % 2 == 0 and x.shape[2] % 2 == 0 and self.activation == 'leaky_relu'
 
-    def forward_pool(self, store, x, want_idx=True, out_bf16=False):
+    def forward_pool(self, store, x, want_idx=True, out_bf16=False, want_sign=False):
         return ops.conv2d_pool(x, store.p[self.name + '/kernel'], store.p[self.name + '/bias'], act=self.activation,
-                               want_idx=want_idx, out_bf16=out_bf16)
+                               want_idx=want_idx, out_bf16=out_bf16, want_sign=want_sign)
 
     def forward_and_pool(self, store, x, out_bf16=False):
         w = store.p[self.name + '/kernel']
diff --git a/neural-imaging_amd/ops.py b/neural-imaging_amd/ops.py
--- a/neural-imaging_amd/ops.py
+++ b/neural-imaging_amd/ops.py
@@ -811,7 +811,16 @@
     return dz
 
 
-def conv2d_pool(x, w, bias=None, act='leaky_relu', want_idx=True, out_bf16=False):
+ACT_SIGN = _os.environ.get('NIMG_NO_ACT_SIGN') is None
+
+
+def conv2d_pool_sign_ok(x, w, out_bf16=True):
+    n, h, wd, cin = x.shape
+    return ACT_SIGN and COMPUTE == 'bf16' and _is_bf16(x) and out_bf16 and _lib.load().nimg_conv2d_pool_sign_ok(
+        cin, w.shape[3], n, h, wd, w.shape[0], BF16_IN | BF16_OUT) == 1
+
+
+def conv2d_pool(x, w, bias=None, act='leaky_relu', want_idx=True, out_bf16=False, want_sign=False):
     _f32(w, bias)
     _fb(x)
     n, h, wd, cin = x.shape
@@ -827,12 +836,17 @@
     if bf16_path:
         wb = None if cin in (3, 4) else weights_bf16(w, 0)
         flags = (BF16_IN if _is_bf16(x) else 0) | (BF16_OUT if out_bf16 else 0)
+        if want_sign and conv2d_pool_sign_ok(x, w, out_bf16):
+            sign = torch.empty((n, h // 2, wd // 2, cout // 8), dtype=torch.uint8, device=x.device)
+            _lib.call('nimg_conv2d_pool_fwd_bf16_sign', _p(x), cin, _p(w), _p(wb), _p(bias), _p(pooled), _p(idx), _p(sign), cout, n,
+                      h, wd, ks, a, LRELU_ALPHA, flags, _stream())
+            return pooled, idx, sign
         _lib.call('nimg_conv2d_pool_fwd_bf16_ex', _p(x), cin, _p(w), _p(wb), _p(bias), _p(pooled), _p(idx), cout, n, h, wd,
                   ks, a, LRELU_ALPHA, flags, _stream())
     else:
         _lib.call('nimg_conv2d_pool_fwd', _p(x), cin, _p(w), _p(bias), _p(pooled), _p(idx), cout, n, h, wd, ks, a,
                   LRELU_ALPHA, _stream())
-    return pooled, idx
+    return (pooled, idx, None) if want_sign else (pooled, idx)
 
 
 POOL_ALSO = _os.environ.get('NIMG_NO_POOL_ALSO') is None
@@ -920,12 +934,19 @@
         _os.environ.get('NIMG_NO_BUFFER_LOADS') is None
 
 
-def conv2d_dgrad_unpool(g, idx, w, act_mask=None, out_bf16=False):
+def conv2d_dgrad_unpool(g, idx, w, act_mask=None, out_bf16=False, act_sign=None):
     _f32(w)
     _fb(g, act_mask)
     _chk(idx)
     n, hp, wp, cz = g.shape
     ks, ci = w.shape[0], w.shape[2]
+    if act_sign is not None:
+        _chk(act_sign)
+        if act_mask is None or act_sign.dtype != torch.uint8 or ci % 8 or tuple(act_sign.shape) != (n, 2 * hp, 2 * wp, ci // 8) or \
+                tuple(act_mask.shape) != (n, 2 * hp, 2 * wp, ci):
+            raise ValueError('conv2d_dgrad_unpool: act_sign is the (N,H,W,Cin/8) uint8 sign plane of the act_mask given with it')
+        if not (ACT_SIGN and out_bf16 and _is_bf16(act_mask)) or SPARSE_DGRAD:
+            act_sign = None
     out = torch.empty((n, 2 * hp, 2 * wp, ci), dtype=torch.bfloat16 if out_bf16 else torch.float32, device=g.device)
     flags = (BF16_OUT if out_bf16 else 0) | (BF16_MASK if _is_bf16(act_mask) else 0)
     if SPARSE_DGRAD and ks == 5 and ci % 32 == 0 and cz % 8 == 0 and _is_bf16(g) and g.numel() * 2 < (1 << 31) - 65536:
@@ -935,6 +956,10 @@
                   flags, _stream())
         return out
     wb = weights_bf16(w, 1)
+    if act_sign is not None:
+        _lib.call('nimg_conv2d_fwd_bf16_unpool_sign', _p(g), _p(idx), cz, _p(wb), None, _p(out), ci, _p(act_mask), _p(act_sign), n,
+                  2 * hp, 2 * wp, ks, ks - 1 - (ks - 1) // 2, ks - 1 - (ks - 1) // 2, 2 * hp, 2 * wp, 0, LRELU_ALPHA, flags, _stream())
+        return out
     _lib.call('nimg_conv2d_fwd_bf16_unpool', _p(g), _p(idx), cz, _p(wb), None, _p(out), ci, _p(act_mask), n, 2 * hp, 2 * wp, ks,
               ks - 1 - (ks - 1) // 2, ks - 1 - (ks - 1) // 2, 2 * hp, 2 * wp, 0, LRELU_ALPHA, flags, _stream())
     return out
@@ -1294,7 +1319,7 @@
         h >= 4 and w >= 4 and small
 
 
-def conv1_pool_c4(c4, w, bias, act='leaky_relu', want_idx=True, out_bf16=True):
+def conv1_pool_c4(c4, w, bias, act='leaky_relu', want_idx=True, out_bf16=True, want_sign=False):
     _f32(w, bias)
     _chk(c4)
     n, h, wd, c = c4.shape
@@ -1302,9 +1327,14 @@
         raise ValueError('conv1_pool_c4: (N,H,W,4) bf16 pixels, a (5,5,3,32) kernel and even sizes expected')
     pooled = torch.empty((n, h // 2, wd // 2, 32), dtype=torch.bfloat16 if out_bf16 else torch.float32, device=c4.device)
     idx = torch.empty((n, h // 2, wd // 2, 8), dtype=torch.uint8, device=c4.device) if want_idx else None
+    if want_sign and ACT_SIGN and out_bf16:
+        sign = torch.empty((n, h // 2, wd // 2, 4), dtype=torch.uint8, device=c4.device)
+        _lib.call('nimg_conv1_pool_fwd_c4_sign', _p(c4), _p(w), _p(bias), _p(pooled), _p(idx), _p(sign), n, h, wd,
+                  LRELU_ALPHA if act == 'leaky_relu' else 1.0, 1, _stream())
+        return pooled, idx, sign
     _lib.call('nimg_conv1_pool_fwd_c4', _p(c4), _p(w), _p(bias), _p(pooled), _p(idx), n, h, wd,
               LRELU_ALPHA if act == 'leaky_relu' else 1.0, 1 if out_bf16 else 0, _stream())
-    return pooled, idx
+    return (pooled, idx, None) if want_sign else (pooled, idx)
 
 
 def conv1_wgrad_c4(c4, g, idx, dw=None, db=None, accumulate=False, side=False):
```

After: 8448 patches/s, median of 6. 1.9% higher.
